# XiangLi2022/CM-TTS

Measured on AMD Instinct MI355X. Metric: mel-frames/s (text->mel hot path, consistency sampling T=4), higher is better.
Workload: dtype f32

## Files before the change

cm-tts_amd/_lib.py:

```python
import ctypes as C
import os
import sys

_HERE = os.path.dirname(os.path.abspath(__file__))
LIB_PATH = os.environ.get("CMTTS_LIB") or os.path.join(_HERE, "libcmtts_hip.so")


class CMTTSConfigStruct(C.Structure):
    _fields_ = [(n, C.c_int32) for n in (
        "n_symbols", "hidden", "enc_layers", "enc_heads", "ffn_kernel",
        "pred_filter", "pred_layers", "pred_kernel", "dur_layers", "dur_kernel", "cwt_hidden",
        "pitch_bins", "energy_bins", "use_uv", "multi_speaker", "external_speaker_dim", "n_speaker",
        "n_mels", "res_layers", "res_channels")] + [(n, C.c_float) for n in (
            "cwt_std_scale", "pitch_norm_eps", "sigma_min", "sigma_max", "sigma_data", "rho")]


class VarianceControlsStruct(C.Structure):
    _fields_ = [("p_control", C.c_float), ("e_control", C.c_float), ("d_target", C.c_void_p), ("e_target", C.c_void_p),
                ("cwt_spec", C.c_void_p), ("f0_mean", C.c_void_p), ("f0_std", C.c_void_p), ("uv", C.c_void_p)]


class ControlTablesStruct(C.Structure):
    _fields_ = [("d", C.c_void_p), ("e", C.c_void_p), ("p", C.c_void_p), ("ld", C.c_int)]

# ... 77 lines not shown
    "cmtts_comm_destroy": (_i, [_vp]),
    "cmtts_allgather_workspace_bytes": (_sz, [_i, _i, _i, _i]),
    "cmtts_allgather_mels": (_i, [_vp, _i, _vp, _vp, _i, _i, _i, _vp, _vp, _vp, _sz, _vp]),
    "cmtts_allgather_pcm_workspace_bytes": (_sz, [_i, _i, _i64]),
    "cmtts_allgather_pcm": (_i, [_vp, _i, _vp, _vp, _i, _i64, _vp, _vp, _vp, _sz, _vp]),
    "cmtts_exchange_records": (_i, [_vp, _i, _vp, C.POINTER(_i64), _vp, C.POINTER(_i64), _sz, _vp]),
    "cmtts_transpose": (_i, [_vp, _vp, _i, _i, _i, _vp]),
    "cmtts_pack_conv_weight": (_i, [_vp, _i, _i, _i, C.POINTER(_vp), C.POINTER(_i)]),
    "cmtts_free_device": (None, [_vp]),
    "cmtts_conv1d": (_i, [_vp, _vp, _i, _vp, _i, _i, _i, _i, _i, _i, _i, _i, _vp, _vp]),
}

ABI_VERSION = 8
_lib = None
HEADER_PATH = os.path.join(os.path.dirname(_HERE), "include", "cmtts_hip.h")


def cdef_from_header(path=HEADER_PATH):
    import re
    text = open(path).read()
    text = re.sub(r"/\*.*?\*/", "", text, flags=re.S)
    lines = [ln for ln in text.splitlines() if not ln.lstrip().startswith("#")]
    text = "\n".join(lines)
    text = text.replace('extern "C" {', "")
    text = re.sub(r"^\}\s*$", "", text, flags=re.M)
    return text


def address_of(arg):
    if arg is None:
        return 0
    if isinstance(arg, int):
        return arg
    if isinstance(arg, C.c_void_p):
        return arg.value or 0
    if hasattr(arg, "_obj"):
        return C.addressof(arg._obj)
    if isinstance(arg, (C.Array, C.Structure)):
        return C.addressof(arg)
    if isinstance(arg, C._Pointer):
        return C.cast(arg, C.c_void_p).value or 0
    if hasattr(arg, "data_ptr"):
        return int(arg.data_ptr())
    raise TypeError(f"cannot take the address of {type(arg).__name__}")


class _CffiLib:

    def __init__(self, path):
        import cffi
        self.ffi = cffi.FFI()
        self.ffi.cdef(cdef_from_header())
        self._c = self.ffi.dlopen(path)
        for name, (res, args) in SIGNATURES.items():
            setattr(self, name, self._wrap(name, res, args))

    def _wrap(self, name, res, args):
        ffi, fn = self.ffi, getattr(self._c, name)
        ctypes_ = ffi.typeof(fn).args
        assert len(ctypes_) == len(args), name

        def call(*a):
            conv = []
            for v, ct, at in zip(a, ctypes_, args):
                if at is C.c_char_p:
                    conv.append(ffi.NULL if v is None else v)
                elif ct.kind == "pointer":
                    conv.append(ffi.cast(ct, address_of(v)))
                else:
                    conv.append(v.value if hasattr(v, "value") else v)
            r = fn(*conv)
            if res is C.c_char_p:
                return None if r == ffi.NULL else ffi.string(r)
            return None if res is None else int(r)
        call.__name__ = name
        return call


def _load_ctypes():
    lib = C.CDLL(LIB_PATH)
    for name, (res, args) in SIGNATURES.items():
        fn = getattr(lib, name)
        fn.restype = res
        fn.argtypes = args
    return lib


def load():
    global _lib
    if _lib is not None:
        return _lib
    if not os.path.exists(LIB_PATH):
        raise RuntimeError(
            f"{LIB_PATH} not found: build the HIP extension first "
            "(python -c 'import __graft_entry__ as g; g.build()' or make -C cm-tts_amd/csrc). "
            "cmtts_amd has no CPU or PyTorch fallback.")
    import torch
    want = os.environ.get("CMTTS_FFI", "ctypes")
    if want == "cffi":
        import cffi
        lib = _CffiLib(LIB_PATH)
    elif want == "ctypes":
        lib = _load_ctypes()
    else:
        raise RuntimeError(f"CMTTS_FFI={want!r}: expected 'ctypes' or 'cffi'")
    got = lib.cmtts_abi_version()
    if got != ABI_VERSION:
        raise RuntimeError(f"{LIB_PATH} implements ABI revision {got}, this binding was written for {ABI_VERSION} "
                           "(include/cmtts_hip.h: CMTTS_ABI_VERSION): rebuild the library")
    _lib = lib
    spec = os.environ.get("CMTTS_INTERNAL", "")
    if spec:
        if os.environ.get("CMTTS_INTERNAL_ENABLE") != "1":
            print(f"cmtts_amd: ignoring CMTTS_INTERNAL={spec!r} (measurement hook: set CMTTS_INTERNAL_ENABLE=1 to apply it)", file=sys.stderr)
        else:
            for kv in filter(None, (e.strip() for e in spec.split(","))):
                k, sep, v = kv.partition("=")
                try:
                    val = int(v)
                except ValueError:
                    val = None
                if not sep or not k.strip() or val is None:
                    raise RuntimeError(f"CMTTS_INTERNAL: malformed entry {kv!r} (expected name=integer[,name=integer...])")
                if internal_set(k.strip(), val) < 0:
                    raise RuntimeError(f"CMTTS_INTERNAL: unknown switch {k.strip()!r} (csrc/internal_hooks.h)")
                print(f"cmtts_amd: CMTTS_INTERNAL applied {k.strip()}={val}", file=sys.stderr)
    return lib


_internal = None


def internal_set(name, value):
    global _internal
    load()
    if _internal is None:
        _internal = C.CDLL(LIB_PATH).cmtts_internal_set
        _internal.restype, _internal.argtypes = _i, [C.c_char_p, _i]
    return _internal(name if isinstance(name, bytes) else name.encode(), int(value))


_noise_bits = None


def internal_noise_bits(seeds, B, T, M, first_draw, n_draws, t0, bits, stream):
    global _noise_bits
    load()
    if _noise_bits is None:
        _noise_bits = C.CDLL(LIB_PATH).cmtts_internal_noise_bits
        _noise_bits.restype, _noise_bits.argtypes = _i, [_vp, _i, _i, _i, _i, _i, _i64, _vp, _vp]
    return _noise_bits(seeds, int(B), int(T), int(M), int(first_draw), int(n_draws), int(t0), bits, stream)


def backend():
    return "cffi" if isinstance(load(), _CffiLib) else "ctypes"


def check(rc):
    if rc != 0:
        msg = load().cmtts_last_error()
        raise RuntimeError(f"libcmtts_hip error {rc}: {msg.decode() if msg else '?'}")
```

cm-tts_amd/csrc/cmtts_api.hip:

```cpp
#include <hip/hip_runtime.h>
#include <limits.h>
#include <math.h>
#include <stdio.h>
#include <stdlib.h>
#include <string.h>

#include <algorithm>
#include <map>
#include <string>
#include <vector>

#include "../../include/cmtts_hip.h"
#include "internal_hooks.h"
#include "conv_args.h"
#include "kernels.h"
#include "resblock_args.h"
#include "persist_args.h"
#include "cond_gemm.h"
#include "resblock_pair.h"
#include "inproj.h"
#include "attention.h"
#include "text_state.h"
#include "stream_windows.h"
#include "resample.h"
// ... 966 lines not shown
            }
        if (H % 16 == 0 && (NL * C) % 32 == 0 && m->cond_all.ld == NL * C) {
            const std::vector<unsigned short> fs = to_fragment16_split(hp, 1, H, NL * C);
            CHK(al.upload_bytes(fs.data(), fs.size() * 2, &m->cond_all_f16[2]));
        }
    }
    CHK(al.upload(dproj, &m->dproj_wt));
    if (c.multi_speaker) CHK(al.upload(sproj, &m->sproj_wt));
    {
        GET(w, "net.skip_projection.conv.weight", C, C, 1); GET(b, "net.skip_projection.conv.bias", C);
        std::vector<float> hp;
        CHK(pack_conv(al, *w, b, nullptr, &m->skip_proj, &hp));
        if (C % 32 == 0 && m->skip_proj.ld == C) CHK(al.upload(to_fragment_order(hp, 1, C, C), &m->skip_f));
        GET(w2, "net.output_projection.conv.weight", c.n_mels, C, 1); GET(b2, "net.output_projection.conv.bias", c.n_mels);
        CHK(pack_conv(al, *w2, b2, nullptr, &m->out_proj, &hp));
        {
            const int ld = m->out_proj.ld, Mp = round_up(c.n_mels, 32);
            std::vector<float> padded((size_t)C * Mp, 0.f);
            for (int k = 0; k < C; ++k)
                for (int n = 0; n < c.n_mels; ++n) padded[(size_t)k * Mp + n] = hp[(size_t)k * ld + n];
            CHK(al.upload(to_fragment_order(padded, 1, C, Mp), &m->outp_f));
        }
    }
    if (m->cond_all_f && (NL * C) % 512 == 0) {
        GET(pe, va + "pitch_embed.weight", c.pitch_bins, H);
        float* peT = nullptr;
        void* p2 = nullptr;
        CHK(al.upload(transpose2d(pe->data.data(), c.pitch_bins, H), &peT));
        CHK(al.upload(std::vector<float>((size_t)NL * C, 0.f), &m->cond_zero_bias));
        HIPCHK(hipMalloc(&p2, (size_t)NL * C * c.pitch_bins * sizeof(float) + 256));
        al.ptrs.push_back(p2);
        CondGemmArgs ga;
        memset(&ga, 0, sizeof(ga));
        ga.X = peT; ga.Wf = m->cond_all_f; ga.bias = m->cond_all.bias; ga.Y = (float*)p2;
        ga.B = 1; ga.T = c.pitch_bins; ga.M = NL * C; ga.K = H; ga.force = 1; ga.row_split = NL * C / 512;
        if (cmtts_launch_cond_gemm(&ga, nullptr) == 0) {
            void* p2t = nullptr;
            HIPCHK(hipMalloc(&p2t, (size_t)NL * C * c.pitch_bins * sizeof(float) + 256));
            al.ptrs.push_back(p2t);
            k_transpose((const float*)p2, (float*)p2t, NL, C, c.pitch_bins, nullptr);
            HIPCHK(hipStreamSynchronize(nullptr));
            m->cond_p2 = (float*)p2;
            m->cond_p2t = (float*)p2t;
        }
    }
#undef GET
#undef UP
    m->host.clear();
    m->finalized = true;
    return 0;
}

constexpr int FFN2_SEG = 8;
struct TextWs {
    float *x, *h, *qk, *vt, *st, *o, *f, *part, *c1, *c2, *spk, *out1, *h128, *logd, *dround, *epred, *escaled, *pctl;
    int* cum;
    int64_t *eidx, *mlen;
    size_t bytes;
};
TextWs carve_text(const cmtts_config& c, int B, int L, void* base) {
    const int Lp = round_up(L, 4), H = c.hidden;
    Carver cv(base);
    TextWs w;
    const size_t n = (size_t)B * H * Lp;
    w.out1 = cv.take<float>(n);
    w.cum = cv.take<int>((size_t)B * L);
    w.spk = cv.take<float>((size_t)B * H);
    w.h128 = cv.take<float>((size_t)B * c.cwt_hidden * Lp);
    w.x = cv.take<float>(n);
    w.h = cv.take<float>(n);
    w.qk = cv.take<float>(3 * n);
    w.vt = w.qk + 2 * n;
    w.st = cv.take<float>((size_t)B * c.enc_heads * Lp * Lp);
    w.o = cv.take<float>(n);
    w.f = cv.take<float>(4 * n);
    w.part = cv.take<float>(FFN2_SEG * n);
    w.c1 = cv.take<float>(n);
    w.c2 = cv.take<float>(n);
    w.logd = cv.take<float>((size_t)B * L);
    w.dround = cv.take<float>((size_t)B * L);
    w.epred = cv.take<float>((size_t)B * L);
    w.eidx = cv.take<int64_t>((size_t)B * L);
    w.mlen = cv.take<int64_t>((size_t)B);
    w.escaled = cv.take<float>((size_t)B * L);
    w.pctl = cv.take<float>((size_t)B * L);
    w.bytes = cv.off + 256;
    return w;
}

struct FrameWs {
    float *xlr, *h128, *hp, *c1, *c2, *cwt, *r, *s1, *s2, *stats, *f0;
    int64_t* pidx;
    size_t bytes;
};
FrameWs carve_frame(const cmtts_config& c, int B, int T, void* base) {
    Carver cv(base);
    FrameWs w;
    const size_t n = (size_t)B * c.hidden * T;
    w.xlr = cv.take<float>(n);
    w.h128 = cv.take<float>((size_t)B * c.cwt_hidden * T);
    w.hp = cv.take<float>((size_t)B * c.cwt_hidden * T);
    w.c1 = cv.take<float>(n);
    w.c2 = cv.take<float>(n);
    w.cwt = cv.take<float>((size_t)B * T * 16);
    w.r = cv.take<float>((size_t)B * T);
    w.s1 = cv.take<float>((size_t)B * c.cwt_hidden);
    w.s2 = cv.take<float>((size_t)B * c.cwt_hidden);
    w.stats = cv.take<float>((size_t)B * 2);
    w.f0 = cv.take<float>((size_t)B * T);
    w.pidx = cv.take<int64_t>((size_t)B * T);
    w.bytes = cv.off + 256;
    return w;
}

struct DenWs {
    float *hin, *h, *u, *zb, *skip, *emb, *e1, *e2, *dproj, *sproj, *dp, *tbuf, *xcur, *cp;
    float* pst;
    unsigned long long* halo;
    size_t bytes;
};
DenWs carve_den(const cmtts_config& c, int B, int T, void* base) {
    Carver cv(base);
    DenWs w;
    const int C = c.res_channels, NL = c.res_layers;
    const size_t n = (size_t)B * C * T;
    w.hin = cv.take<float>((size_t)B * c.n_mels * T);
    w.h = cv.take<float>(n);
    w.u = cv.take<float>(n);
    w.zb = cv.take<float>(n);
    w.skip = cv.take<float>(n);
    w.emb = cv.take<float>((size_t)B * C);
    w.e1 = cv.take<float>((size_t)B * 4 * C);
    w.e2 = cv.take<float>((size_t)B * C);
    w.dproj = cv.take<float>((size_t)B * NL * C);
    w.sproj = cv.take<float>((size_t)B * NL * C);
    w.dp = cv.take<float>((size_t)B * NL * C);
    w.tbuf = cv.take<float>((size_t)B);
    w.xcur = cv.take<float>((size_t)B * T * c.n_mels);
    w.cp = cv.take<float>((size_t)NL * n);
    w.halo = cv.take<unsigned long long>(cmtts_persist_halo_bytes(B, T) / sizeof(unsigned long long));
    w.pst = cv.take<float>(cmtts_persist_state_floats(B, T));
    w.bytes = cv.off + 256;
    return w;
}

struct EnergyHead {
    const float* xin; const float* e_target; float e_control; const float* bins; int nbins; const float* E; float* out1; int64_t* e_idx; float* e_scaled;
    bool done;
    const float* e_table = nullptr;
};
int g_energy_head = 1;
int g_pred_wino = 1;
int g_pred_xres = 1;
int predictor(const Predictor& P, const float* in, int ld_in, int B, int T, int ld, const int64_t* ln_lens,
              const int64_t* out_lens, float* bufA, float* bufB, float* out, int O, hipStream_t s, int mode16 = 0, bool frame_level = false,
              EnergyHead* eh = nullptr) {
    const float* cur = in;
    int ldc = ld_in;
    auto other = [&](const float* p) { return p == bufA ? bufB : bufA; };
    int pend_ln = -1;
    for (size_t li = 0; li < P.convs.size(); ++li) {
        const PackedConv& w = P.convs[li];
        int rx = -2;
        float* dst = other(cur);
        if (frame_level && !mode16 && g_pred_wino && !ln_lens && li < P.convs_q.size() && P.convs_q[li] && w.taps == 5 && w.cout == 256 &&
            (pend_ln < 0 || w.cin == 256)) {
            ConvXlArgs xa;
            memset(&xa, 0, sizeof(xa));
            xa.x = cur; xa.y = dst; xa.wf = P.convs_q[li]; xa.bias = w.bias; xa.bstride = (long)w.cout * ld;
            xa.B = B; xa.C = 256; xa.T = T; xa.ld = ld; xa.k = w.taps; xa.dil = 1; xa.slope = 1.0f; xa.relu = 1;
            if (w.cin != 256) { xa.cin = w.cin; xa.xbstride = (long)w.cin * ldc; }
            if (pend_ln >= 0) { xa.ln_g = P.ln_g[pend_ln]; xa.ln_b = P.ln_b[pend_ln]; xa.ln_eps = 1e-12f; }
            if (ldc == ld || w.cin != 256) {
                rx = cmtts_launch_conv_k5q(&xa, (void*)s);
                if (rx == -3) return fail(CMTTS_E_HIP, "conv_k5q launch failed");
                if (rx == 0) pend_ln = -2;
            }
        }
        const bool small = (long)((T + 63) / 64) * B < 192;
        if (rx != 0 && !mode16 && g_pred_xres && small && P.convs_f[li] && w.cin == 256 && w.cout == 256 && ldc == ld) {
            ConvArgs a = conv_args(w, cur, T, ldc, (long)w.cin * ldc, dst, ld, (long)w.cout * ld, T);
            a.out[0].act = ACT_RELU;
            a.xres_nt = 1;
            if (pend_ln >= 0) { a.ln_g = P.ln_g[pend_ln]; a.ln_b = P.ln_b[pend_ln]; a.ln_eps = 1e-12f; a.ln_lens = ln_lens; a.ln_skip_tiles = 1; }
            rx = cmtts_launch_conv_xres(&a, P.convs_f[li], B, (void*)s);
            if (rx == -3) return fail(CMTTS_E_HIP, "conv_xres launch failed");
            if (rx == 0) pend_ln = -2;
        }
        if (pend_ln >= 0) {
            float* nd = other(cur);
            k_layernorm_ct(cur, nd, P.ln_g[pend_ln], P.ln_b[pend_ln], 1e-12f, ln_lens, B, T, ld, s);
            cur = nd;
            dst = other(cur);
        }
        pend_ln = -1;
        if (mode16 && li < P.convs_f16[mode16 - 1].size() && P.convs_f16[mode16 - 1][li]) {
            ConvArgs a = conv_args(w, cur, T, ldc, (long)w.cin * ldc, dst, ld, (long)w.cout * ld, T);
            a.out[0].act = ACT_RELU;
            a.text_epi = 1;
            rx = cmtts_launch_conv16(&a, P.convs_f16[mode16 - 1][li], mode16, B, (void*)s);
            if (rx == -3) return fail(CMTTS_E_HIP, "text16: predictor conv launch failed");
        }
        if (rx != 0 && g_pred_xl && P.convs_f[li] && ldc == ld && (long)((T + 63) / 64) * B >= 192) {
            ConvXlArgs xa;
            memset(&xa, 0, sizeof(xa));
            xa.x = cur; xa.y = dst; xa.wf = P.convs_f[li]; xa.bias = w.bias; xa.bstride = (long)w.cout * ld;
            xa.B = B; xa.C = 256; xa.T = T; xa.ld = ld; xa.k = w.taps; xa.dil = 1; xa.slope = 1.0f; xa.relu = 1;
            if (w.cin != 256) { xa.cin = w.cin; xa.xbstride = (long)w.cin * ldc; }
            rx = cmtts_launch_conv_xl(&xa, (void*)s);
            if (rx == -3) return fail(CMTTS_E_HIP, "conv_xl launch failed");
        }
        if (rx != 0) {
            ConvArgs a = conv_args(w, cur, T, ldc, (long)w.cin * ldc, dst, ld, (long)w.cout * ld, T);
            a.out[0].act = ACT_RELU;
            CHK(launch(a, EPI_PLAIN, B, s));
        }
        cur = dst;
        ldc = ld;
        if (g_pred_head && eh && g_energy_head && O == 1 && li + 1 == P.convs.size() && w.cout == 256) {
            k_ln_linear_energy(cur, P.ln_g[li], P.ln_b[li], 1e-12f, P.lin_w, P.lin_b, out, ln_lens, out_lens, B, T, ld, eh->xin, eh->e_target, eh->e_control,
                               eh->bins, eh->nbins, eh->E, eh->out1, eh->e_idx, eh->e_scaled, s, eh->e_table);
            eh->done = true;
            return 0;
        }
        if (g_pred_head && li + 1 == P.convs.size() && w.cout == 256 &&
            k_ln_linear(cur, P.ln_g[li], P.ln_b[li], 1e-12f, P.lin_w, P.lin_b, out, ln_lens, out_lens, B, T, ld, O, s))
            return 0;
        pend_ln = (int)li;
    }
    if (pend_ln >= 0) {
        float* nd = other(cur);
        k_layernorm_ct(cur, nd, P.ln_g[pend_ln], P.ln_b[pend_ln], 1e-12f, ln_lens, B, T, ld, s);
        cur = nd;
    }
    k_chan_linear(cur, P.lin_w, P.lin_b, out, out_lens, B, P.convs.back().cout, T, ld, O, s);
    return 0;
}

int cond_projections(cmtts_model* m, const DenWs& w, const float* cond_ct, int B, int T, hipStream_t s) {
    const cmtts_config& c = m->cfg;
    if (g_cond_gemm16 && m->precision >= 1 && m->precision <= 3 && m->cond_all_f16[m->precision - 1]) {
        CondGemmArgs g;
        g.X = cond_ct; g.Wf = nullptr; g.bias = m->cond_all.bias; g.Y = w.cp;
        g.row_split = 0;
        g.B = B; g.T = T; g.M = c.res_layers * c.res_channels; g.K = c.hidden; g.force = 1;
        const int r = cmtts_launch_cond_gemm16(&g, m->cond_all_f16[m->precision - 1], m->precision, (void*)s);
        if (r == 0) return 0;
        if (r != -2) return fail(CMTTS_E_HIP, "cond_gemm16 launch failed");
    }
    if (m->cond_all_f) {
        CondGemmArgs g;
        g.X = cond_ct; g.Wf = m->cond_all_f; g.bias = m->cond_all.bias; g.Y = w.cp;
        g.row_split = 0;
        g.B = B; g.T = T; g.M = c.res_layers * c.res_channels; g.K = c.hidden; g.force = g_cond_gemm == 2;
        const int r = g_cond_gemm ? cmtts_launch_cond_gemm(&g, (void*)s) : -2;
        if (r == 0) return 0;
        if (r != -2) return fail(CMTTS_E_HIP, "cond_gemm launch failed");
    }
    ConvArgs a = conv_args(m->cond_all, cond_ct, T, T, (long)c.hidden * T, w.cp, T, (long)c.res_layers * c.res_channels * T, T);
    return launch(a, EPI_PLAIN, B, s);
}

struct CondFactors {
    const float* p1 = nullptr;
    const float* p1t = nullptr;
    int ldp = 0, L = 0;
    const int64_t* mel2ph = nullptr;
    const int64_t* p_idx = nullptr;
    bool usable(const cmtts_model* m) const;
};
int g_cond_factored = 1;
int g_cond_inkernel = 1;
inline bool C_IS_256(const cmtts_config& c) { return c.res_channels == 256; }
bool CondFactors::usable(const cmtts_model* m) const {
    return g_cond_factored && p1 && mel2ph && p_idx && m->precision == 0 && m->cond_p2 && g_fused_resblock;
}
int cond_factored(cmtts_model* m, const DenWs& w, const CondFactors& f, int B, int T, hipStream_t s) {
    const cmtts_config& c = m->cfg;
    const int r = cmtts_launch_cond_expand(f.p1, f.ldp, f.L, m->cond_p2, c.pitch_bins, f.mel2ph, f.p_idx, w.cp, B, c.res_layers * c.res_channels, T, (void*)s);
    return r == 0 ? 0 : fail(CMTTS_E_HIP, "cond_expand launch failed");
}
int cond_phoneme_factor(cmtts_model* m, const float* out1, int B, int Lp, float* p1, hipStream_t s) {
    const cmtts_config& c = m->cfg;
    if (!m->cond_p2) return fail(CMTTS_E_UNSUPPORTED, "factored conditioner projections are not available for this model");
    CondGemmArgs g;
    memset(&g, 0, sizeof(g));
    g.X = out1; g.Wf = m->cond_all_f; g.bias = m->cond_zero_bias; g.Y = p1;
    g.B = B; g.T = Lp; g.M = c.res_layers * c.res_channels; g.K = c.hidden; g.force = 1;
    g.flat = 1;
    const long tiles = ((long)B * Lp + 63) / 64;
    const int npass = g.M / 512;
    int best = 1;
    double best_t = 1e30;
    for (int sp = 1; sp <= npass; ++sp) {
        const int ppg = (npass + sp - 1) / sp, groups = (npass + ppg - 1) / ppg;
        const long wg = tiles * groups, cap = persist_blocks();
        const double t = (double)((wg + cap - 1) / cap) * ppg;
        if (t < best_t - 1e-9) { best_t = t; best = sp; }
    }
    g.row_split = best;
    const int r = cmtts_launch_cond_gemm(&g, (void*)s);
    return r == 0 ? 0 : fail(r == -2 ? CMTTS_E_UNSUPPORTED : CMTTS_E_HIP, "cond_gemm (phoneme factor) launch failed");
}

int step_embedding(cmtts_model* m, const DenWs& w, const float* timesteps, const float* spk, int B, hipStream_t s,
                   float t_host = NAN) {
    const cmtts_config& c = m->cfg;
    const int C = c.res_channels, NL = c.res_layers;
    if (c.multi_speaker && !spk) return fail(CMTTS_E_INVALID, "speaker_emb is required for a multi-speaker model");
    const bool cacheable = g_step_cache && t_host == t_host;
    if (cacheable) {
        for (const cmtts_model::StepRow& e : m->step_rows)
            if (e.t == t_host && hipEventQuery(e.ready) == hipSuccess) {
                k_broadcast_row(e.row, w.dproj, B, NL * C, s);
                if (c.multi_speaker) {
                    k_dense_small(spk, c.hidden, 1, m->sproj_wt, nullptr, nullptr, w.sproj, B, c.hidden, NL * C, DENSE_NONE, s);
                    k_add_rows(w.dproj, w.sproj, w.dp, (long)B * NL * C, s);
                }
                return 0;
            }
    }
    k_diff_embed(timesteps, m->omega_res, w.emb, B, C, s);
    k_dense_small(w.emb, C, 1, m->mlp0_wt, nullptr, nullptr, w.e1, B, C, 4 * C, DENSE_MISH, s);
    k_dense_small(w.e1, 4 * C, 1, m->mlp2_wt, nullptr, nullptr, w.e2, B, 4 * C, C, DENSE_NONE, s);
    k_dense_small(w.e2, C, 1, m->dproj_wt, nullptr, nullptr, w.dproj, B, C, NL * C, DENSE_NONE, s);
    if (c.multi_speaker) {
        k_dense_small(spk, c.hidden, 1, m->sproj_wt, nullptr, nullptr, w.sproj, B, c.hidden, NL * C, DENSE_NONE, s);
        k_dense_small(w.e2, C, 1, m->dproj_wt, nullptr, w.sproj, w.dp, B, C, NL * C, DENSE_NONE, s);
    }
    if (cacheable && m->step_rows.size() < 16) {
        bool known = false;
        for (const cmtts_model::StepRow& e : m->step_rows) known = known || e.t == t_host;
        if (!known) {
            cmtts_model::StepRow e{t_host, nullptr, nullptr};
            void* p = nullptr;
            if (hipMalloc(&p, (size_t)NL * C * sizeof(float)) == hipSuccess && hipEventCreateWithFlags(&e.ready, hipEventDisableTiming) == hipSuccess) {
                e.row = (float*)p;
                m->al.ptrs.push_back(p);
                HIPCHK(hipMemcpyAsync(e.row, w.dproj, (size_t)NL * C * sizeof(float), hipMemcpyDeviceToDevice, s));
                HIPCHK(hipEventRecord(e.ready, s));
                m->step_rows.push_back(e);
            } else if (p) {
                (void)hipFree(p);
            }
        }
    }
    return 0;
}

struct MelPost {
    const float* xold;
    const float* noise;
    float c_out, c_skip, nstd;
    float* out;
};

int denoiser_prologue(cmtts_model* m, const DenWs& w, const float* x_src, float in_scale, const float* timesteps, const float* spk, int B,
                      int T, hipStream_t s, bool embed, float t_host, bool* halo_zeroed) {
    const cmtts_config& c = m->cfg;
    const int C = c.res_channels, NL = c.res_layers, M = c.n_mels;
    const long cs = (long)C * T;
    *halo_zeroed = false;
    int rin = -2;
    if (g_inproj_fused && m->in_proj_f) {
        InProjArgs ia;
        memset(&ia, 0, sizeof(ia));
        ia.x = x_src; ia.scale = in_scale; ia.wf = m->in_proj_f; ia.bias = m->in_proj.bias; ia.h = w.h;
        ia.B = B; ia.T = T; ia.M = M; ia.C = C;
        const bool persist_path = g_fused_resblock && g_persist && NL <= PERSIST_MAX_LAYERS;
        if (persist_path) { ia.zero = w.halo; ia.zero_f4 = (long)(cmtts_persist_halo_bytes(B, T) / 16); }
        rin = cmtts_launch_inproj(&ia, (void*)s);
        if (rin == -3) return fail(CMTTS_E_HIP, "inproj launch failed");
        *halo_zeroed = rin == 0 && persist_path && cmtts_persist_halo_bytes(B, T) % 16 == 0;
    }
    if (rin != 0) {
        k_mel_prep(x_src, nullptr, in_scale, w.hin, B, T, M, s);
        ConvArgs a = conv_args(m->in_proj, w.hin, T, T, (long)M * T, w.h, T, cs, T);
        a.out[0].act = ACT_RELU;
        CHK(launch(a, EPI_PLAIN, B, s));
    }
    if (embed) CHK(step_embedding(m, w, timesteps, spk, B, s, t_host));
    return 0;
}

int batch_invariant_form(const cmtts_model* m) {
    if (!m->batch_invariant || m->precision != 0 || !m->winograd || !g_persist_wino || !m->res[0].w3w) return 0;
    return m->winograd == 1 && g_persist_wino == 3 && m->res[0].w3w43 ? 1 : -1;
}
int check_batch_invariant(const cmtts_model* m) {
    if (batch_invariant_form(m) >= 0) return 0;
    return fail(CMTTS_E_UNSUPPORTED, "batch_invariant: the persistent denoiser stack runs the F(2,3) form (model option \"winograd\" = 2), "
                                     "which has no per-layer counterpart; set \"winograd\" to 1 or 0");
}

int denoiser_core(cmtts_model* m, const DenWs& w, const float* x_src, float in_scale, const float* timesteps,
                  const float* cond_ct, const float* spk, int B, int T, const MelPost& post, hipStream_t s, bool embed = true,
                  SideStream* pending = nullptr, float t_host = NAN,
                  const CondFactors* cfk = nullptr, bool* cp_ready = nullptr) {
    CHK(check_device_flag(true));
    const cmtts_config& c = m->cfg;
    const int C = c.res_channels, NL = c.res_layers, M = c.n_mels;
    const long cs = (long)C * T;
    bool halo_zeroed = false;
    CHK(denoiser_prologue(m, w, x_src, in_scale, timesteps, spk, B, T, s, embed, t_host, &halo_zeroed));
    if (pending) CHK(branch_join(pending));
    const float* dp = m->cfg.multi_speaker ? w.dp : w.dproj;
    const bool unfused = !g_fused_resblock;
    float* hcur = w.h;
    float* halt = w.u;
    bool layers_done = false;
    if (!unfused && g_persist && NL <= PERSIST_MAX_LAYERS) {
        PersistArgs pa;
        memset(&pa, 0, sizeof(pa));
        pa.x0 = w.h; pa.cp = w.cp; pa.cp_bstride = (long)NL * C * T;
        pa.dp = dp; pa.d = w.dproj; pa.vec_stride = (long)NL * C;
        pa.skip = w.skip; pa.halo = w.halo; pa.tmo = g_tmo_host;
        pa.B = B; pa.T = T; pa.NL = NL;
        pa.halo_zeroed = halo_zeroed;
        const int prec = m->precision;
        if (cfk && !(cp_ready && *cp_ready)) {
            pa.fact = 1; pa.p1 = cfk->p1; pa.p2 = m->cond_p2; pa.mel2ph = (const long long*)cfk->mel2ph; pa.pidx = (const long long*)cfk->p_idx;
            pa.ldp = cfk->ldp; pa.Lph = cfk->L; pa.ld2 = c.pitch_bins;
            pa.p1t = cfk->p1t; pa.p2t = m->cond_p2t;
        }
        if (g_persist_tail && m->skip_f && m->outp_f) {
            pa.tail = 1;
            pa.Wsf = m->skip_f; pa.bs = m->skip_proj.bias; pa.Wpf = m->outp_f; pa.bp = m->out_proj.bias;
            pa.skip_div = (float)sqrt((double)NL); pa.n_mels = M;
            pa.xold = post.xold; pa.noise = post.noise; pa.c_out = post.c_out; pa.c_skip = post.c_skip; pa.nstd = post.nstd;
            pa.out = post.out;
        }
        pa.wino = g_persist_wino && m->winograd && !prec && m->res[0].w3w && w.pst;
        if (pa.wino && g_persist_wino == 3 && m->winograd == 1 && m->res[0].w3w43) pa.wino = 3;
        pa.xst = w.pst;
        for (int l = 0; l < NL; ++l) {
            pa.W3f[l] = prec ? (const float*)m->res[l].w3f16[prec - 1] : (pa.wino == 3 ? m->res[l].w3w43 : pa.wino ? m->res[l].w3w : m->res[l].w3f);
            pa.Wof[l] = prec ? (const float*)m->res[l].wof16[prec - 1] : m->res[l].wof;
            pa.b3[l] = m->res[l].b3f; pa.bo[l] = m->res[l].outp.bias;
        }
        const bool prof = g_prof.on && g_prof.used + 2 <= g_prof.ev.size();
        const int need = cmtts_persist_plan(B, T, NL, persist_blocks(), g_persist == 2);
        if (need) CHK(persist_admit(s, need, persist_blocks()));
        if (prof) (void)hipEventRecord(g_prof.ev[g_prof.used], s);
        const int rc = prec ? cmtts_launch_denoiser_persist_lp(&pa, prec, persist_blocks(), g_persist == 2, (void*)s)
                            : cmtts_launch_denoiser_persist(&pa, persist_blocks(), g_persist == 2, (void*)s);
        if (rc == -3) return fail(CMTTS_E_HIP, "persistent denoiser launch failed");
        if (rc == 0) {
            CHK(persist_launched(s, need));
            if (prof) { (void)hipEventRecord(g_prof.ev[g_prof.used + 1], s); g_prof.used += 2; }
            layers_done = true;
            if (pa.tail) return 0;
        }
    }
    if (!layers_done && cfk && !(cp_ready && *cp_ready)) {
        CHK(cond_factored(m, w, *cfk, B, T, s));
        if (cp_ready) *cp_ready = true;
    }
    const bool w43 = batch_invariant_form(m) > 0;
    for (int l = 0; l < NL && !layers_done; ++l) {
        const ResLayer& R = m->res[l];
        const bool prof = g_prof.on && g_prof.used + 2 <= g_prof.ev.size() && (g_prof.seen++ % g_prof.stride) == 0;
        if (!unfused) {
            ResArgs ra;
            memset(&ra, 0, sizeof(ra));
            ra.x_in = hcur; ra.cp = w.cp + (long)l * C * T; ra.cp_bstride = (long)NL * C * T;
            ra.dp = dp + (long)l * C; ra.d = w.dproj + (long)l * C;
            ra.x_out = halt; ra.skip = w.skip;
            ra.W3f = R.w3f; ra.b3 = R.b3f; ra.Wof = R.wof; ra.bo = R.outp.bias;
            ra.vec_stride = (long)NL * C; ra.B = B; ra.T = T; ra.accum_skip = l > 0; ra.flag = g_tmo_host;
            if (prof) (void)hipEventRecord(g_prof.ev[g_prof.used], s);
            int lrc;
            if (m->precision == 0 || m->precision == 3) {
                const long tiles32 = (long)((T + 31) / 32) * B;
                ra.z = w.zb;
                if (w43) {
                    ra.W3f = R.w3w43;
                    lrc = cmtts_launch_resblock_w43(&ra, (void*)s);
                } else if (g_split_resblock == 2 || (g_split_resblock == 1 && tiles32 <= SPLIT_MAX_TILES)) lrc = cmtts_launch_resblock_split(&ra, (void*)s);
                else lrc = cmtts_launch_resblock(&ra, (void*)s);
            } else {
                ra.W3f = (const float*)R.w3f16[m->precision - 1];
                ra.Wof = (const float*)R.wof16[m->precision - 1];
                lrc = cmtts_launch_resblock_lp(&ra, m->precision, (void*)s);
            }
            if (lrc != 0) return fail(CMTTS_E_HIP, "fused residual block launch failed");
            if (prof) { (void)hipEventRecord(g_prof.ev[g_prof.used + 1], s); g_prof.used += 2; }
            float* t = hcur; hcur = halt; halt = t;
            continue;
        }
        {
            ConvArgs a = conv_args(R.cond, cond_ct, T, T, (long)c.hidden * T, halt, T, cs, T);
            a.out[0].bvec = dp + (long)l * C; a.out[0].bvec_zs = (long)NL * C;
            a.out[0].res = hcur; a.out[0].r_zs0 = cs; a.out[0].ldr = T;
            CHK(launch(a, EPI_PLAIN, B, s));
        }
        if (w43) {
            ResArgs ra;
            memset(&ra, 0, sizeof(ra));
            ra.u = halt; ra.x_in = hcur; ra.x_out = halt; ra.skip = w.skip; ra.z = w.zb;
            ra.d = w.dproj + (long)l * C; ra.dp = dp + (long)l * C; ra.cp = w.cp;
            ra.W3f = R.w3w43; ra.b3 = R.b3f; ra.Wof = R.wof; ra.bo = R.outp.bias;
// ... 235 lines not shown
            }
        }
        if (ffn_fused) {
            k_reduce_partials(w.part, FFN2_SEG, E.ffn2.bias, w.x, src_lens, w.x, B, H, L, Lp, s);
        } else if (ffn2_seg) {
            const int kseg = E.ffn2.cin / FFN2_SEG;
            ConvArgs a = conv_args(E.ffn2, w.f, L, Lp, 4 * hs, w.part, Lp, (long)FFN2_SEG * hs, L);
            a.K = kseg;
            a.zdiv = FFN2_SEG; a.a_zs0 = 0; a.a_zs1 = (long)kseg * a.a_ld; a.x_zs1 = (long)kseg * Lp;
            a.out[0].y_zs1 = hs; a.out[0].bias = nullptr;
            CHK(launch(a, EPI_PLAIN, B * FFN2_SEG, s));
            k_reduce_partials(w.part, FFN2_SEG, E.ffn2.bias, w.x, src_lens, w.x, B, H, L, Lp, s);
        } else {
            ConvArgs a = conv_args(E.ffn2, w.f, L, Lp, 4 * hs, w.x, Lp, hs, L);
            a.out[0].res = w.x; a.out[0].r_zs0 = hs; a.out[0].ldr = Lp; a.out[0].lens = src_lens;
            CHK(launch(a, EPI_PLAIN, B, s));
        }
    }
    return 0;
}

int cmtts_text_forward(cmtts_model* m, const int64_t* texts, const int64_t* src_lens, const float* spker_embeds,
                       const int64_t* speakers, int B, int L, float d_control, float* log_d, float* d_rounded, int64_t* mel_len,
                       float* e_pred, int64_t* e_idx, float* enc_out_ct, float* speaker_emb,
                       void* text_ws, size_t text_ws_bytes, void* stream) {
    return cmtts_text_forward_ragged(m, texts, src_lens, nullptr, spker_embeds, speakers, B, L, d_control, log_d, d_rounded, mel_len, e_pred,
                                     e_idx, enc_out_ct, speaker_emb, text_ws, text_ws_bytes, stream);
}

int cmtts_text_forward_ragged(cmtts_model* m, const int64_t* texts, const int64_t* src_lens, const int64_t* pad_lens, const float* spker_embeds,
                              const int64_t* speakers, int B, int L, float d_control, float* log_d, float* d_rounded, int64_t* mel_len,
                              float* e_pred, int64_t* e_idx, float* enc_out_ct, float* speaker_emb,
                              void* text_ws, size_t text_ws_bytes, void* stream) {
    if (!m || !m->finalized) return fail(CMTTS_E_INVALID, "model not finalized");
    if (!texts || !src_lens || !text_ws || B <= 0 || L <= 0) return fail(CMTTS_E_INVALID, "cmtts_text_forward: bad argument");
    const cmtts_config& c = m->cfg;
    if (c.multi_speaker && c.n_speaker > 0 && !speakers) return fail(CMTTS_E_INVALID, "speakers (ids into the speaker_emb table) are required (model/cmtts.py:78)");
    if (c.multi_speaker && c.n_speaker <= 0 && !spker_embeds) return fail(CMTTS_E_INVALID, "Speaker embedding should not be None (model/cmtts.py:80)");
    const cmtts_control_tables& ct = m->ct;
    if ((ct.d || ct.e || ct.p) && ct.ld != L)
        return fail(CMTTS_E_INVALID, "cmtts_text_forward: the control tables' row pitch ld must equal L (cmtts_set_control_tables)");
    if (ct.d && d_control != 1.0f)
        return fail(CMTTS_E_INVALID, "cmtts_text_forward: a duration table replaces d_control, which must then be 1");
    if (ct.e && m->vc.e_control != 1.0f)
        return fail(CMTTS_E_INVALID, "cmtts_text_forward: an energy table replaces e_control, which must then be 1");
    TextWs w = carve_text(c, B, L, text_ws);
    if (text_ws_bytes < w.bytes) return fail(CMTTS_E_WORKSPACE, "text workspace too small");
    hipStream_t s = (hipStream_t)stream;
    const int H = c.hidden, Lp = round_up(L, 4);
    if (!log_d) log_d = w.logd;
    if (!d_rounded) d_rounded = w.dround;
    if (!mel_len) mel_len = w.mlen;
    if (!e_pred) e_pred = w.epred;
    if (!e_idx) e_idx = w.eidx;

    k_embed_tokens(texts, src_lens, m->embed, m->omega_h, m->pe_h, PE_ROWS, w.x, B, L, Lp, H, (float)sqrt((double)H), s);
    CHK(fft_stack(m, m->enc, w, src_lens, B, L, s, pad_lens));
    k_layernorm_ct(w.x, w.x, m->encln_g, m->encln_b, 1e-5f, src_lens, B, L, Lp, s);
    if (enc_out_ct && c.multi_speaker)
        k_copy_rows(enc_out_ct, L, w.x, Lp, L, (long)B * H, s);
    if (c.multi_speaker) {
        if (c.n_speaker > 0) k_gather_rows(m->spk_table, speakers, w.spk, B, H, c.n_speaker, s);
        else k_dense_small(spker_embeds, c.external_speaker_dim, 1, m->spk_wt, m->spk_b, nullptr, w.spk, B,
                      c.external_speaker_dim, H, DENSE_NONE, s);
        k_add_rowvec(w.x, w.spk, B, H, L, Lp, s, pad_lens);
        if (speaker_emb) HIPCHK(hipMemcpyAsync(speaker_emb, w.spk, (size_t)B * H * 4, hipMemcpyDeviceToDevice, s));
    }
    SideStream* ss = side_for(s);
    hipStream_t se = ss ? ss->side : s;
    float* ec1 = ss ? w.qk : w.c1;
    float* ec2 = ss ? w.qk + (size_t)B * H * Lp : w.c2;
    if (ss) CHK(branch_fork(ss));
    const int t16mode = (m->text16 && (m->precision == 1 || m->precision == 2)) ? m->precision : 0;
    CHK(predictor(m->dur, w.x, Lp, B, L, Lp, src_lens, src_lens, w.c1, w.c2, log_d, 1, s, t16mode));
    if (m->vc.d_target) {
        HIPCHK(hipMemcpyAsync(d_rounded, m->vc.d_target, (size_t)B * L * 4, hipMemcpyDeviceToDevice, s));
        k_cumsum_durations(m->vc.d_target, w.cum, mel_len, B, L, s);
    } else if (ct.d) {
        k_durations_table(log_d, ct.d, d_rounded, w.cum, mel_len, B, L, s);
    } else {
        k_durations(log_d, d_control, d_rounded, w.cum, mel_len, B, L, s);
    }
    if (ct.p) HIPCHK(hipMemcpyAsync(w.pctl, ct.p, (size_t)B * L * 4, hipMemcpyDeviceToDevice, s));
    if (enc_out_ct && !c.multi_speaker)
        k_copy_rows(enc_out_ct, L, w.x, Lp, L, (long)B * H, s);
    k_pos_embed_add(w.x, w.h, m->energy.alpha, m->omega_h, m->pe_h, PE_ROWS, B, H, L, Lp, se);
    EnergyHead eh{w.x, m->vc.e_target, m->vc.e_control, m->energy_bins, c.energy_bins - 1, m->energy_emb, w.out1, e_idx, w.escaled, false, ct.e};
    CHK(predictor(m->energy, w.h, Lp, B, L, Lp, pad_lens, pad_lens, ec1, ec2, e_pred, 1, se, t16mode, false, H == 256 ? &eh : nullptr));
    if (ss) CHK(branch_join(ss));
    if (!eh.done)
        k_energy_embed(w.x, e_pred, w.escaled, m->vc.e_target, m->vc.e_control, m->energy_bins, c.energy_bins - 1, m->energy_emb,
                       w.out1, e_idx, B, H, L, Lp, s, ct.e);
    {
        ConvArgs a = conv_args(m->cwt_in, w.out1, L, Lp, (long)H * Lp, w.h128, Lp, (long)c.cwt_hidden * Lp, L);
        int rc = -2;
        if (g_ffn_xres && g_pred_xres && m->cwt_in_f) {
            a.xres_nt = 1;
            rc = cmtts_launch_conv_xres(&a, m->cwt_in_f, B, (void*)s);
            if (rc == -3) return fail(CMTTS_E_HIP, "conv_xres launch failed");
            a.xres_nt = 0;
        }
        if (rc != 0) CHK(launch(a, EPI_PLAIN, B, s));
    }
    if (!m->vc.e_target && (ct.e || m->vc.e_control != 1.0f))
        HIPCHK(hipMemcpyAsync(e_pred, w.escaled, (size_t)B * L * 4, hipMemcpyDeviceToDevice, s));
    HIPCHK(hipGetLastError());
    return 0;
}

int cmtts_frame_forward(cmtts_model* m, const void* text_ws, int B, int L, int T, float* cond_ct, int64_t* mel2ph,
                        float* cwt_out, float* f0_denorm, int64_t* p_idx, float* f0_stats, void* frame_ws,
                        size_t frame_ws_bytes, void* stream) {
    return cmtts_frame_forward_sub(m, text_ws, B, L, 0, B, T, cond_ct, mel2ph, cwt_out, f0_denorm, p_idx, f0_stats, nullptr, frame_ws, frame_ws_bytes, stream);
}

int cmtts_frame_forward_sub(cmtts_model* m, const void* text_ws, int B_all, int L_all, int b0, int B, int T, float* cond_ct, int64_t* mel2ph,
                            float* cwt_out, float* f0_denorm, int64_t* p_idx, float* f0_stats, float* cond_p1, void* frame_ws,
                            size_t frame_ws_bytes, void* stream) {
    return cmtts_frame_forward_sub_t(m, text_ws, B_all, L_all, b0, B, T, cond_ct, mel2ph, cwt_out, f0_denorm, p_idx, f0_stats, cond_p1, nullptr, frame_ws,
                                     frame_ws_bytes, stream);
}

int cmtts_frame_forward_sub_t(cmtts_model* m, const void* text_ws, int B_all, int L_all, int b0, int B, int T, float* cond_ct, int64_t* mel2ph,
                              float* cwt_out, float* f0_denorm, int64_t* p_idx, float* f0_stats, float* cond_p1, float* cond_p1t, void* frame_ws,
                              size_t frame_ws_bytes, void* stream) {
    if (!m || !m->finalized) return fail(CMTTS_E_INVALID, "model not finalized");
    if (!text_ws || !frame_ws || !cond_ct || !mel2ph || B <= 0 || L_all <= 0 || T <= 0 || b0 < 0 || b0 + B > B_all)
        return fail(CMTTS_E_INVALID, "cmtts_frame_forward: bad argument");
    const cmtts_config& c = m->cfg;
    const int L = L_all;
    TextWs tw = carve_text(c, B_all, L_all, const_cast<void*>(text_ws));
    tw.out1 += (size_t)b0 * c.hidden * round_up(L_all, 4);
    tw.h128 += (size_t)b0 * c.cwt_hidden * round_up(L_all, 4);
    tw.cum += (size_t)b0 * L_all;
    tw.pctl += (size_t)b0 * L_all;
    if (m->ct.p && m->ct.ld != L_all)
        return fail(CMTTS_E_INVALID, "cmtts_frame_forward: the control tables' row pitch ld must equal L_all (cmtts_set_control_tables)");
    if (m->ct.p && m->vc.p_control != 1.0f)
        return fail(CMTTS_E_INVALID, "cmtts_frame_forward: a pitch table replaces p_control, which must then be 1");
    FrameWs w = carve_frame(c, B, T, frame_ws);
    if (frame_ws_bytes < w.bytes) return fail(CMTTS_E_WORKSPACE, "frame workspace too small");
    hipStream_t s = (hipStream_t)stream;
    const int H = c.hidden, Lp = round_up(L, 4), O = c.use_uv ? 11 : 10, CH = c.cwt_hidden;
    if (!cwt_out) cwt_out = w.cwt;
    if (!f0_denorm) f0_denorm = w.f0;
    if (!p_idx) p_idx = w.pidx;
    if (!f0_stats) f0_stats = w.stats;

    SideStream* ss = side_for(s);
    hipStream_t sst = ss ? ss->side : s;
    if (ss) CHK(branch_fork(ss));
    if (cond_p1t && !cond_p1) return fail(CMTTS_E_INVALID, "cmtts_frame_forward_sub_t: cond_p1t needs cond_p1");
    if (cond_p1 && m->cond_p2) {
        CHK(cond_phoneme_factor(m, tw.out1, B, Lp, cond_p1, sst));
        if (cond_p1t) k_transpose(cond_p1, cond_p1t, B * c.res_layers, c.res_channels, Lp, sst);
    }
    if (!(g_stats_mlp && k_stats_mlp(tw.out1, (long)H * Lp, Lp, m->st0_wt, m->st0_b, m->st2_wt, m->st2_b, m->st4_wt, m->st4_b, f0_stats, B, H, CH, CH, 2, sst))) {
        k_dense_small(tw.out1, (long)H * Lp, Lp, m->st0_wt, m->st0_b, nullptr, w.s1, B, H, CH, DENSE_RELU, sst);
        k_dense_small(w.s1, CH, 1, m->st2_wt, m->st2_b, nullptr, w.s2, B, CH, CH, DENSE_RELU, sst);
        k_dense_small(w.s2, CH, 1, m->st4_wt, m->st4_b, nullptr, f0_stats, B, CH, 2, DENSE_NONE, sst);
    }
    k_mel2ph(tw.cum, mel2ph, B, L, T, s);
    if (!g_cwt_in_phoneme) k_length_regulate(tw.out1, mel2ph, w.xlr, B, H, Lp, T, s);
    bool hp_done = false;
    if (g_cwt_in_phoneme) {
        k_pos_embed_add_lr(tw.h128, Lp, mel2ph, m->cwt_in.bias, w.hp, m->cwt.alpha, m->omega_cwt, m->pe_cwt, PE_ROWS, B, CH, T, s);
        hp_done = true;
    } else {
        ConvArgs a = conv_args(m->cwt_in, w.xlr, T, T, (long)H * T, w.h128, T, (long)CH * T, T);
        CHK(launch(a, EPI_PLAIN, B, s));
    }
    if (!hp_done) k_pos_embed_add(w.h128, w.hp, m->cwt.alpha, m->omega_cwt, m->pe_cwt, PE_ROWS, B, CH, T, T, s);
    CHK(predictor(m->cwt, w.hp, T, B, T, T, nullptr, nullptr, w.c1, w.c2, cwt_out, O, s, (m->text16 && (m->precision == 1 || m->precision == 2)) ? m->precision : 0, true));
    if (ss) CHK(branch_join(ss));
    if (m->ct.p) k_pitch_table_scale(cwt_out, mel2ph, tw.cum, tw.pctl, B, O, L, T, s);
    else if (m->vc.p_control != 1.0f) k_scale(cwt_out, cwt_out, (long)B * T * O, m->vc.p_control, s);
    if (m->vc.cwt_spec) {
        k_pitch_index(m->vc.cwt_spec, 10, m->vc.f0_mean, m->vc.f0_std, 1, 1.0f, nullptr, 0, c.use_uv ? m->vc.uv : nullptr,
                      c.pitch_norm_eps, w.r, p_idx, f0_denorm, B, T, s);
    } else {
        k_pitch_index(cwt_out, O, f0_stats, f0_stats + 1, 2, c.cwt_std_scale, c.use_uv ? cwt_out + (O - 1) : nullptr, O, nullptr,
                      c.pitch_norm_eps, w.r, p_idx, f0_denorm, B, T, s);
    }
    if (g_cwt_in_phoneme) k_lr_gather_add(tw.out1, mel2ph, Lp, p_idx, m->pitch_emb, cond_ct, B, H, T, s);
    else k_gather_add(w.xlr, p_idx, m->pitch_emb, cond_ct, B, H, T, s);
    HIPCHK(hipGetLastError());
    return 0;
}

namespace {
struct TextStateLayout {
    long off[TEXT_STATE_MAX_REGIONS], bytes[TEXT_STATE_MAX_REGIONS], stride[TEXT_STATE_MAX_REGIONS];
    long rec_bytes;
    int n_regions;
};
TextStateLayout text_state_layout(const cmtts_config& c, int L, bool with_p) {
    const int Lp = round_up(L, 4);
    TextStateLayout t;
    t.bytes[0] = (long)c.hidden * Lp * 4;
    t.bytes[1] = (long)c.cwt_hidden * Lp * 4;
    t.bytes[2] = (long)c.hidden * 4;
    t.bytes[3] = (long)L * 4;
    t.bytes[4] = (long)L * 4;
    t.n_regions = with_p ? 5 : 4;
    long off = TEXT_STATE_HEADER_BYTES;
    for (int g = 0; g < t.n_regions; ++g) {
        t.stride[g] = t.bytes[g];
        t.off[g] = off;
        off += (t.bytes[g] + 15) / 16 * 16;
    }
    t.rec_bytes = off;
    return t;
}
TextStateCopy text_state_args(const cmtts_config& c, void* ws, int B_all, int L, void* records, int n, int unpack, bool with_p) {
    const TextStateLayout t = text_state_layout(c, L, with_p);
    TextWs tw = carve_text(c, B_all, L, ws);
    char* base[TEXT_STATE_MAX_REGIONS] = {(char*)tw.out1, (char*)tw.h128, (char*)tw.spk, (char*)tw.cum, (char*)tw.pctl};
    TextStateCopy a;
    memset(&a, 0, sizeof(a));
    int chunks = 0;
    for (int g = 0; g < t.n_regions; ++g) {
        TextStateRegion& R = a.reg[g];
        R.ws = base[g]; R.ws_stride = t.stride[g]; R.rec_off = t.off[g]; R.bytes = t.bytes[g];
        R.vec16 = ((uintptr_t)R.ws % 16 == 0 && R.ws_stride % 16 == 0 && R.bytes % 16 == 0 && (uintptr_t)records % 16 == 0) ? 1 : 0;
        R.chunk0 = chunks;
        chunks += (int)((R.bytes + TEXT_STATE_CHUNK - 1) / TEXT_STATE_CHUNK);
    }
    a.n_regions = t.n_regions; a.n_chunks = chunks; a.unpack = unpack;
    a.layout = with_p ? TEXT_STATE_LAYOUT_P : TEXT_STATE_LAYOUT;
    a.n = n; a.B_all = B_all; a.L_all = L; a.hidden = c.hidden; a.cwt_hidden = c.cwt_hidden;
    a.rec = (char*)records; a.rec_bytes = t.rec_bytes;
    a.cum = tw.cum;
    return a;
}
}

size_t cmtts_text_state_record_bytes(const cmtts_model* m, int L_all) {
    if (!m || L_all <= 0) return 0;
    return (size_t)text_state_layout(m->cfg, L_all, m->ct.p != nullptr).rec_bytes;
}

int cmtts_text_state_pack(cmtts_model* m, const void* text_ws, int B_all, int L_all, const int32_t* rows, int n, const int64_t* global_idx,
                          const int64_t* src_lens, void* records, void* stream) {
    if (!m || !m->finalized) return fail(CMTTS_E_INVALID, "model not finalized");
    if (!text_ws || !records || (n > 0 && !rows) || B_all <= 0 || L_all <= 0 || n < 0)
        return fail(CMTTS_E_INVALID, "cmtts_text_state_pack: bad argument");
    if ((uintptr_t)records % 16) return fail(CMTTS_E_INVALID, "cmtts_text_state_pack: records must be 16-byte aligned");
    if (m->ct.p && m->ct.ld != L_all)
        return fail(CMTTS_E_INVALID, "cmtts_text_state_pack: the control tables' row pitch ld must equal L_all (cmtts_set_control_tables)");
    TextStateCopy a = text_state_args(m->cfg, const_cast<void*>(text_ws), B_all, L_all, records, n, 0, m->ct.p != nullptr);
    a.rows = rows; a.index = global_idx; a.src_lens = src_lens;
    if (cmtts_launch_text_state_copy(&a, stream) != 0) return fail(CMTTS_E_HIP, "text-state pack launch failed");
    return 0;
}

int cmtts_text_state_unpack(cmtts_model* m, const void* records, int n, int L_all, void* text_ws, size_t text_ws_bytes, void* stream) {
    if (!m || !m->finalized) return fail(CMTTS_E_INVALID, "model not finalized");
    if (!text_ws || !records || n <= 0 || L_all <= 0) return fail(CMTTS_E_INVALID, "cmtts_text_state_unpack: bad argument");
    if ((uintptr_t)records % 16) return fail(CMTTS_E_INVALID, "cmtts_text_state_unpack: records must be 16-byte aligned");
    if (text_ws_bytes < carve_text(m->cfg, n, L_all, nullptr).bytes) return fail(CMTTS_E_WORKSPACE, "text workspace too small");
    if (m->ct.p && m->ct.ld != L_all)
        return fail(CMTTS_E_INVALID, "cmtts_text_state_unpack: the control tables' row pitch ld must equal L_all (cmtts_set_control_tables)");
    TextStateCopy a = text_state_args(m->cfg, text_ws, n, L_all, const_cast<void*>(records), n, 1, m->ct.p != nullptr);
    if (cmtts_launch_text_state_copy(&a, stream) != 0) return fail(CMTTS_E_HIP, "text-state unpack launch failed");
    return 0;
}

int cmtts_length_regulate(const float* x_ct, const float* durations, int B, int C, int L, int T, float* out_ct,
                          int64_t* mel2ph, int64_t* mel_len, int32_t* scratch_cum, void* stream) {
    if (!x_ct || !durations || !out_ct || !mel2ph || !mel_len || !scratch_cum || B <= 0 || L <= 0 || T <= 0)
        return fail(CMTTS_E_INVALID, "cmtts_length_regulate: bad argument");
    hipStream_t s = (hipStream_t)stream;
    k_cumsum_durations(durations, scratch_cum, mel_len, B, L, s);
    k_mel2ph(scratch_cum, mel2ph, B, L, T, s);
    k_length_regulate(x_ct, mel2ph, out_ct, B, C, L, T, s);
    HIPCHK(hipGetLastError());
    return 0;
}

int cmtts_denoiser_forward(cmtts_model* m, const float* x, const float* timesteps, const float* cond_ct,
                           const float* speaker_emb, int B, int T, float* out, void* ws, size_t ws_bytes, void* stream) {
    if (!m || !m->finalized) return fail(CMTTS_E_INVALID, "model not finalized");
    if (!x || !timesteps || !cond_ct || !out || !ws || B <= 0 || T <= 0)
        return fail(CMTTS_E_INVALID, "cmtts_denoiser_forward: bad argument");
    CHK(check_batch_invariant(m));
    DenWs w = carve_den(m->cfg, B, T, ws);
    if (ws_bytes < w.bytes) return fail(CMTTS_E_WORKSPACE, "denoiser workspace too small");
    hipStream_t s = (hipStream_t)stream;
    SideStream* ss = g_fused_resblock ? side_for(s) : nullptr;
    if (ss) CHK(branch_fork(ss));
    if (g_fused_resblock) CHK(cond_projections(m, w, cond_ct, B, T, ss ? ss->side : s));
    const MelPost post = {nullptr, nullptr, 1.0f, 0.0f, 0.0f, out};
    CHK(denoiser_core(m, w, x, 1.0f, timesteps, cond_ct, speaker_emb, B, T, post, s, true, ss));
    HIPCHK(hipGetLastError());
    return 0;
}

int cmtts_schedule(const cmtts_model* m, int n_steps, float* sigmas, float* renoise_std) {
    if (!m || !sigmas || !renoise_std || n_steps < 1) return fail(CMTTS_E_INVALID, "cmtts_schedule: bad argument");
    const cmtts_config& c = m->cfg;
    if (n_steps == 1) {
        sigmas[0] = c.sigma_max;
        renoise_std[0] = -1.0f;
        return 0;
    }
    const double rho = c.rho, tmax = pow((double)c.sigma_max, 1.0 / rho), tmin = pow((double)c.sigma_min, 1.0 / rho);
    for (int i = 0; i < n_steps; ++i) {
        const double tsi = 0.0, tsn = (i + 1 == n_steps) ? 1.0 : 0.0;
        const double t = pow(tmax + tsi / 1.0 * (tmin - tmax), rho);
        double nt = pow(tmax + tsn / 1.0 * (tmin - tmax), rho);
        nt = nt < c.sigma_min ? (double)c.sigma_min : (nt > c.sigma_max ? (double)c.sigma_max : nt);
        sigmas[i] = (float)t;
        renoise_std[i] = (float)sqrt(nt * nt - (double)c.sigma_min * (double)c.sigma_min);
    }
    return 0;
}

}
namespace {
int sample_core(cmtts_model* m, const DenWs& w, const float* noise, long noise_stride, const float* cond_ct, const float* speaker_emb, int B,
                int T, int n_steps, const float* sigmas, const float* renoise_std, float* mel, hipStream_t s, const CondFactors* cf = nullptr,
                const int64_t* seeds = nullptr) {
    const cmtts_config& c = m->cfg;
    const long nel = (long)B * T * c.n_mels;
    SideStream* ss = g_fused_resblock ? side_for(s) : nullptr;
    if (ss) CHK(branch_fork(ss));
    const CondFactors* cfk = nullptr;
    CondFactors cf_local;
    bool cp_ready = false;
    if (g_fused_resblock) {
        if (cf && cf->usable(m)) {
            const bool inkernel = g_cond_inkernel && g_persist && g_persist_tail && m->skip_f && m->outp_f && c.res_layers <= PERSIST_MAX_LAYERS &&
                                  cmtts_persist_plan(B, T, c.res_layers, persist_blocks(), g_persist == 2) > 0;
            if (inkernel && cf->ldp <= T && m->cond_p2t && C_IS_256(c)) {
                cf_local = *cf;
                if (!cf_local.p1t) {
                    k_transpose(cf->p1, w.cp, B * c.res_layers, c.res_channels, cf->ldp, ss ? ss->side : s);
                    cf_local.p1t = w.cp;
                }
                cfk = &cf_local;
            } else CHK(cond_factored(m, w, *cf, B, T, ss ? ss->side : s));
        } else CHK(cond_projections(m, w, cond_ct, B, T, ss ? ss->side : s));
    }
    const float* renoise0 = noise + noise_stride;
    if (seeds) {
        renoise0 = noise;
        int n_re = 0;
        for (int i = 0; i < n_steps; ++i)
            if (renoise_std[i] >= 0.0f) n_re = i + 1;
        if (cmtts_launch_noise_fill(seeds, B, T, c.n_mels, 0, 1, 0, c.sigma_max, w.xcur, nullptr, (void*)s) != 0 ||
            (n_re && cmtts_launch_noise_fill(seeds, B, T, c.n_mels, 1, n_re, 0, 1.0f, const_cast<float*>(noise), nullptr, (void*)(ss ? ss->side : s)) != 0))
            return fail(CMTTS_E_HIP, "seeded noise launch failed");
    } else
        k_scale(noise, w.xcur, nel, c.sigma_max, s);
    const float smin = c.sigma_min, sd2 = c.sigma_data * c.sigma_data;
    for (int i = 0; i < n_steps; ++i) {
        const float sg = sigmas[i];
        const float dm = sg - smin;
        const float c_skip = sd2 / (dm * dm + sd2);
        const float rt = sqrtf(sg * sg + sd2);
        const float c_out = dm * c.sigma_data / rt;
        const float c_in = 1.0f / rt;
        const float t_resc = 250.0f * logf(sg + 1e-44f);
        const bool new_sigma = i == 0 || sigmas[i] != sigmas[i - 1];
        const bool embed_side = i == 0 && ss != nullptr;
        if (new_sigma) k_fill_float(w.tbuf, t_resc, B, embed_side ? ss->side : s);
        if (embed_side) CHK(step_embedding(m, w, w.tbuf, speaker_emb, B, ss->side, t_resc));
        const bool last = i + 1 == n_steps;
        const bool renoise = renoise_std[i] >= 0.0f;
        const MelPost post = {w.xcur, renoise ? renoise0 + (long)i * noise_stride : nullptr, c_out, c_skip,
                              renoise ? renoise_std[i] : 0.0f, last ? mel : w.xcur};
        CHK(denoiser_core(m, w, w.xcur, c_in, w.tbuf, cond_ct, speaker_emb, B, T, post, s, new_sigma && !embed_side, i == 0 ? ss : nullptr, t_resc, cfk, &cp_ready));
    }
    HIPCHK(hipGetLastError());
    return 0;
}

DenWs den_slice(const cmtts_config& c, const DenWs& w, int b0, int T) {
    const long C = c.res_channels, NL = c.res_layers, M = c.n_mels;
    DenWs v = w;
    v.hin += (long)b0 * M * T; v.h += b0 * C * T; v.u += b0 * C * T; v.zb += b0 * C * T; v.skip += b0 * C * T;
    v.emb += b0 * C; v.e1 += b0 * 4 * C; v.e2 += b0 * C; v.dproj += b0 * NL * C; v.sproj += b0 * NL * C; v.dp += b0 * NL * C;
    v.tbuf += b0; v.xcur += (long)b0 * T * M; v.cp += (long)b0 * NL * C * T;
    return v;
}
}
extern "C" {

int cmtts_sample(cmtts_model* m, const float* noise, const float* cond_ct, const float* speaker_emb, int B, int T,
                 int n_steps, const float* sigmas, const float* renoise_std, float* mel, void* ws, size_t ws_bytes,
                 void* stream) {
    if (!m || !m->finalized) return fail(CMTTS_E_INVALID, "model not finalized");
    if (!noise || !cond_ct || !mel || !ws || !sigmas || !renoise_std || B <= 0 || T <= 0 || n_steps < 1)
        return fail(CMTTS_E_INVALID, "cmtts_sample: bad argument");
    CHK(check_batch_invariant(m));
    const cmtts_config& c = m->cfg;
    DenWs w = carve_den(c, B, T, ws);
    if (ws_bytes < w.bytes) return fail(CMTTS_E_WORKSPACE, "denoiser workspace too small");
    return sample_core(m, w, noise, (long)B * T * c.n_mels, cond_ct, speaker_emb, B, T, n_steps, sigmas, renoise_std, mel, (hipStream_t)stream);
}

int cmtts_sample_factored(cmtts_model* m, const float* noise, const float* cond_ct, const float* speaker_emb, int B, int T,
                          int n_steps, const float* sigmas, const float* renoise_std, float* mel, void* ws, size_t ws_bytes,
                          void* stream, const float* cond_p1, int p1_ld, int L, const int64_t* mel2ph, const int64_t* p_idx) {
    return cmtts_sample_factored_t(m, noise, cond_ct, speaker_emb, B, T, n_steps, sigmas, renoise_std, mel, ws, ws_bytes, stream, cond_p1, nullptr, p1_ld, L,
                                   mel2ph, p_idx);
}

int cmtts_sample_factored_t(cmtts_model* m, const float* noise, const float* cond_ct, const float* speaker_emb, int B, int T,
                            int n_steps, const float* sigmas, const float* renoise_std, float* mel, void* ws, size_t ws_bytes,
                            void* stream, const float* cond_p1, const float* cond_p1t, int p1_ld, int L, const int64_t* mel2ph, const int64_t* p_idx) {
    if (!m || !m->finalized) return fail(CMTTS_E_INVALID, "model not finalized");
    if (!noise || !cond_ct || !mel || !ws || !sigmas || !renoise_std || B <= 0 || T <= 0 || n_steps < 1)
        return fail(CMTTS_E_INVALID, "cmtts_sample_factored: bad argument");
    if (cond_p1 && (!mel2ph || !p_idx || L <= 0 || p1_ld < L)) return fail(CMTTS_E_INVALID, "cmtts_sample_factored: incomplete factors");
    CHK(check_batch_invariant(m));
    const cmtts_config& c = m->cfg;
    DenWs w = carve_den(c, B, T, ws);
    if (ws_bytes < w.bytes) return fail(CMTTS_E_WORKSPACE, "denoiser workspace too small");
    CondFactors cf;
    cf.p1 = cond_p1; cf.ldp = p1_ld; cf.L = L; cf.mel2ph = mel2ph; cf.p_idx = p_idx;
    cf.p1t = cond_p1 ? cond_p1t : nullptr;
    return sample_core(m, w, noise, (long)B * T * c.n_mels, cond_ct, speaker_emb, B, T, n_steps, sigmas, renoise_std, mel, (hipStream_t)stream,
                       cond_p1 ? &cf : nullptr);
}

int cmtts_noise_fill(const int64_t* seeds, int B, int T, int M, int first_draw, int n_draws, int64_t t0, float* out, void* stream) {
    if (!seeds || !out || B < 1 || T < 1 || M < 1 || n_draws < 1 || first_draw < 0 || t0 < 0)
        return fail(CMTTS_E_INVALID, "cmtts_noise_fill: bad argument");
    const int rc = cmtts_launch_noise_fill(seeds, B, T, M, first_draw, n_draws, t0, 1.0f, out, nullptr, stream);
    if (rc == -2) return fail(CMTTS_E_UNSUPPORTED, "cmtts_noise_fill: B or n_draws > 65535, or T * ceil(M / 4) >= 2^31");
    if (rc != 0) return fail(CMTTS_E_HIP, "cmtts_noise_fill: launch failed");
    return 0;
}

int cmtts_noise_fill_groups(const cmtts_noise_group* groups, int n_groups, int M, int first_draw, int n_draws, void* stream) {
    if (!groups || n_groups < 1 || M < 1 || n_draws < 1 || first_draw < 0) return fail(CMTTS_E_INVALID, "cmtts_noise_fill_groups: bad argument");
    std::vector<NoiseGroup> gs((size_t)n_groups);
    for (int g = 0; g < n_groups; ++g) {
        const cmtts_noise_group& G = groups[g];
        if (!G.seeds || !G.out || G.B < 1 || G.T < 1) return fail(CMTTS_E_INVALID, "cmtts_noise_fill_groups: bad group");
        gs[g] = NoiseGroup{G.seeds, G.out, G.B, G.T, 0, 1};
    }
    const int rc = cmtts_launch_noise_fill_groups(gs.data(), n_groups, M, first_draw, n_draws, stream);
    if (rc == -2) return fail(CMTTS_E_UNSUPPORTED, "cmtts_noise_fill_groups: n_draws > 65535 or a launch of more than 2^31 - 1 workgroups");
    if (rc != 0) return fail(CMTTS_E_HIP, "cmtts_noise_fill_groups: launch failed");
    return 0;
}

int cmtts_internal_noise_bits(const int64_t* seeds, int B, int T, int M, int first_draw, int n_draws, int64_t t0, uint32_t* bits, void* stream) {
    if (!seeds || !bits || B < 1 || T < 1 || M < 1 || n_draws < 1 || first_draw < 0 || t0 < 0)
        return fail(CMTTS_E_INVALID, "cmtts_internal_noise_bits: bad argument");
    if (cmtts_launch_noise_fill(seeds, B, T, M, first_draw, n_draws, t0, 1.0f, nullptr, bits, stream) != 0)
        return fail(CMTTS_E_HIP, "cmtts_internal_noise_bits: launch failed");
    return 0;
}

static size_t seeded_tail_offset(const cmtts_config& c, int B, int T) { return (carve_den(c, B, T, nullptr).bytes + 255) & ~(size_t)255; }
size_t cmtts_sample_seeded_workspace_bytes(const cmtts_model* m, int B, int T, int n_steps) {
    if (!m || B < 1 || T < 1 || n_steps < 1) return 0;
    return seeded_tail_offset(m->cfg, B, T) + (size_t)n_steps * B * T * m->cfg.n_mels * sizeof(float);
}

int cmtts_sample_seeded(cmtts_model* m, const int64_t* seeds, const float* cond_ct, const float* speaker_emb, int B, int T,
                        int n_steps, const float* sigmas, const float* renoise_std, float* mel, void* ws, size_t ws_bytes,
                        void* stream, const float* cond_p1, const float* cond_p1t, int p1_ld, int L, const int64_t* mel2ph, const int64_t* p_idx) {
    if (!m || !m->finalized) return fail(CMTTS_E_INVALID, "model not finalized");
    if (!seeds || !cond_ct || !mel || !ws || !sigmas || !renoise_std || B <= 0 || T <= 0 || n_steps < 1)
        return fail(CMTTS_E_INVALID, "cmtts_sample_seeded: bad argument");
    if (cond_p1 && (!mel2ph || !p_idx || L <= 0 || p1_ld < L)) return fail(CMTTS_E_INVALID, "cmtts_sample_seeded: incomplete factors");
    CHK(check_batch_invariant(m));
    const cmtts_config& c = m->cfg;
    if (B > 65535) return fail(CMTTS_E_UNSUPPORTED, "cmtts_sample_seeded: B > 65535");
    DenWs w = carve_den(c, B, T, ws);
    if (ws_bytes < cmtts_sample_seeded_workspace_bytes(m, B, T, n_steps)) return fail(CMTTS_E_WORKSPACE, "seeded sampler workspace too small");
    const float* tail = reinterpret_cast<const float*>(static_cast<char*>(ws) + seeded_tail_offset(c, B, T));
    CondFactors cf;
    cf.p1 = cond_p1; cf.ldp = p1_ld; cf.L = L; cf.mel2ph = mel2ph; cf.p_idx = p_idx;
    cf.p1t = cond_p1 ? cond_p1t : nullptr;
    return sample_core(m, w, tail, (long)B * T * c.n_mels, cond_ct, speaker_emb, B, T, n_steps, sigmas, renoise_std, mel, (hipStream_t)stream,
                       cond_p1 ? &cf : nullptr, seeds);
}

int cmtts_sample_ragged(cmtts_model* m, const cmtts_sample_group* groups, int n_groups, int n_steps, const float* sigmas,
                        const float* renoise_std, int tail_frames, void* stream) {
    if (!m || !m->finalized) return fail(CMTTS_E_INVALID, "model not finalized");
    if (!groups || n_groups < 1 || n_steps < 1 || !sigmas || !renoise_std || tail_frames < 0)
        return fail(CMTTS_E_INVALID, "cmtts_sample_ragged: bad argument");
    CHK(check_batch_invariant(m));
    const cmtts_config& c = m->cfg;
    const int C = c.res_channels, NL = c.res_layers, M = c.n_mels;
    hipStream_t s = (hipStream_t)stream;
    long padded_tiles = 0;
    for (int g = 0; g < n_groups; ++g) {
        const cmtts_sample_group& G = groups[g];
        if (!G.noise || !G.cond_ct || !G.mel || !G.ws || G.B <= 0 || G.T <= 0) return fail(CMTTS_E_INVALID, "cmtts_sample_ragged: bad group");
        if (c.multi_speaker && !G.speaker_emb) return fail(CMTTS_E_INVALID, "speaker_emb is required for a multi-speaker model");
        if (G.ws_bytes < carve_den(c, G.B, G.T, nullptr).bytes) return fail(CMTTS_E_WORKSPACE, "denoiser workspace too small");
        padded_tiles += (long)G.B * ((G.T + 63) / 64);
    }
    bool one_launch = m->precision == 0 && g_fused_resblock && g_persist && g_persist_tail && g_inproj_fused && m->skip_f && m->outp_f &&
                      m->in_proj_f && NL <= PERSIST_MAX_LAYERS && n_groups <= PERSIST_MAX_GROUPS && padded_tiles * 2 > persist_blocks();
    for (int g = 0; g < n_groups && one_launch; ++g)
        if ((groups[g].T + 63) / 64 > 127 || (groups[g].T + 63) / 64 > std::min(persist_blocks(), PERSIST_MAX_WG) || groups[g].B > 1023 || (long)C * groups[g].T >= (1L << 30) ||
            cmtts_persist_halo_bytes(groups[g].B, groups[g].T) % 16 != 0)
            one_launch = false;
    if (!one_launch) {
        for (int g = 0; g < n_groups; ++g) {
            const cmtts_sample_group& G = groups[g];
            const int rc = cmtts_sample_factored(m, G.noise, G.cond_ct, G.speaker_emb, G.B, G.T, n_steps, sigmas, renoise_std, G.mel, G.ws, G.ws_bytes,
                                                 stream, G.cond_p1, G.p1_ld, G.L, G.mel2ph, G.p_idx);
            if (rc != 0) return rc;
        }
        return 0;
    }
    CHK(check_device_flag(true));
    const int cap_all = std::min(persist_blocks(), PERSIST_MAX_WG);
    auto utt_tiles = [&](const cmtts_sample_group& G, int b, int eval) {
        const int tiles = (G.T + 63) / 64;
        if (!G.active_frames) return (long)tiles;
// ... 682 lines not shown
    if (!r) return fail(CMTTS_E_INVALID, "cmtts_resampler_half_width: null argument");
    return r->R;
}
int cmtts_resample_encode(cmtts_resampler* r, const float* wav, int rows, int64_t ld, const int32_t* segments, int N, int encoding,
                          float max_wav_value, void* out, int64_t out_ld, void* stream) {
    const char* who = "cmtts_resample_encode";
    if (!r || !wav || !segments || !out) return fail(CMTTS_E_INVALID, std::string(who) + ": null argument");
    if (rows <= 0 || ld <= 0 || N <= 0 || N > 65535 || out_ld <= 0)
        return fail(CMTTS_E_INVALID, std::string(who) + ": rows, ld, N and out_ld must be positive (N <= 65535)");
    if (encoding < CMTTS_ENC_F32 || encoding > CMTTS_ENC_ALAW) return fail(CMTTS_E_INVALID, std::string(who) + ": unknown encoding");
    if (!(max_wav_value > 0.f && max_wav_value <= 32768.f)) return fail(CMTTS_E_INVALID, std::string(who) + ": max_wav_value outside (0, 32768]");
    hipStream_t s = (hipStream_t)stream;
    std::vector<ResampleSegment> tab(N);
    bool on_host = false;
    CHK(fetch_table(who, segments, tab.data(), (size_t)N * sizeof(ResampleSegment), s, &on_host));
    const long L = r->L, M = r->M, half = r->half;
    auto fdiv = [](long a, long b) { return a >= 0 ? a / b : -((-a + b - 1) / b); };
    for (int n = 0; n < N; ++n) {
        const ResampleSegment& g = tab[n];
        const char* bad = nullptr;
        if (g.row < 0 || g.row >= rows) bad = "source row outside [0, rows)";
        else if (g.n_valid < 0) bad = "negative sample count";
        else if (g.m0 < 0 || g.m1 < g.m0) bad = "m0 < 0 or m1 < m0";
        else if ((long)g.m1 > ((long)g.n_valid * L + M - 1) / M) bad = "m1 beyond ceil(n L / M)";
        else if ((long)g.m1 - g.m0 > out_ld) bad = "more outputs than out_ld";
        else if (g.m1 > g.m0) {
            const long lo = std::max(-fdiv(-((long)g.m0 * M - half), L), 0L);
            const long hi = std::min(fdiv(((long)g.m1 - 1) * M + half, L), (long)g.n_valid - 1);
            if (lo <= hi && (lo < g.origin || hi >= (long)g.origin + ld)) bad = "the row does not hold the source samples these outputs need";
        }
        if (bad) {
            char msg[240];
            snprintf(msg, sizeof msg, "%s: segment %d (%d, %d, %d, %d, %d): %s", who, n, g.row, g.origin, g.m0, g.m1, g.n_valid, bad);
            return fail(CMTTS_E_INVALID, msg);
        }
    }
    if (N > r->seg_cap) {
        if (r->seg) (void)hipFree(r->seg);
        r->seg = nullptr; r->seg_cap = 0;
        const int cap = std::max(64, N);
        HIPCHK(hipMalloc(&r->seg, (size_t)cap * sizeof(ResampleSegment)));
        r->seg_cap = cap;
    }
    HIPCHK(hipMemcpyAsync(r->seg, segments, (size_t)N * sizeof(ResampleSegment), on_host ? hipMemcpyHostToDevice : hipMemcpyDeviceToDevice, s));
    const int rc = cmtts_launch_resample_encode(wav, (long)ld, r->seg, N, r->table, r->L, r->M, r->R, encoding, max_wav_value, out, (long)out_ld, (void*)s);
    if (rc != 0) return fail(CMTTS_E_HIP, "resample_encode launch failed");
    return 0;
}
int cmtts_internal_mel_window_gather(const float* mel_ct, int B, int T, const int32_t* windows, int N, int Tw, float* out, void* stream) {
    (void)B;
    if (!mel_ct || !windows || !out || N <= 0 || Tw <= 0 || Tw > T) return fail(CMTTS_E_INVALID, "cmtts_internal_mel_window_gather: bad argument");
    return cmtts_launch_mel_window_gather(mel_ct, 80, T, (const StreamWindow*)windows, N, Tw, out, stream) == 0 ? 0
                                                                                                              : fail(CMTTS_E_HIP, "gather launch failed");
}

struct Knob { const char* name; int* var; int lo, hi; };
static int knob_set(const Knob* tab, size_t n, const char* name, int value, bool* found) {
    for (size_t i = 0; i < n; ++i)
        if (!strcmp(name, tab[i].name)) {
            *found = true;
            const int prev = *tab[i].var;
            if (value >= tab[i].lo && value <= tab[i].hi) *tab[i].var = value;
            return prev;
        }
    *found = false;
    return 0;
}

int cmtts_set_option(const char* name, int value) {
    if (!name) return fail(CMTTS_E_INVALID, "cmtts_set_option: null name");
    if (!strcmp(name, "cooperative_launch")) {
        const int prev = cmtts_persist_set_cooperative(value == 2 ? -1 : (value == 0 || value == 1) ? value : -2);
        return prev < 0 ? 2 : prev;
    }
    if (!strcmp(name, "process_group")) {
        return cmtts_persist_note_process_group(value);
    }
    static const Knob tab[] = {
        {"branch_streams", &g_branch_streams, 0, 1},
        {"resblock_split", &g_split_resblock, 0, 2},
        {"step_cache", &g_step_cache, 0, 1},
    };
    bool found;
    const int prev = knob_set(tab, sizeof(tab) / sizeof(tab[0]), name, value, &found);
    if (found) return prev;
    return fail(CMTTS_E_INVALID, "cmtts_set_option: unknown option");
}

int cmtts_model_set_option(cmtts_model* m, const char* name, int value) {
    if (!m || !name) return fail(CMTTS_E_INVALID, "cmtts_model_set_option: null argument");
    const Knob tab[] = {
        {"ffn2_split", &m->ffn2_split, 0, 1},
        {"text16", &m->text16, 0, 1},
        {"winograd", &m->winograd, 0, 2},
        {"batch_invariant", &m->batch_invariant, 0, 1},
    };
    bool found;
    const int prev = knob_set(tab, sizeof(tab) / sizeof(tab[0]), name, value, &found);
    if (found) return prev;
    return fail(CMTTS_E_INVALID, "cmtts_model_set_option: unknown option");
}

int cmtts_vocoder_set_option(cmtts_vocoder* v, const char* name, int value) {
    if (!v || !name) return fail(CMTTS_E_INVALID, "cmtts_vocoder_set_option: null argument");
    const Knob tab[] = {
        {"ups16", &v->ups16, 0, 1},
        {"winograd", &v->winograd, 0, 1},
        {"batch_invariant", &v->batch_invariant, 0, 1},
    };
    bool found;
    const int prev = knob_set(tab, sizeof(tab) / sizeof(tab[0]), name, value, &found);
    if (found) return prev;
    return fail(CMTTS_E_INVALID, "cmtts_vocoder_set_option: unknown option");
}

int cmtts_internal_set(const char* name, int value) {
    if (!name) return fail(CMTTS_E_INVALID, "cmtts_internal_set: null name");
    static const Knob tab[] = {
        {"qkv_nt", &g_qkv_nt, 0, 3},
        {"cwt_in_phoneme", &g_cwt_in_phoneme, 0, 1},
        {"pred_xres", &g_pred_xres, 0, 1},
        {"xres_small", &g_xres_small, 0, 1},
        {"cond_inkernel", &g_cond_inkernel, 0, 1},
        {"cond_factored", &g_cond_factored, 0, 1},
        {"cond_gemm16", &g_cond_gemm16, 0, 1},
        {"cond_gemm", &g_cond_gemm, 0, 2},
        {"persist_tail", &g_persist_tail, 0, 1},
        {"persist_wino", &g_persist_wino, 0, 3},
        {"inproj_fused", &g_inproj_fused, 0, 1},
        {"ffn_xres", &g_ffn_xres, 0, 1},
        {"ffn_wino", &g_ffn_wino, 0, 2},
        {"ffn_fused", &g_ffn_fused, 0, 1},
        {"text_xres", &g_text_xres, 0, 15},
        {"attn_fused", &g_attn_fused, 0, 1},
        {"pred_xl", &g_pred_xl, 0, 1},
        {"pred_head", &g_pred_head, 0, 1},
        {"voc_pair", &g_voc_pair, 0, 2},
        {"voc_pair3", &g_voc_pair3, 0, 1},
        {"voc_pairw", &g_voc_pairw, 0, 1},
        {"voc_pair128", &g_voc_pair128, 0, 1},
        {"voc_rb16", &g_voc_rb16, 0, 2},
        {"voc_xl", &g_voc_xl, 0, 1},
        {"voc_wino64_k", &g_voc_wino64_k, 3, 99},
        {"voc_wino43", &g_voc_wino43, 0, 3},
        {"voc_qpair", &g_voc_qpair, 0, 2},
        {"voc_wino64", &g_voc_wino64, 0, 1},
        {"voc_wino", &g_voc_wino, 0, 2},
        {"voc_xl16", &g_voc_xl16, 0, 1},
        {"voc_upsT", &g_voc_upsT, 0, 1},
        {"post_v4", &g_post_v4, 0, 1},
        {"pred_wino", &g_pred_wino, 0, 1},
        {"energy_head", &g_energy_head, 0, 1},
        {"stats_mlp", &g_stats_mlp, 0, 1},
        {"text_xt16", &g_conv_xt16, 0, 1},
    };
    if (!strcmp(name, "voc_xl_split")) return cmtts_xl_set_split(value);
    if (!strcmp(name, "attn_qb")) return cmtts_attention_set_qb(value);
    if (!strcmp(name, "xres_nt")) return cmtts_xres_set_nt(value);
    bool found;
    const int prev = knob_set(tab, sizeof(tab) / sizeof(tab[0]), name, value, &found);
    if (found) return prev;
    return fail(CMTTS_E_INVALID, "cmtts_internal_set: unknown switch");
}

int cmtts_internal_cond_projections(cmtts_model* m, const float* cond_ct, int B, int T, float* cp, void* stream) {
    if (!m || !cond_ct || !cp || B <= 0 || T <= 0) return fail(CMTTS_E_INVALID, "cmtts_internal_cond_projections: bad argument");
    DenWs w;
    memset(&w, 0, sizeof(w));
    w.cp = cp;
    return cond_projections(m, w, cond_ct, B, T, (hipStream_t)stream);
}

int cmtts_internal_cond_factored(cmtts_model* m, const float* p1, int p1_ld, int L, const int64_t* mel2ph, const int64_t* p_idx, int B, int T,
                                 float* cp, void* stream) {
    if (!m || !m->finalized || !p1 || !mel2ph || !p_idx || !cp) return fail(CMTTS_E_INVALID, "cmtts_internal_cond_factored: bad argument");
    if (!m->cond_p2) return fail(CMTTS_E_UNSUPPORTED, "no pitch-table factor for this model");
    DenWs w;
    memset(&w, 0, sizeof(w));
    w.cp = cp;
    CondFactors cf;
    cf.p1 = p1; cf.ldp = p1_ld; cf.L = L; cf.mel2ph = mel2ph; cf.p_idx = p_idx;
    return cond_factored(m, w, cf, B, T, (hipStream_t)stream);
}

int cmtts_poll_error(void) { return check_device_flag(); }

int cmtts_set_persistent_denoiser(int mode) {
    const int prev = g_persist;
    if (mode >= 0 && mode <= 2) g_persist = mode;
    return prev;
}

int cmtts_set_fused_resblock(int on) {
    const int prev = g_fused_resblock ? 1 : 0;
    g_fused_resblock = on != 0;
    return prev;
}

int cmtts_set_precision(cmtts_model* m, int mode) {
    if (!m || mode < 0 || mode > 3) return fail(CMTTS_E_INVALID, "cmtts_set_precision: mode 0 (fp32), 1 (bf16), 2 (fp16) or 3 (fp16x3)");
    m->precision = mode;
    return 0;
}

int cmtts_set_variance_controls(cmtts_model* m, const cmtts_variance_controls* vc) {
    if (!m) return fail(CMTTS_E_INVALID, "cmtts_set_variance_controls: null model");
    const cmtts_variance_controls off = {1.f, 1.f, nullptr, nullptr, nullptr, nullptr, nullptr, nullptr};
    if (!vc) { m->vc = off; return 0; }
    if (!(vc->p_control > 0.f) || !(vc->e_control == vc->e_control))
        return fail(CMTTS_E_INVALID, "cmtts_set_variance_controls: p_control must be > 0 (it also scales the uv logit)");
    if (vc->cwt_spec && (!vc->f0_mean || !vc->f0_std || (m->cfg.use_uv && !vc->uv)))
        return fail(CMTTS_E_INVALID, "cmtts_set_variance_controls: a pitch target needs cwt_spec, f0_mean, f0_std (and uv)");
    m->vc = *vc;
    return 0;
}

int cmtts_set_control_tables(cmtts_model* m, const cmtts_control_tables* t) {
    if (!m) return fail(CMTTS_E_INVALID, "cmtts_set_control_tables: null model");
    const cmtts_control_tables off = {nullptr, nullptr, nullptr, 0};
    if (!t) t = &off;
    if ((t->d || t->e || t->p) && t->ld <= 0)
        return fail(CMTTS_E_INVALID, "cmtts_set_control_tables: ld (the row pitch = L of the next text-side call) must be > 0");
    m->ct = *t;
    return 0;
}

int cmtts_vocoder_set_precision(cmtts_vocoder* v, int mode) {
    if (!v || mode < 0 || mode > 3) return fail(CMTTS_E_INVALID, "cmtts_vocoder_set_precision: mode 0 (fp32), 1 (bf16), 2 (fp16) or 3 (fp16x3)");
    v->precision = mode;
    return 0;
}

int cmtts_set_resblock_tile(int frames) {
    if (frames != 0 && frames != 32 && frames != 64) return fail(CMTTS_E_INVALID, "cmtts_set_resblock_tile: 0, 32 or 64");
    cmtts_resblock_set_tile(frames);
    return 0;
}

int cmtts_set_debug_stamps(void* dev_buf) {
    cmtts_resblock_set_debug((long long*)dev_buf);
    cmtts_persist_set_debug((long long*)dev_buf);
    cmtts_pair_set_debug((long long*)dev_buf);
    cmtts_xres_set_debug((long long*)dev_buf);
    {
        int M = 0, K = 0;
        const char* mk = getenv("CMTTS_CONV_DBG_MK");
        if (mk && sscanf(mk, "%d,%d", &M, &K) == 2) cmtts_conv_set_debug(dev_buf ? (long long*)dev_buf : nullptr, M, K);
        else cmtts_conv_set_debug(nullptr, 0, 0);
    }
    return 0;
}

int cmtts_profile_begin(int max_launches, int stride) {
    if (max_launches <= 0 || stride <= 0) return fail(CMTTS_E_INVALID, "cmtts_profile_begin: bad argument");
    g_prof.stride = stride;
    g_prof.seen = 0;
    for (hipEvent_t e : g_prof.ev) (void)hipEventDestroy(e);
    g_prof.ev.assign((size_t)max_launches * 2, nullptr);
    for (auto& e : g_prof.ev) HIPCHK(hipEventCreate(&e));
    g_prof.used = 0;
    g_prof.on = true;
    return 0;
}
int cmtts_profile_end(double* total_ms, int* n_launches) {
    if (!total_ms || !n_launches) return fail(CMTTS_E_INVALID, "cmtts_profile_end: bad argument");
    g_prof.on = false;
    double tot = 0.0;
    for (size_t i = 0; i + 1 < g_prof.used; i += 2) {
        HIPCHK(hipEventSynchronize(g_prof.ev[i + 1]));
        float ms = 0.f;
        HIPCHK(hipEventElapsedTime(&ms, g_prof.ev[i], g_prof.ev[i + 1]));
        tot += ms;
    }
    *total_ms = tot;
    *n_launches = (int)(g_prof.used / 2);
    for (hipEvent_t e : g_prof.ev) (void)hipEventDestroy(e);
    g_prof.ev.clear();
    g_prof.used = 0;
    return 0;
}

int cmtts_wav_to_int16(const float* wav, int16_t* pcm, int64_t n, float max_wav_value, void* stream) {
    if (!wav || !pcm || n < 0) return fail(CMTTS_E_INVALID, "cmtts_wav_to_int16: bad argument");
    if (n) k_wav_to_int16(wav, pcm, (long)n, max_wav_value, (hipStream_t)stream);
    HIPCHK(hipGetLastError());
    return 0;
}

size_t cmtts_decoder_workspace_bytes(const cmtts_model* m, int B, int T) { return carve_text(m->cfg, B, T, nullptr).bytes; }

int cmtts_decoder_forward(cmtts_model* m, const float* x_ct, const int64_t* lens, int B, int T, float* out_ct, void* ws,
                          size_t ws_bytes, void* stream) {
    if (!m || !m->finalized) return fail(CMTTS_E_INVALID, "model not finalized");
    if (m->dec.empty()) return fail(CMTTS_E_INVALID, "cmtts_decoder_forward: the state dict held no decoder.* tensors");
    if (!x_ct || !lens || !out_ct || !ws || B <= 0 || T <= 0) return fail(CMTTS_E_INVALID, "cmtts_decoder_forward: bad argument");
    if (T + 1 >= PE_ROWS) return fail(CMTTS_E_UNSUPPORTED, "cmtts_decoder_forward: T exceeds the position table");
    const cmtts_config& c = m->cfg;
    TextWs w = carve_text(c, B, T, ws);
    if (ws_bytes < w.bytes) return fail(CMTTS_E_WORKSPACE, "decoder workspace too small");
    hipStream_t s = (hipStream_t)stream;
    const int H = c.hidden, Tp = round_up(T, 4);
    k_copy_rows(w.f, Tp, x_ct, T, T, (long)B * H, s);
    k_pos_embed_add(w.f, w.x, m->dec_alpha, m->omega_h, m->pe_h, PE_ROWS, B, H, T, Tp, s, lens);
    CHK(fft_stack(m, m->dec, w, lens, B, T, s));
    k_layernorm_ct(w.x, w.x, m->decln_g, m->decln_b, 1e-5f, lens, B, T, Tp, s);
    k_copy_rows(out_ct, T, w.x, Tp, T, (long)B * H, s);
    HIPCHK(hipGetLastError());
    return 0;
}

int cmtts_length_mask(const int64_t* lens, uint8_t* mask, int B, int W, void* stream) {
    if (!lens || !mask || B <= 0 || W < 0) return fail(CMTTS_E_INVALID, "cmtts_length_mask: bad argument");
    if (W == 0) return 0;
    k_length_mask(lens, mask, B, W, (hipStream_t)stream);
    HIPCHK(hipGetLastError());
// ... 43 lines not shown
```

cm-tts_amd/csrc/cond_gemm.h:

```cpp
#pragma once

struct CondGemmArgs {
    const float* X;
    const float* Wf;
    const float* bias;
    float* Y;
    int B, T, M, K;
    int force;
    int flat;
    int row_split;
};

#ifdef __cplusplus
extern "C" {
#endif
int cmtts_launch_cond_gemm(const CondGemmArgs* a, void* stream);
int cmtts_launch_cond_expand(const float* p1, int ldp, int L, const float* p2, int ld2, const int64_t* mel2ph, const int64_t* pidx,
                             float* cp, int B, int M, int T, void* stream);
int cmtts_launch_cond_gemm16(const CondGemmArgs* a, const void* wf16, int mode, void* stream);
#ifdef __cplusplus
}
#endif
```

cm-tts_amd/csrc/cond_gemm.hip:

```cpp
#include <hip/hip_runtime.h>
#include "cond_gemm.h"

typedef float f32x16 __attribute__((ext_vector_type(16)));
typedef float f32x4 __attribute__((ext_vector_type(4)));

namespace {

constexpr int K = 256;
constexpr int NW = 8;
constexpr int MT = 2;
constexpr int FN = 64;
constexpr int NT = FN / 32;
constexpr int X_LD = FN + 4;
constexpr int RING = 4;
constexpr int NG = K / 8;

__device__ __forceinline__ float ldg(const float* base, unsigned idx) {
    return *reinterpret_cast<const float*>(reinterpret_cast<const char*>(base) + (size_t)(idx * 4u));
}
__device__ __forceinline__ int acc_row(int r, int lane) { return (r & 3) + 8 * (r >> 2) + 4 * (lane >> 5); }

__global__ __launch_bounds__(64 * NW, 2) void cond_gemm_kernel(const CondGemmArgs a) {
    extern __shared__ __attribute__((aligned(16))) float xs[];
    const int tid = threadIdx.x, lane = tid & 63, w = tid >> 6;
    const int t0 = blockIdx.x * FN;
    const int l31 = lane & 31, khalf = lane >> 5;
    const int T = a.T;
    const long ncol = a.flat ? (long)a.B * T : T;
    auto col_x = [&](long c) -> long { return a.flat ? (c / T) * (long)K * T + (c % T) : (long)blockIdx.y * K * T + c; };
    auto col_y = [&](long c) -> long { return a.flat ? (c / T) * (long)a.M * T + (c % T) : (long)blockIdx.y * a.M * T + c; };
    const float* xin = a.X;
    float* yb = a.Y;

    {
        const long t = t0 + lane;
        const long xo = col_x(t < ncol ? t : ncol - 1);
#pragma unroll 1
        for (int i = 0; i < K / NW; i += 8) {
            float xv[8];
#pragma unroll
            for (int q = 0; q < 8; ++q) xv[q] = xin[xo + (long)(w * (K / NW) + i + q) * T];
#pragma unroll
            for (int q = 0; q < 8; ++q) xs[(w * (K / NW) + i + q) * X_LD + lane] = t < ncol ? xv[q] : 0.f;
        }
    }
    const int MTn = a.M / 32;
    auto load_a = [&](f32x4 (&dst)[MT], int mt0, int g) {
#pragma unroll
        for (int i = 0; i < MT; ++i)
            dst[i] = *reinterpret_cast<const f32x4*>(a.Wf + (((long)g * MTn + mt0 + i) * 64 + lane) * 4);
    };
    auto load_b = [&](float (&dst)[4][NT], int g) {
        const float* bs = xs + (g * 8 + khalf) * X_LD + l31;
#pragma unroll
        for (int kk = 0; kk < 4; ++kk)
#pragma unroll
            for (int j = 0; j < NT; ++j) dst[kk][j] = bs[2 * kk * X_LD + j * 32];
    };
    const int npass_all = a.M / (32 * MT * NW);
    const int ppg = (npass_all + (int)gridDim.z - 1) / (int)gridDim.z;
    const int p_first = (int)blockIdx.z * ppg;
    const int npass = min(npass_all, p_first + ppg);
    if (p_first >= npass) return;
    f32x4 A[RING][MT];
#pragma unroll
    for (int s = 0; s < RING - 1; ++s) load_a(A[s], (p_first * NW + w) * MT, s);
    __syncthreads();

    for (int p = p_first; p < npass; ++p) {
        const int mt0 = (p * NW + w) * MT;
        f32x16 acc[MT][NT];
#pragma unroll
        for (int i = 0; i < MT; ++i)
#pragma unroll
            for (int j = 0; j < NT; ++j)
#pragma unroll
                for (int r = 0; r < 16; ++r) acc[i][j][r] = 0.f;
        float Bv[2][4][NT];
        load_b(Bv[0], 0);
        const int mt_next = (min(p + 1, npass - 1) * NW + w) * MT;
#pragma unroll 1
        for (int it = 0; it < NG; it += RING) {
#pragma unroll
            for (int s = 0; s < RING; ++s) {
                const int nx = it + s + RING - 1;
                if (nx < NG) load_a(A[(s + RING - 1) % RING], mt0, nx);
                else load_a(A[(s + RING - 1) % RING], mt_next, nx - NG);
                load_b(Bv[(s + 1) & 1], min(it + s + 1, NG - 1));
                __builtin_amdgcn_sched_barrier(0);
#pragma unroll
                for (int kk = 0; kk < 4; ++kk)
#pragma unroll
                    for (int i = 0; i < MT; ++i)
#pragma unroll
                        for (int j = 0; j < NT; ++j)
                            acc[i][j] = __builtin_amdgcn_mfma_f32_32x32x2f32(A[s][i][kk], Bv[s & 1][kk][j], acc[i][j], 0, 0, 0);
                __builtin_amdgcn_sched_barrier(0);
            }
        }
#pragma unroll
        for (int i = 0; i < MT; ++i) {
            const int m0 = (mt0 + i) * 32;
            float bi[16];
#pragma unroll
            for (int r = 0; r < 16; ++r) bi[r] = ldg(a.bias, (unsigned)(m0 + acc_row(r, lane)));
#pragma unroll
            for (int j = 0; j < NT; ++j) {
                const long t = t0 + j * 32 + l31;
                const long yo = col_y(t < ncol ? t : ncol - 1);
#pragma unroll
                for (int r = 0; r < 16; ++r)
                    if (t < ncol) yb[yo + (long)(m0 + acc_row(r, lane)) * T] = acc[i][j][r] + bi[r];
            }
        }
    }
}

}

extern "C" int cmtts_launch_cond_gemm(const CondGemmArgs* ap, void* stream_) {
    const CondGemmArgs& a = *ap;
    if (a.K != K || a.M % (32 * MT * NW) != 0 || (long)a.M * a.T >= (1L << 30) || a.B <= 0 || a.T <= 0) return -2;
    if (a.flat && (long)a.B * a.T >= (1L << 30)) return -2;
    if (!a.force && (long)((a.T + FN - 1) / FN) * a.B < 128) return -2;
    static bool attr_set = false;
    const size_t lds = (size_t)K * X_LD * sizeof(float);
    if (!attr_set) {
        if (hipFuncSetAttribute(reinterpret_cast<const void*>(cond_gemm_kernel), hipFuncAttributeMaxDynamicSharedMemorySize,
                                (int)lds) != hipSuccess)
            return -3;
        attr_set = true;
    }
    const int zsplit = a.row_split > 1 ? a.row_split : 1;
    const dim3 grid = a.flat ? dim3((unsigned)(((long)a.B * a.T + FN - 1) / FN), 1, zsplit) : dim3((a.T + FN - 1) / FN, a.B, zsplit);
    hipLaunchKernelGGL(cond_gemm_kernel, grid, dim3(64 * NW), lds, (hipStream_t)stream_, a);
    return hipGetLastError() == hipSuccess ? 0 : -3;
}

namespace {
constexpr int CEX_ROWS = 64;
template <int V>
__global__ __launch_bounds__(256) void cond_expand_kernel(const float* __restrict__ p1, int ldp, int L, const float* __restrict__ p2, int ld2,
                                                          const int64_t* __restrict__ mel2ph, const int64_t* __restrict__ pidx,
                                                          float* __restrict__ cp, int M, int T) {
    const int t = (blockIdx.x * 64 + (threadIdx.x & 63)) * V;
    const int r0 = blockIdx.y * CEX_ROWS + (threadIdx.x >> 6) * (CEX_ROWS / 4), b = blockIdx.z;
    if (t >= T) return;
    int ph[V], ix[V];
#pragma unroll
    for (int e = 0; e < V; ++e) {
        const int64_t p64 = mel2ph[(long)b * T + t + e];
        ph[e] = (int)(p64 > L ? L : p64);
        const int i = (int)pidx[(long)b * T + t + e];
        ix[e] = i < 0 ? 0 : (i >= ld2 ? ld2 - 1 : i);
    }
    const float* a = p1 + ((long)b * M + r0) * ldp;
    const float* q = p2 + (long)r0 * ld2;
    float* o = cp + ((long)b * M + r0) * T + t;
#pragma unroll 1
    for (int r = 0; r < CEX_ROWS / 4; r += 4) {
        float av[4][V], qv[4][V];
#pragma unroll
        for (int j = 0; j < 4; ++j)
#pragma unroll
            for (int e = 0; e < V; ++e) {
                av[j][e] = a[(long)(r + j) * ldp + (ph[e] > 0 ? ph[e] - 1 : 0)];
                qv[j][e] = q[(long)(r + j) * ld2 + ix[e]];
            }
#pragma unroll
        for (int j = 0; j < 4; ++j) {
            if (V == 4) {
                f32x4 v;
#pragma unroll
                for (int e = 0; e < 4; ++e) v[e] = (ph[e] > 0 ? av[j][e] : 0.f) + qv[j][e];
                *reinterpret_cast<f32x4*>(o + (long)(r + j) * T) = v;
            } else {
                o[(long)(r + j) * T] = (ph[0] > 0 ? av[j][0] : 0.f) + qv[j][0];
            }
        }
    }
}
}

extern "C" int cmtts_launch_cond_expand(const float* p1, int ldp, int L, const float* p2, int ld2, const int64_t* mel2ph, const int64_t* pidx,
                                        float* cp, int B, int M, int T, void* stream_) {
    if (M % CEX_ROWS != 0 || B <= 0 || T <= 0 || L <= 0) return -2;
    if ((T & 3) == 0 && ((uintptr_t)cp & 15) == 0)
        hipLaunchKernelGGL(cond_expand_kernel<4>, dim3((T / 4 + 63) / 64, M / CEX_ROWS, B), dim3(256), 0, (hipStream_t)stream_, p1, ldp, L, p2, ld2,
                           mel2ph, pidx, cp, M, T);
    else
        hipLaunchKernelGGL(cond_expand_kernel<1>, dim3((T + 63) / 64, M / CEX_ROWS, B), dim3(256), 0, (hipStream_t)stream_, p1, ldp, L, p2, ld2,
                           mel2ph, pidx, cp, M, T);
    return hipGetLastError() == hipSuccess ? 0 : -3;
}
```

cm-tts_amd/csrc/conv_k5q.hip:

```cpp
#include <hip/hip_runtime.h>
#include <stdint.h>
#include "resblock_pair.h"
#include "xcd_map.h"
#ifndef XCD_MAP
#define XCD_MAP 1
#endif

namespace {

typedef float f32x4 __attribute__((ext_vector_type(4)));
typedef float f32x2 __attribute__((ext_vector_type(2)));

constexpr int CO = 256;
constexpr int KT = 5, PAD = 2;
constexpr int BN = 64;
constexpr int XIN = BN + KT;
constexpr int XW = 72;
constexpr int NPT = 12;
constexpr int NV = XW / 4;
constexpr int R = 4;
constexpr int U = 2;

template <int CIN, bool LN>
__global__ __launch_bounds__(256, 2) void conv_k5q_kernel(const ConvXlArgs a) {
    constexpr int NKS = CIN / 4;
    static_assert(NKS % U == 0, "k-steps per round");
    extern __shared__ __attribute__((aligned(16))) float Xs[];
    const int tid = threadIdx.x, lane = tid & 63, nthr = blockDim.x;
    const int wl = __builtin_amdgcn_readfirstlane(tid >> 6), nwv = nthr >> 6;
    const int w = blockIdx.z * nwv + wl;
    int bx_ = blockIdx.x, by_ = blockIdx.y;
    if (XCD_MAP) xcd_tile(bx_, by_);
    const int b = by_;
    const int t0 = bx_ * BN;
    const int T = a.T;
    const float* xb = a.x + (long)b * (a.cin ? a.xbstride : a.bstride);
    float* gs = Xs + CIN * XW;
    if (LN) {
        for (int i = tid; i < 256; i += nthr) { gs[i] = a.ln_g[i]; gs[256 + i] = a.ln_b[i]; }
    }
    {
        const int tbase = t0 - PAD;
        constexpr int total = CIN * NV;
#pragma unroll 1
        for (int base = tid; base < total; base += nthr * NV) {
            f32x4 v[NV];
#pragma unroll
            for (int u = 0; u < NV; ++u) {
                const int idx = min(base + u * nthr, total - 1), r = idx / NV, q = idx - r * NV;
                const int t = tbase + 4 * q;
                const float* src = xb + (long)r * a.ld;
                if (t >= 0 && t + 3 < T) v[u] = *reinterpret_cast<const f32x4*>(src + t);
                else {
#pragma unroll
                    for (int c = 0; c < 4; ++c) v[u][c] = src[min(max(t + c, 0), T - 1)];
                }
            }
#pragma unroll
            for (int u = 0; u < NV; ++u) {
                const int idx = base + u * nthr;
                if (idx < total) {
                    const int r = idx / NV, q = idx - r * NV;
                    const int t = tbase + 4 * q;
                    f32x4 o;
#pragma unroll
                    for (int c = 0; c < 4; ++c) o[c] = (4 * q + c < XIN && t + c >= 0 && t + c < T) ? v[u][c] : 0.f;
                    *reinterpret_cast<f32x4*>(Xs + r * XW + 4 * q) = o;
                }
            }
        }
    }
    __syncthreads();
    if constexpr (LN) {
        static_assert(!LN || CIN == 256, "LayerNorm prologue: 256 channels");
        const int l31 = lane & 31, khalf = lane >> 5;
        for (int cb = 32 * wl; cb < XW; cb += 32 * nwv) {
            const int c = cb + l31;
            const int t = t0 - PAD + c;
            const bool live = c < XIN && t >= 0 && t < T;
            const float* cr = Xs + min(c, XW - 1) + 4 * khalf * XW;
            float p[4] = {0.f, 0.f, 0.f, 0.f}, q[4];
#pragma unroll 8
            for (int i2 = 0; i2 < 32; ++i2)
#pragma unroll
                for (int y = 0; y < 4; ++y) p[y] += cr[(y + 8 * i2) * XW];
#pragma unroll
            for (int y = 0; y < 4; ++y) q[y] = __shfl_xor(p[y], 32);
            float tot = 0.f;
#pragma unroll
            for (int y = 0; y < 4; ++y) tot += khalf ? q[y] : p[y];
#pragma unroll
            for (int y = 0; y < 4; ++y) tot += khalf ? p[y] : q[y];
            const float mean = tot / 256.0f;
#pragma unroll
            for (int y = 0; y < 4; ++y) p[y] = 0.f;
#pragma unroll 8
            for (int i2 = 0; i2 < 32; ++i2)
#pragma unroll
                for (int y = 0; y < 4; ++y) { const float d = cr[(y + 8 * i2) * XW] - mean; p[y] = __fmaf_rn(d, d, p[y]); }
#pragma unroll
            for (int y = 0; y < 4; ++y) q[y] = __shfl_xor(p[y], 32);
            float var = 0.f;
#pragma unroll
            for (int y = 0; y < 4; ++y) var += khalf ? q[y] : p[y];
#pragma unroll
            for (int y = 0; y < 4; ++y) var += khalf ? p[y] : q[y];
            var = var / 256.0f;
            const float rstd = 1.0f / sqrtf(var + a.ln_eps);
            if (live) {
                float* wc = Xs + c + 4 * khalf * XW;
                const float* g = gs + 4 * khalf;
                const float* be = gs + 256 + 4 * khalf;
#pragma unroll 1
                for (int i0 = 0; i0 < 32; i0 += 4) {
                    float xv[16], gv[16], bv[16];
#pragma unroll
                    for (int e = 0; e < 16; ++e) {
                        const int k = (e & 3) + 8 * (i0 + (e >> 2));
                        xv[e] = wc[k * XW]; gv[e] = g[k]; bv[e] = be[k];
                    }
#pragma unroll
                    for (int e = 0; e < 16; ++e) {
                        const int k = (e & 3) + 8 * (i0 + (e >> 2));
                        wc[k * XW] = __fmaf_rn((xv[e] - mean) * rstd, gv[e], bv[e]);
                    }
                }
            }
        }
        __syncthreads();
    }

    f32x4 M[4][6];
#pragma unroll
    for (int i = 0; i < 4; ++i)
#pragma unroll
        for (int p = 0; p < 6; ++p) M[i][p] = f32x4{0.f, 0.f, 0.f, 0.f};
    {
        constexpr int NWVT = CO / 64;
        const __amdgpu_buffer_rsrc_t rs = __builtin_amdgcn_make_buffer_rsrc(const_cast<float*>(a.wf), 0, NKS * NWVT * NPT * 1024, 0x00020000);
        const int voff = lane * 16;
        f32x4 A[R][6];
        auto load_a = [&](f32x4 (&dst)[6], int ks0, int n) {
            const int soff = ((min(ks0 + n / 2, NKS - 1) * NWVT + w) * NPT + 6 * (n % 2)) * 1024;
#pragma unroll
            for (int p = 0; p < 6; ++p) dst[p] = __builtin_bit_cast(f32x4, __builtin_amdgcn_raw_buffer_load_b128(rs, voff + p * 1024, soff, 0));
        };
        const float* xl = Xs + (lane >> 4) * XW + 4 * (lane & 15);
        float D[2][6];
        auto load_d = [&](float (&d)[6], int ks0, int n) {
            const float* r = xl + min(ks0 + n / 2, NKS - 1) * (4 * XW);
            if (n % 2 == 0) {
                const f32x4 p = *reinterpret_cast<const f32x4*>(r);
                const f32x2 q = *reinterpret_cast<const f32x2*>(r + 4);
                d[0] = p[0]; d[1] = p[1]; d[2] = p[2]; d[3] = p[3]; d[4] = q.x; d[5] = q.y;
            } else {
                const f32x4 p = *reinterpret_cast<const f32x4*>(r + 4);
                d[0] = r[3]; d[1] = p[0]; d[2] = p[1]; d[3] = p[2]; d[4] = p[3]; d[5] = r[8];
            }
        };
#pragma unroll
        for (int s = 0; s < R - 1; ++s) load_a(A[s], 0, s);
        load_d(D[0], 0, 0);
#pragma unroll 1
        for (int ks0 = 0; ks0 < NKS; ks0 += U) {
#pragma unroll
            for (int n = 0; n < U * 2; ++n) {
                const int slot = n % R;
                float V[6];
                {
                    const float (&d)[6] = D[n & 1];
                    const f32x2 P01 = {d[0], d[1]}, P23 = {d[2], d[3]}, P45 = {d[4], d[5]};
                    const f32x2 c4 = {4.f, 4.f}, cm5 = {-5.f, -5.f}, c2 = {2.f, -2.f};
                    const f32x2 V05 = __builtin_elementwise_fma(c4, P01, __builtin_elementwise_fma(cm5, P23, P45));
                    const float u0 = __builtin_fmaf(-4.f, d[2], d[4]), u1 = __builtin_fmaf(-4.f, d[1], d[3]);
                    const float u2 = d[4] - d[2], u3 = d[3] - d[1];
                    const f32x2 a0 = {u0, u0}, a1 = {u1, -u1}, b0 = {u2, u2}, b1 = {u3, u3};
                    const f32x2 V12 = a0 + a1;
                    const f32x2 V34 = __builtin_elementwise_fma(c2, b1, b0);
                    V[0] = V05.x; V[1] = V12.x; V[2] = V12.y; V[3] = V34.x; V[4] = V34.y; V[5] = V05.y;
                }
                __builtin_amdgcn_sched_barrier(0);
                load_a(A[(slot + R - 1) % R], ks0, n + R - 1);
                load_d(D[(n + 1) & 1], ks0, n + 1);
#pragma unroll
                for (int p = 0; p < 6; ++p)
#pragma unroll
                    for (int i = 0; i < 4; ++i) M[i][p] = __builtin_amdgcn_mfma_f32_16x16x4f32(A[slot][p][i], V[p], M[i][p], 0, 0, 0);
                __builtin_amdgcn_sched_barrier(0);
            }
        }
    }

    float* yb = a.y + (long)b * a.bstride;
    const int q4 = lane & 15, rq = lane >> 4;
    const int tq = t0 + 4 * q4;
    const bool vec = ((a.ld & 3) == 0) && ((reinterpret_cast<size_t>(yb) & 15) == 0) && tq + 3 < T;
#pragma unroll
    for (int i = 0; i < 4; ++i) {
        float bi[4];
#pragma unroll
        for (int r = 0; r < 4; ++r) bi[r] = a.bias[w * 64 + 16 * i + 4 * rq + r];
#pragma unroll
        for (int r = 0; r < 4; ++r) {
            const int row = w * 64 + 16 * i + 4 * rq + r;
            const float m0 = M[i][0][r], m1 = M[i][1][r], m2 = M[i][2][r], m3 = M[i][3][r], m4 = M[i][4][r], m5 = M[i][5][r];
            const float s12 = m1 + m2, d12 = m1 - m2, s34 = m3 + m4, d34 = m3 - m4;
            f32x4 y;
            y[0] = ((m0 + s12) + s34) + bi[r];
            y[1] = __builtin_fmaf(2.f, d34, d12) + bi[r];
            y[2] = __builtin_fmaf(4.f, s34, s12) + bi[r];
            y[3] = (__builtin_fmaf(8.f, d34, d12) + m5) + bi[r];
            if (a.relu) {
#pragma unroll
                for (int c = 0; c < 4; ++c) y[c] = y[c] > 0.f ? y[c] : 0.f;
            }
            const long o = (long)row * a.ld + tq;
            if (vec) *reinterpret_cast<f32x4*>(yb + o) = y;
            else {
#pragma unroll
                for (int c = 0; c < 4; ++c)
                    if (tq + c < T) yb[o + c] = y[c];
            }
        }
    }
}

template <int CIN, bool LN>
int launch_k5q(const ConvXlArgs& a, hipStream_t stream) {
    const size_t lds = ((size_t)CIN * XW + (LN ? 512 : 0)) * sizeof(float);
    static bool attr_set = false;
    if (!attr_set) {
        if (hipFuncSetAttribute(reinterpret_cast<const void*>(conv_k5q_kernel<CIN, LN>), hipFuncAttributeMaxDynamicSharedMemorySize, (int)lds) != hipSuccess) return -3;
        attr_set = true;
    }
    const long tiles = (long)((a.T + BN - 1) / BN) * a.B;
    const int split = a.row_split == 1 || a.row_split == 2 || a.row_split == 4 ? a.row_split : (tiles >= 128 ? 1 : tiles >= 64 ? 2 : 4);
    dim3 grid((a.T + BN - 1) / BN, a.B, split);
    hipLaunchKernelGGL((conv_k5q_kernel<CIN, LN>), grid, dim3(256 / split), lds, stream, a);
    return hipGetLastError() == hipSuccess ? 0 : -3;
}

}

extern "C" int cmtts_launch_conv_k5q(const ConvXlArgs* a, void* stream_) {
    hipStream_t s = (hipStream_t)stream_;
    if (a->C != CO || a->k != KT || a->dil != 1 || a->T < 1 || a->B < 1 || a->res || a->accum || a->slope != 1.0f || !a->wf || !a->bias) return -2;
    const int cin = a->cin ? a->cin : a->C;
    if (a->ln_g && (!a->ln_b || cin != 256)) return -2;
    if (cin == 256) return a->ln_g ? launch_k5q<256, true>(*a, s) : launch_k5q<256, false>(*a, s);
    if (cin == 128 && !a->ln_g) return launch_k5q<128, false>(*a, s);
    return -2;
}
```

cm-tts_amd/csrc/internal_hooks.h:

```cpp
#pragma once
#ifdef __cplusplus
extern "C" {
#endif
int cmtts_internal_set(const char* name, int value);
struct cmtts_model;
int cmtts_internal_cond_projections(struct cmtts_model* m, const float* cond_ct, int B, int T, float* cp, void* stream);
int cmtts_internal_cond_factored(struct cmtts_model* m, const float* p1, int p1_ld, int L, const int64_t* mel2ph, const int64_t* p_idx, int B, int T,
                                 float* cp, void* stream);
int cmtts_internal_mel_window_gather(const float* mel_ct, int B, int T, const int32_t* windows, int N, int Tw, float* out, void* stream);
int cmtts_internal_noise_bits(const int64_t* seeds, int B, int T, int M, int first_draw, int n_draws, int64_t t0, uint32_t* bits, void* stream);
#ifdef __cplusplus
}
#endif
```

cm-tts_amd/csrc/kernels.h:

```cpp
#pragma once
#include <hip/hip_runtime.h>
#include <stdint.h>

enum DenseAct { DENSE_NONE = 0, DENSE_RELU = 1, DENSE_MISH = 2 };

void k_embed_tokens(const int64_t* texts, const int64_t* lens, const float* E, const float* omega, const float* tab,
                    int tab_rows, float* x, int B, int L, int ld, int C, float scale, hipStream_t s);
void k_layernorm_ct(const float* in, float* out, const float* gamma, const float* beta, float eps,
                    const int64_t* lens, int B, int T, int ld, hipStream_t s);
void k_softmax_cols(float* st, const int64_t* lens, int nz, int H, int L, int ld, long zs, hipStream_t s);
void k_add_rowvec(float* x, const float* vec, int B, int C, int L, int ld, hipStream_t s,
                  const int64_t* lens = nullptr);
void k_pos_embed_add(const float* x, float* out, const float* alpha, const float* omega, const float* tab,
                     int tab_rows, int B, int C, int T, int ld, hipStream_t s,
                     const int64_t* lens = nullptr);
void k_pos_embed_add_lr(const float* src, int ldl, const int64_t* mel2ph, const float* padv, float* out, const float* alpha, const float* omega,
                        const float* tab, int tab_rows, int B, int C, int T, hipStream_t s);
void k_chan_linear(const float* x, const float* W, const float* bias, float* out, const int64_t* lens,
                   int B, int C, int T, int ld, int O, hipStream_t s);
bool k_stats_mlp(const float* in, long in_bs, long in_ks, const float* W0, const float* b0, const float* W1, const float* b1, const float* W2,
                 const float* b2, float* out, int B, int K0, int N0, int N1, int N2, hipStream_t s);
void k_dense_small(const float* in, long in_bs, long in_ks, const float* Wt, const float* bias,
                   const float* add, float* out, int B, int K, int N, int act, hipStream_t s);
void k_energy_embed(const float* x, const float* e_pred, float* e_scaled, const float* e_target, float e_control,
                    const float* bins, int nbins, const float* E, float* out1, int64_t* e_idx, int B, int C, int L, int ld,
                    hipStream_t s, const float* e_table = nullptr);
void k_durations(const float* logd, float d_control, float* d_rounded, int* cum, int64_t* mel_len,
                 int B, int L, hipStream_t s);
void k_durations_table(const float* logd, const float* dtab, float* d_rounded, int* cum, int64_t* mel_len,
                       int B, int L, hipStream_t s);
void k_durations_table_serial(const float* logd, const float* dtab, float* d_rounded, int* cum, int64_t* mel_len,
                              int B, int L, hipStream_t s);
void k_pitch_table_scale(float* cwt, const int64_t* mel2ph, const int* cum, const float* ptab, int B, int O, int L, int T, hipStream_t s);
void k_durations_serial(const float* logd, float d_control, float* d_rounded, int* cum, int64_t* mel_len,
                 int B, int L, hipStream_t s);
void k_broadcast_row(const float* row, float* out, int B, int n, hipStream_t s);
void k_add_rows(const float* a, const float* b, float* out, long n, hipStream_t s);
void k_reduce_partials(const float* part, int nseg, const float* bias, const float* res, const int64_t* lens, float* out, int B, int C,
                       int L, int ld, hipStream_t s);
void k_ln_linear_energy(const float* x, const float* gamma, const float* beta, float eps, const float* W, const float* bias, float* out,
                        const int64_t* ln_lens, const int64_t* out_lens, int B, int T, int ld, const float* xin, const float* e_target, float e_control,
                        const float* bins, int nbins, const float* E, float* out1, int64_t* e_idx, float* e_scaled, hipStream_t s,
                        const float* e_table = nullptr);
bool k_ln_linear(const float* x, const float* gamma, const float* beta, float eps, const float* W, const float* bias, float* out,
                 const int64_t* ln_lens, const int64_t* out_lens, int B, int T, int ld, int O, hipStream_t s);
void k_cumsum_durations(const float* dur, int* cum, int64_t* mel_len, int B, int L, hipStream_t s);
void k_mel2ph(const int* cum, int64_t* mel2ph, int B, int L, int T, hipStream_t s);
void k_length_regulate(const float* out1, const int64_t* mel2ph, float* xlr, int B, int C, int ldl,
                       int T, hipStream_t s, const float* padv = nullptr);
void k_pitch_index(const float* cwt, int O, const float* mean_p, const float* std_p, int stat_ld, float std_scale,
                   const float* uv_logit, int uv_ld, const uint8_t* uv_mask, float eps, float* r_ws, int64_t* p_idx,
                   float* f0_denorm, int B, int T, hipStream_t s);
void k_gather_add(const float* x, const int64_t* idx, const float* E, float* out, int B, int C, int T,
                  hipStream_t s);
void k_lr_gather_add(const float* out1, const int64_t* mel2ph, int ldl, const int64_t* idx, const float* E, float* out, int B, int C, int T,
                     hipStream_t s);
void k_mel_prep(const float* x, const float* scale_b, float scale, float* hin, int B, int T, int M, hipStream_t s);
void k_mel_post(const float* F, const float* xold, const float* noise, float c_out, float c_skip,
                float nstd, float* out, int B, int T, int M, unsigned* flag, hipStream_t s);
void k_diff_embed(const float* t, const float* omega, float* emb, int B, int C, hipStream_t s);
extern int g_post_v4;
void k_conv_post(const float* x, const float* w, const float* bias, float pre_div, float slope, float* wav, int B,
                 int C, int T, int ld, int KW, hipStream_t s);
void k_wav_to_int16(const float* wav, int16_t* pcm, long n, float max_wav, hipStream_t s);
void k_length_mask(const int64_t* lens, uint8_t* mask, int B, int W, hipStream_t s);
void k_transpose(const float* in, float* out, int B, int R, int Cn, hipStream_t s);
void k_fill_lens(int64_t* lens, int64_t v, int B, hipStream_t s);
void k_gather_rows(const float* table, const int64_t* idx, float* out, int B, int C, int n_rows, hipStream_t s);
void k_copy_rows(float* dst, int dst_ld, const float* src, int src_ld, int width, long rows, hipStream_t s);
void k_scale(const float* in, float* out, long n, float sc, hipStream_t s);
void k_fill_float(float* p, float v, int n, hipStream_t s);
```

cm-tts_amd/csrc/kernels.hip:

```cpp
#include <hip/hip_runtime.h>
#include <math.h>
#include <stdint.h>
#include "kernels.h"

namespace {

__device__ __forceinline__ float sin_exact(float a) { return (float)sin((double)a); }
__device__ __forceinline__ float cos_exact(float a) { return (float)cos((double)a); }

__device__ __forceinline__ float pos_embed(int p, int c, int C, const float* omega, const float* tab, int tab_rows) {
    if (p == 0) return 0.f;
    if (p < tab_rows) return tab[(long)p * C + c];
    const int half = C >> 1;
    const int j = c < half ? c : c - half;
    const float arg = (float)p * omega[j];
    return c < half ? sin_exact(arg) : cos_exact(arg);
}

template <typename FlagFn>
__device__ void block_positions(FlagFn flag, int T, int* pos, int* counts) {
    const int tid = threadIdx.x;
    const int seg = (T + 255) / 256;
    const int start = tid * seg;
    const int end = min(T, start + seg);
// ... 622 lines not shown
    if (t >= T) return;
    const long off = ((long)b * C + c) * T + t;
    out[off] = x[off] + E[idx[(long)b * T + t] * C + c];
}

__global__ void mel_prep_kernel(const float* x, const float* scale_b, float scale, float* hin, int T, int M) {
    const int t = blockIdx.x * blockDim.x + threadIdx.x;
    const int m = blockIdx.y, b = blockIdx.z;
    if (t >= T) return;
    const float s = scale_b ? scale_b[b] : scale;
    hin[((long)b * M + m) * T + t] = s * x[((long)b * T + t) * M + m];
}

__global__ void mel_post_kernel(const float* F, const float* xold, const float* noise, float c_out, float c_skip,
                                float nstd, float* out, int T, int M, unsigned* flag) {
    const int m = threadIdx.x;
    const int t = blockIdx.x * blockDim.y + threadIdx.y;
    const int b = blockIdx.y;
    if (t >= T || m >= M) return;
    const long o = ((long)b * T + t) * M + m;
    float v = c_out * F[((long)b * M + m) * T + t];
    if (xold) v += c_skip * xold[o];
    if (noise) v += noise[o] * nstd * 0.85f;
    out[o] = v;
    if (flag && !(fabsf(v) <= 3.402823466e38f) && *(volatile unsigned*)flag == 0u) *(volatile unsigned*)flag = 2u;
}

__global__ void diff_embed_kernel(const float* t, const float* omega, float* emb, int C) {
    const int c = threadIdx.x, b = blockIdx.x;
    if (c >= C) return;
    const int half = C >> 1;
    const int j = c < half ? c : c - half;
    const float arg = t[b] * omega[j];
    emb[(long)b * C + c] = c < half ? sin_exact(arg) : cos_exact(arg);
}

constexpr int POST_V = 4;
constexpr int POST_KW_MAX = 7;
__global__ __launch_bounds__(256) void conv_post_kernel(const float* __restrict__ x, const float* __restrict__ w, const float* __restrict__ bias,
                                                        float pre_div, float slope, float* __restrict__ wav, int C, int T, int ld, int KW) {
    extern __shared__ float wsh[];
    for (int i = threadIdx.x; i < C * KW; i += 256) wsh[i] = w[i];
    __syncthreads();
    const int t0 = (blockIdx.x * 256 + threadIdx.x) * POST_V;
    const int b = blockIdx.y;
    if (t0 >= T) return;
    const int pad = KW / 2;
    float acc[POST_V];
#pragma unroll
    for (int v = 0; v < POST_V; ++v) acc[v] = 0.f;
    for (int c = 0; c < C; ++c) {
        const float* xr = x + ((long)b * C + c) * ld;
        float xv[POST_V + POST_KW_MAX - 1];
#pragma unroll
        for (int q = 0; q < POST_V + POST_KW_MAX - 1; ++q) {
            const int tt = t0 + q - pad;
            float v = (q < POST_V + KW - 1 && tt >= 0 && tt < T) ? xr[tt] : 0.f;
            if (pre_div != 1.0f) v = v / pre_div;
            xv[q] = v > 0.f ? v : v * slope;
        }
#pragma unroll
        for (int k = 0; k < POST_KW_MAX; ++k) {
            if (k < KW) {
                const float wk = wsh[c * KW + k];
#pragma unroll
                for (int v = 0; v < POST_V; ++v) acc[v] = fmaf(wk, xv[v + k], acc[v]);
            }
        }
    }
    const float bs = bias[0];
#pragma unroll
    for (int v = 0; v < POST_V; ++v)
        if (t0 + v < T) wav[(long)b * T + t0 + v] = tanhf(acc[v] + bs);
}

__global__ __launch_bounds__(256) void conv_post_v4_kernel(const float* __restrict__ x, const float* __restrict__ w, const float* __restrict__ bias,
                                                           float pre_div, float slope, float* __restrict__ wav, int C, int T, int ld, int KW) {
    extern __shared__ float wsh[];
    for (int i = threadIdx.x; i < C * KW; i += 256) wsh[i] = w[i];
    __syncthreads();
    const int t0 = (blockIdx.x * 256 + threadIdx.x) * POST_V;
    const int b = blockIdx.y;
    if (t0 >= T) return;
    const int pad = KW / 2;
    float acc[POST_V];
#pragma unroll
    for (int v = 0; v < POST_V; ++v) acc[v] = 0.f;
    const int tl = max(t0 - 4, 0), tr = min(t0 + 4, ((T + 3) & ~3) - 4);
    constexpr int CU = 4;
    for (int c0 = 0; c0 < C; c0 += CU) {
        float4 Lq[CU], Mq[CU], Rq[CU];
#pragma unroll
        for (int u = 0; u < CU; ++u) {
            const float* xr = x + ((long)b * C + min(c0 + u, C - 1)) * ld;
            Lq[u] = *reinterpret_cast<const float4*>(xr + tl);
            Mq[u] = *reinterpret_cast<const float4*>(xr + t0);
            Rq[u] = *reinterpret_cast<const float4*>(xr + tr);
        }
#pragma unroll
        for (int u = 0; u < CU; ++u) {
            if (c0 + u >= C) break;
            const float raw[12] = {Lq[u].x, Lq[u].y, Lq[u].z, Lq[u].w, Mq[u].x, Mq[u].y, Mq[u].z, Mq[u].w, Rq[u].x, Rq[u].y, Rq[u].z, Rq[u].w};
            float xv[POST_V + POST_KW_MAX - 1];
#pragma unroll
            for (int q = 0; q < POST_V + POST_KW_MAX - 1; ++q) {
                const int tt = t0 + q - pad;
                const int ri = q - pad + 4;
                float v = (q < POST_V + KW - 1 && tt >= 0 && tt < T && ri >= 0 && ri < 12) ? raw[ri < 0 ? 0 : (ri > 11 ? 11 : ri)] : 0.f;
                if (pre_div != 1.0f) v = v / pre_div;
                xv[q] = v > 0.f ? v : v * slope;
            }
#pragma unroll
            for (int k = 0; k < POST_KW_MAX; ++k) {
                if (k < KW) {
                    const float wk = wsh[(c0 + u) * KW + k];
#pragma unroll
                    for (int v = 0; v < POST_V; ++v) acc[v] = fmaf(wk, xv[v + k], acc[v]);
                }
            }
        }
    }
    const float bs = bias[0];
#pragma unroll
    for (int v = 0; v < POST_V; ++v)
        if (t0 + v < T) wav[(long)b * T + t0 + v] = tanhf(acc[v] + bs);
}

__global__ void wav_to_int16_kernel(const float* wav, int16_t* pcm, long n, float max_wav) {
    const long i = (long)blockIdx.x * blockDim.x + threadIdx.x;
    if (i < n) pcm[i] = (int16_t)(int)(wav[i] * max_wav);
}

__global__ __launch_bounds__(256) void transpose_kernel(const float* in, float* out, int R, int Cn) {
    __shared__ float tile[32][33];
    const int b = blockIdx.z;
    const int r0 = blockIdx.y * 32, c0 = blockIdx.x * 32;
    const int tx = threadIdx.x & 31, ty = threadIdx.x >> 5;
    for (int i = ty; i < 32; i += 8) {
        const int r = r0 + i, c = c0 + tx;
        tile[i][tx] = (r < R && c < Cn) ? in[((long)b * R + r) * Cn + c] : 0.f;
    }
    __syncthreads();
    for (int i = ty; i < 32; i += 8) {
        const int c = c0 + i, r = r0 + tx;
        if (c < Cn && r < R) out[((long)b * Cn + c) * R + r] = tile[tx][i];
    }
}

__global__ void scale_kernel(const float* in, float* out, long n, float sc) {
    const long i = (long)blockIdx.x * blockDim.x + threadIdx.x;
    if (i < n) out[i] = in[i] * sc;
}

__global__ void pitch_table_scale_kernel(float* cwt, const int64_t* mel2ph, const int* cum, const float* ptab, int O, int L, int T) {
    const int i = blockIdx.x * blockDim.x + threadIdx.x;
    const int b = blockIdx.y;
    if (i >= T * O) return;
    int64_t ph = mel2ph[(long)b * T + i / O];
    if (ph <= 0) {
        const int ml = cum[(long)b * L + L - 1];
        ph = (ml > 0 && ml <= T) ? mel2ph[(long)b * T + ml - 1] : 1;
    }
    ph = ph < 1 ? 1 : (ph > L ? L : ph);
    const long off = (long)b * T * O + i;
    cwt[off] = cwt[off] * ptab[(long)b * L + (ph - 1)];
}

__global__ void fill_float_kernel(float* p, float v, int n) {
    const int i = blockIdx.x * blockDim.x + threadIdx.x;
    if (i < n) p[i] = v;
}

__global__ void fill_lens_kernel(int64_t* lens, int64_t v, int B) {
    const int i = blockIdx.x * blockDim.x + threadIdx.x;
    if (i < B) lens[i] = v;
}

inline int cdiv(long a, long b) { return (int)((a + b - 1) / b); }

}

void k_embed_tokens(const int64_t* texts, const int64_t* lens, const float* E, const float* omega, const float* tab,
                    int tab_rows, float* x, int B, int L, int ld, int C, float scale, hipStream_t s) {
    hipLaunchKernelGGL(embed_tokens_kernel, dim3(B, cdiv(C, EMB_CG)), dim3(256), (256 + L) * sizeof(int), s, texts, lens, E, omega,
                       tab, tab_rows, x, L, ld, C, scale);
}
void k_layernorm_ct(const float* in, float* out, const float* gamma, const float* beta, float eps,
                    const int64_t* lens, int B, int T, int ld, hipStream_t s) {
    hipLaunchKernelGGL(layernorm_ct_kernel, dim3(cdiv(T, 32), B), dim3(256), 0, s, in, out, gamma, beta, eps, lens, T, ld);
}
void k_softmax_cols(float* st, const int64_t* lens, int nz, int H, int L, int ld, long zs, hipStream_t s) {
    hipLaunchKernelGGL(softmax_cols_kernel, dim3(cdiv(L, 64), nz), dim3(256), 0, s, st, lens, H, L, ld, zs);
}
void k_add_rowvec(float* x, const float* vec, int B, int C, int L, int ld, hipStream_t s, const int64_t* lens) {
    hipLaunchKernelGGL(add_rowvec_kernel, dim3(cdiv(L, 64), C, B), dim3(64), 0, s, x, vec, C, L, ld, lens);
}
void k_pos_embed_add(const float* x, float* out, const float* alpha, const float* omega, const float* tab,
                     int tab_rows, int B, int C, int T, int ld, hipStream_t s, const int64_t* lens) {
    hipLaunchKernelGGL(pos_embed_add_kernel, dim3(B, cdiv(C, POS_CG)), dim3(256), (256 + T) * sizeof(int), s, x, out, alpha, omega, tab,
                       tab_rows, C, T, ld, lens);
}
void k_pos_embed_add_lr(const float* src, int ldl, const int64_t* mel2ph, const float* padv, float* out, const float* alpha, const float* omega,
                        const float* tab, int tab_rows, int B, int C, int T, hipStream_t s) {
    hipLaunchKernelGGL(pos_embed_add_lr_kernel, dim3(B, cdiv(C, POS_CG)), dim3(256), (256 + T) * sizeof(int), s, src, ldl, mel2ph, padv, out, alpha,
                       omega, tab, tab_rows, C, T);
}
void k_chan_linear(const float* x, const float* W, const float* bias, float* out, const int64_t* lens, int B,
                   int C, int T, int ld, int O, hipStream_t s) {
    hipLaunchKernelGGL(chan_linear_kernel, dim3(cdiv(T, 64), B), dim3(256), (size_t)(O * C + 3 * 16 * 64) * sizeof(float), s,
                       x, W, bias, out, lens, C, T, ld, O);
}
void k_dense_small(const float* in, long in_bs, long in_ks, const float* Wt, const float* bias, const float* add,
                   float* out, int B, int K, int N, int act, hipStream_t s) {
    if (K >= 512 && cdiv(N, 64) * cdiv(B, DB) < 128)
        hipLaunchKernelGGL(dense_small_kernel<16>, dim3(cdiv(N, 64), cdiv(B, DB)), dim3(1024), 0, s, in, in_bs, in_ks, Wt,
                           bias, add, out, B, K, N, act);
    else
        hipLaunchKernelGGL(dense_small_kernel<4>, dim3(cdiv(N, 64), cdiv(B, DB)), dim3(256), 0, s, in, in_bs, in_ks, Wt,
                           bias, add, out, B, K, N, act);
}
bool k_stats_mlp(const float* in, long in_bs, long in_ks, const float* W0, const float* b0, const float* W1, const float* b1, const float* W2,
                 const float* b2, float* out, int B, int K0, int N0, int N1, int N2, hipStream_t s) {
    const size_t lds = (size_t)(K0 + N0 + N1 + 3 * SM_COLS) * sizeof(float);
    if (lds > 48 * 1024) return false;
    hipLaunchKernelGGL(stats_mlp_kernel, dim3(B), dim3(4 * SM_COLS), lds, s, in, in_bs, in_ks, W0, b0, W1, b1, W2, b2, out, K0, N0, N1, N2);
    return true;
}
void k_energy_embed(const float* x, const float* e_pred, float* e_scaled, const float* e_target, float e_control,
                    const float* bins, int nbins, const float* E, float* out1, int64_t* e_idx, int B, int C, int L, int ld,
                    hipStream_t s, const float* e_table) {
    hipLaunchKernelGGL(energy_embed_kernel, dim3(cdiv(L, 64), B, cdiv(C, ENE_CG)), dim3(64), 0, s, x, e_pred, e_scaled, e_target,
                       e_control, bins, nbins, E, out1, e_idx, C, L, ld, e_table);
}
void k_durations(const float* logd, float d_control, float* d_rounded, int* cum, int64_t* mel_len, int B, int L,
                 hipStream_t s) {
    hipLaunchKernelGGL(durations_wave_kernel, dim3(B), dim3(64), 0, s, logd, d_control, d_rounded, cum, mel_len, L);
}
void k_durations_table(const float* logd, const float* dtab, float* d_rounded, int* cum, int64_t* mel_len, int B, int L,
                       hipStream_t s) {
    hipLaunchKernelGGL(durations_wave_table_kernel, dim3(B), dim3(64), 0, s, logd, dtab, d_rounded, cum, mel_len, L);
}
void k_durations_table_serial(const float* logd, const float* dtab, float* d_rounded, int* cum, int64_t* mel_len, int B, int L,
                              hipStream_t s) {
    hipLaunchKernelGGL(durations_table_kernel, dim3(cdiv(B, 64)), dim3(64), 0, s, logd, dtab, d_rounded, cum, mel_len, B, L);
}
void k_durations_serial(const float* logd, float d_control, float* d_rounded, int* cum, int64_t* mel_len, int B, int L,
                        hipStream_t s) {
    hipLaunchKernelGGL(durations_kernel, dim3(cdiv(B, 64)), dim3(64), 0, s, logd, d_control, d_rounded, cum, mel_len, B, L);
}
void k_broadcast_row(const float* row, float* out, int B, int n, hipStream_t s) {
    hipLaunchKernelGGL(broadcast_row_kernel, dim3(cdiv(n, 256), B), dim3(256), 0, s, row, out, n);
}
void k_add_rows(const float* a, const float* b, float* out, long n, hipStream_t s) {
    hipLaunchKernelGGL(add_rows_kernel, dim3((unsigned)((n + 255) / 256)), dim3(256), 0, s, a, b, out, n);
}
void k_reduce_partials(const float* part, int nseg, const float* bias, const float* res, const int64_t* lens, float* out, int B, int C,
                       int L, int ld, hipStream_t s) {
    hipLaunchKernelGGL(reduce_partials_kernel, dim3(cdiv(L, 64), cdiv(C, 4), B), dim3(256), 0, s, part, nseg, bias, res, lens, out, C, L, ld);
}
void k_ln_linear_energy(const float* x, const float* gamma, const float* beta, float eps, const float* W, const float* bias, float* out,
                        const int64_t* ln_lens, const int64_t* out_lens, int B, int T, int ld, const float* xin, const float* e_target, float e_control,
                        const float* bins, int nbins, const float* E, float* out1, int64_t* e_idx, float* e_scaled, hipStream_t s,
                        const float* e_table) {
    const EnergyEpi ee{xin, e_target, e_control, bins, nbins, E, out1, e_idx, e_scaled, e_table};
    if (e_table)
        hipLaunchKernelGGL((ln_linear_kernel<1, 2>), dim3(cdiv(T, 64), B), dim3(256), 0, s, x, gamma, beta, eps, W, bias, out, ln_lens, out_lens, T, ld, ee);
    else
        hipLaunchKernelGGL((ln_linear_kernel<1, 1>), dim3(cdiv(T, 64), B), dim3(256), 0, s, x, gamma, beta, eps, W, bias, out, ln_lens, out_lens, T, ld, ee);
}
bool k_ln_linear(const float* x, const float* gamma, const float* beta, float eps, const float* W, const float* bias, float* out,
                 const int64_t* ln_lens, const int64_t* out_lens, int B, int T, int ld, int O, hipStream_t s) {
    const dim3 grid(cdiv(T, 64), B), block(256);
    switch (O) {
        case 1: hipLaunchKernelGGL(ln_linear_kernel<1>, grid, block, 0, s, x, gamma, beta, eps, W, bias, out, ln_lens, out_lens, T, ld); return true;
        case 10: hipLaunchKernelGGL(ln_linear_kernel<10>, grid, block, 0, s, x, gamma, beta, eps, W, bias, out, ln_lens, out_lens, T, ld); return true;
        case 11: hipLaunchKernelGGL(ln_linear_kernel<11>, grid, block, 0, s, x, gamma, beta, eps, W, bias, out, ln_lens, out_lens, T, ld); return true;
        default: return false;
    }
}
void k_cumsum_durations(const float* dur, int* cum, int64_t* mel_len, int B, int L, hipStream_t s) {
    hipLaunchKernelGGL(cumsum_durations_kernel, dim3(cdiv(B, 64)), dim3(64), 0, s, dur, cum, mel_len, B, L);
}
void k_mel2ph(const int* cum, int64_t* mel2ph, int B, int L, int T, hipStream_t s) {
    hipLaunchKernelGGL(mel2ph_kernel, dim3(cdiv(T, 256), B), dim3(256), 0, s, cum, mel2ph, L, T);
}
void k_length_regulate(const float* out1, const int64_t* mel2ph, float* xlr, int B, int C, int ldl, int T,
                       hipStream_t s, const float* padv) {
    hipLaunchKernelGGL(length_regulate_kernel, dim3(cdiv(T, 256), C, B), dim3(256), 0, s, out1, mel2ph, xlr, C, ldl, T, padv);
}
void k_pitch_index(const float* cwt, int O, const float* mean_p, const float* std_p, int stat_ld, float std_scale,
                   const float* uv_logit, int uv_ld, const uint8_t* uv_mask, float eps, float* r_ws, int64_t* p_idx,
                   float* f0_denorm, int B, int T, hipStream_t s) {
    hipLaunchKernelGGL(pitch_index_kernel, dim3(B), dim3(256), 0, s, cwt, O, mean_p, std_p, stat_ld, std_scale, uv_logit,
                       uv_ld, uv_mask, eps, r_ws, p_idx, f0_denorm, T);
}
void k_gather_add(const float* x, const int64_t* idx, const float* E, float* out, int B, int C, int T, hipStream_t s) {
    hipLaunchKernelGGL(gather_add_kernel, dim3(cdiv(T, 256), C, B), dim3(256), 0, s, x, idx, E, out, C, T);
}
void k_lr_gather_add(const float* out1, const int64_t* mel2ph, int ldl, const int64_t* idx, const float* E, float* out, int B, int C, int T,
                     hipStream_t s) {
    hipLaunchKernelGGL(lr_gather_add_kernel, dim3(cdiv(T, 256), C, B), dim3(256), 0, s, out1, mel2ph, ldl, idx, E, out, C, T);
}
void k_mel_prep(const float* x, const float* scale_b, float scale, float* hin, int B, int T, int M, hipStream_t s) {
    hipLaunchKernelGGL(mel_prep_kernel, dim3(cdiv(T, 256), M, B), dim3(256), 0, s, x, scale_b, scale, hin, T, M);
}
void k_mel_post(const float* F, const float* xold, const float* noise, float c_out, float c_skip, float nstd,
                float* out, int B, int T, int M, unsigned* flag, hipStream_t s) {
    const int ty = 256 / M > 0 ? 256 / M : 1;
    hipLaunchKernelGGL(mel_post_kernel, dim3(cdiv(T, ty), B), dim3(M, ty), 0, s, F, xold, noise, c_out, c_skip, nstd,
                       out, T, M, flag);
}
void k_diff_embed(const float* t, const float* omega, float* emb, int B, int C, hipStream_t s) {
    hipLaunchKernelGGL(diff_embed_kernel, dim3(B), dim3(C), 0, s, t, omega, emb, C);
}
int g_post_v4 = 1;
void k_conv_post(const float* x, const float* w, const float* bias, float pre_div, float slope, float* wav, int B,
                 int C, int T, int ld, int KW, hipStream_t s) {
    if (g_post_v4 && KW <= POST_KW_MAX && KW / 2 <= 4 && (ld & 3) == 0 && ((uintptr_t)x & 15) == 0 && ld >= ((T + 3) & ~3) && T >= 4) {
        hipLaunchKernelGGL(conv_post_v4_kernel, dim3(cdiv(T, 256 * POST_V), B), dim3(256), (size_t)C * KW * sizeof(float), s, x, w,
                           bias, pre_div, slope, wav, C, T, ld, KW);
        return;
    }
    hipLaunchKernelGGL(conv_post_kernel, dim3(cdiv(T, 256 * POST_V), B), dim3(256), (size_t)C * KW * sizeof(float), s, x, w,
                       bias, pre_div, slope, wav, C, T, ld, KW);
}
void k_wav_to_int16(const float* wav, int16_t* pcm, long n, float max_wav, hipStream_t s) {
    hipLaunchKernelGGL(wav_to_int16_kernel, dim3(cdiv(n, 256)), dim3(256), 0, s, wav, pcm, n, max_wav);
}
__global__ void length_mask_kernel(const int64_t* __restrict__ lens, uint8_t* __restrict__ mask, int B, int W) {
    const long i = (long)blockIdx.x * 256 + threadIdx.x;
    if (i >= (long)B * W) return;
    const int b = (int)(i / W), t = (int)(i - (long)b * W);
    mask[i] = t >= lens[b] ? 1 : 0;
}
void k_length_mask(const int64_t* lens, uint8_t* mask, int B, int W, hipStream_t s) {
    hipLaunchKernelGGL(length_mask_kernel, dim3(cdiv((long)B * W, 256)), dim3(256), 0, s, lens, mask, B, W);
}
void k_transpose(const float* in, float* out, int B, int R, int Cn, hipStream_t s) {
    hipLaunchKernelGGL(transpose_kernel, dim3(cdiv(Cn, 32), cdiv(R, 32), B), dim3(256), 0, s, in, out, R, Cn);
}
__global__ void gather_rows_kernel(const float* __restrict__ table, const int64_t* __restrict__ idx, float* __restrict__ out, int C, int n_rows) {
    const int b = blockIdx.x;
    long r = idx[b];
    r = r < 0 ? 0 : (r >= n_rows ? n_rows - 1 : r);
    for (int c = threadIdx.x; c < C; c += blockDim.x) out[(long)b * C + c] = table[r * C + c];
}
void k_gather_rows(const float* table, const int64_t* idx, float* out, int B, int C, int n_rows, hipStream_t s) {
    hipLaunchKernelGGL(gather_rows_kernel, dim3(B), dim3(256), 0, s, table, idx, out, C, n_rows);
}
__global__ void copy_rows_kernel(float* __restrict__ dst, int dst_ld, const float* __restrict__ src, int src_ld, int width, long rows) {
    const int t = blockIdx.y * blockDim.x + threadIdx.x;
    const long r = (long)blockIdx.x * 4 + threadIdx.y;
    if (t < width && r < rows) dst[r * dst_ld + t] = src[r * src_ld + t];
}
void k_copy_rows(float* dst, int dst_ld, const float* src, int src_ld, int width, long rows, hipStream_t s) {
    hipLaunchKernelGGL(copy_rows_kernel, dim3(cdiv(rows, 4), cdiv(width, 64)), dim3(64, 4), 0, s, dst, dst_ld, src, src_ld, width, rows);
}
void k_scale(const float* in, float* out, long n, float sc, hipStream_t s) {
    hipLaunchKernelGGL(scale_kernel, dim3(cdiv(n, 256)), dim3(256), 0, s, in, out, n, sc);
}
void k_pitch_table_scale(float* cwt, const int64_t* mel2ph, const int* cum, const float* ptab, int B, int O, int L, int T, hipStream_t s) {
    hipLaunchKernelGGL(pitch_table_scale_kernel, dim3(cdiv(T * O, 256), B), dim3(256), 0, s, cwt, mel2ph, cum, ptab, O, L, T);
}
void k_fill_float(float* p, float v, int n, hipStream_t s) {
    hipLaunchKernelGGL(fill_float_kernel, dim3(cdiv(n, 64)), dim3(64), 0, s, p, v, n);
}
void k_fill_lens(int64_t* lens, int64_t v, int B, hipStream_t s) {
    hipLaunchKernelGGL(fill_lens_kernel, dim3(cdiv(B, 64)), dim3(64), 0, s, lens, v, B);
}
```

cm-tts_amd/csrc/resblock_pair.h:

```cpp
#pragma once

struct PairArgs {
    const float* x;
    float* y;
    const void* w1f;
    const float* b1;
    const void* w2f;
    const float* b2;
    long bstride;
    int B, C, T, ld;
    int k, dil;
    int accum;
    float slope;
    long long* dbg;
};

struct ConvXlArgs {
    const float* x;
    float* y;
    const float* wf;
    const float* bias;
    const float* res;
    long bstride;
    int B, C, T, ld;
    int k, dil;
    int accum;
    float slope;
    int relu;
    int cin;
    long xbstride;
    int wino_force;
    const float* ln_g;
    const float* ln_b;
    float ln_eps;
    int row_split;
};

struct WinoEntry { signed char acc, a, b, sgn, wkind, tau; };
#define WINO_F23(t) {0, t, (t) + 2, -1, 0, t}, {1, (t) + 1, (t) + 2, 1, 1, t}, {2, (t) + 2, (t) + 1, -1, 2, t}, {3, (t) + 1, (t) + 3, -1, 3, t}
#define WINO_F22(t) {0, t, (t) + 1, -1, 0, t}, {1, (t) + 1, 0, 0, 5, t}, {3, (t) + 1, (t) + 2, -1, 6, t}
#define WINO_ONE(t) {0, t, 0, 0, 0, t}, {3, (t) + 1, 0, 0, 4, t}
template <int KT> struct WinoTab;
template <> struct WinoTab<3> { static constexpr int N = 4; static constexpr WinoEntry e[N] = {WINO_F23(0)}; };
template <> struct WinoTab<7> { static constexpr int N = 10; static constexpr WinoEntry e[N] = {WINO_F23(0), WINO_F23(3), WINO_ONE(6)}; };
template <> struct WinoTab<11> { static constexpr int N = 15; static constexpr WinoEntry e[N] = {WINO_F23(0), WINO_F23(3), WINO_F23(6), WINO_F22(9)}; };

#ifdef __cplusplus
extern "C" {
#endif
int cmtts_launch_conv_xl(const ConvXlArgs* a, void* stream);
int cmtts_launch_conv_xlw(const ConvXlArgs* a, void* stream);
int cmtts_launch_conv_xlq(const ConvXlArgs* a, void* stream);
int cmtts_launch_conv_xlq_pair(const PairArgs* a, void* stream);
int cmtts_launch_conv_k5q(const ConvXlArgs* a, void* stream);
int cmtts_launch_convT(const float* x, float* y, const float* wf, const float* bias, long xbstride, long ybstride, int B, int cin,
                       int co, int Ti, int To, int ldx, int ldy, int s, float pre_div, float slope, void* stream);
int cmtts_launch_conv_xl16(const ConvXlArgs* a, int mode, int io, void* stream);
int cmtts_launch_resblock_pair(const PairArgs* a, void* stream);
int cmtts_launch_resblock_pair16(const PairArgs* a, int mode, void* stream);
int cmtts_launch_convT16(const float* x, float* y, const void* wf16, const float* bias, long xbstride, long ybstride, int B, int cin,
                         int co, int Ti, int To, int ldx, int ldy, int s, float pre_div, float slope, int mode, void* stream);
int cmtts_launch_resblock16(const float* x, float* y, const void* const* w1f, const void* const* w2f, const float* const* b1,
                            const float* const* b2, long bstride, int B, int C, int T, int ld, int k, int accum, float slope,
                            int mode, void* stream);
int cmtts_launch_resblock_pairw16(const PairArgs* a, int mode, void* stream);
int cmtts_launch_resblock_pair16x3(const PairArgs* a, void* stream);
int cmtts_launch_conv_xl16x3(const ConvXlArgs* a, void* stream);
void cmtts_pair_set_debug(long long* dbg);
int cmtts_xl_set_split(int on);
#ifdef __cplusplus
}
#endif
```

cm-tts_amd/host.py:

```python
import ctypes as C
import math

import numpy as np
import torch

from . import _lib
from . import noise as _noise
from .config import CMTTSConfig, HifiGanConfig


def _ptr(t):
    return C.c_void_p(0) if t is None else C.c_void_p(t.data_ptr())


def _stream():
    return C.c_void_p(torch.cuda.current_stream().cuda_stream)


def _f32(t, device):
    return t.to(device=device, dtype=torch.float32).contiguous()


def _i64(t, device):
    return t.to(device=device, dtype=torch.int64).contiguous()


def _resolve_controls(B, L, p_control=1.0, e_control=1.0, d_control=1.0):
    scal, tabs = [], {}
    for name, v in (("p", p_control), ("e", e_control), ("d", d_control)):
        if isinstance(v, np.ndarray):
            v = torch.from_numpy(v)
        if not isinstance(v, torch.Tensor):
            if isinstance(v, bool) or not isinstance(v, (int, float, np.floating, np.integer)):
                raise ValueError(f"{name}_control: a number, a [B] tensor or a [B, L] tensor, not {type(v).__name__}")
            scal.append(float(v))
            continue
        if v.dtype != torch.float32:
            raise ValueError(f"{name}_control: the table must be float32, not {v.dtype}")
        t = v.detach().to("cpu")
        if t.dim() == 1 and t.shape[0] == B:
            t = t[:, None].expand(B, L)
        elif t.dim() != 2 or tuple(t.shape) != (B, L):
            raise ValueError(f"{name}_control: shape {tuple(v.shape)}, expected [{B}] (per utterance) or [{B}, {L}] (per phoneme)")
        if bool(torch.isnan(t).any()):
            raise ValueError(f"{name}_control: NaN in the table")
        if name == "p" and not bool((t > 0).all()):
            raise ValueError("p_control: every factor must be > 0 (it also scales the uv logit)")
        if name == "d" and not bool((t >= 0).all()):
            raise ValueError("d_control: every factor must be >= 0")
        tabs[name] = t.contiguous()
        scal.append(1.0)
    return tuple(scal), tabs


def _check_no_scalar_with_table(scalars, p_control=None, e_control=None, d_control=None):
    for name, sc, v in zip("ped", scalars, (p_control, e_control, d_control)):
        if isinstance(v, (torch.Tensor, np.ndarray)) and not isinstance(sc, (torch.Tensor, np.ndarray)) and float(sc) != 1.0:
            raise ValueError(f"{name}_control: a table replaces the scalar control, which is {sc} here (it must be 1)")


class _InstalledTables:

    def __init__(self, model, tabs, L, lo=None, hi=None, present_only=()):
        self.model, self.keep = model, []
        ct = _lib.ControlTablesStruct(ld=int(L))
        for name, t in tabs.items():
            if name in present_only:
                t = t[:1]
            elif lo is not None:
                t = t[lo:hi]
            self.keep.append(t.to(device=model.device, dtype=torch.float32).contiguous())
            setattr(ct, name, _ptr(self.keep[-1]))
        self.active = bool(self.keep)
        if self.active:
            _lib.check(model.lib.cmtts_set_control_tables(model._h, C.byref(ct)))

    def clear(self):
        if self.active:
            self.model.lib.cmtts_set_control_tables(self.model._h, None)
            torch.cuda.current_stream(self.model.device).synchronize()
            self.active = False


def _push_state_dict(lib, setter, handle, sd):
    for name, v in sd.items():
        if isinstance(v, torch.Tensor):
            v = v.detach().cpu().numpy()
        a = np.ascontiguousarray(np.asarray(v, dtype=np.float32))
        if a.ndim == 0:
            a = a.reshape(1)
        shape = (C.c_int64 * a.ndim)(*a.shape)
        _lib.check(setter(handle, name.encode(), a.ctypes.data_as(C.c_void_p), shape, a.ndim))


_PG_NOTED = False


def _note_process_group(lib):
    global _PG_NOTED
    if not _PG_NOTED and torch.distributed.is_available() and torch.distributed.is_initialized():
        lib.cmtts_set_option(b"process_group", 1)
        _PG_NOTED = True


def _norm_device(device):
    device = torch.device(device)
    if device.type == "cuda" and device.index is None:
        device = torch.device("cuda", torch.cuda.current_device())
    return device


class _Workspace:

    def __init__(self):
        self._bufs = {}

    def get(self, key, nbytes, device):
        device = _norm_device(device)
        key = (key, torch.cuda.current_stream(device).cuda_stream)
        buf = self._bufs.get(key)
        if buf is None or buf.numel() < nbytes or buf.device != device:
            buf = torch.empty(int(nbytes), dtype=torch.uint8, device=device)
            self._bufs[key] = buf
        return buf


def get_mask_from_lengths(lengths, max_len=None):
    if max_len is None:
        max_len = int(lengths.max().item())
    if lengths.is_cuda and lengths.dtype == torch.int64:
        lengths = lengths.contiguous()
        mask = torch.empty(lengths.shape[0], int(max_len), dtype=torch.bool, device=lengths.device)
        with torch.cuda.device(lengths.device):
            _lib.check(_lib.load().cmtts_length_mask(_ptr(lengths), _ptr(mask), lengths.shape[0], int(max_len), _stream()))
        return mask
    ids = torch.arange(0, max_len, device=lengths.device).unsqueeze(0)
    return ids >= lengths.unsqueeze(1)


class CondFactors:
    __slots__ = ("p1", "p1t", "p1_ld", "L", "mel2ph", "p_idx", "_ptr", "_version", "_shape", "_aux")

    def __init__(self, p1, p1_ld, L, mel2ph, p_idx, cond_ct, p1t=None):
        self.p1, self.p1_ld, self.L, self.mel2ph, self.p_idx = p1, int(p1_ld), int(L), mel2ph, p_idx
        self.p1t = p1t
        self._ptr, self._version, self._shape = cond_ct.data_ptr(), cond_ct._version, tuple(cond_ct.shape)
        self._aux = (p1._version, mel2ph._version, p_idx._version, None if p1t is None else p1t._version)

    def matches(self, cond_ct):
        return (cond_ct.data_ptr() == self._ptr and cond_ct._version == self._version and tuple(cond_ct.shape) == self._shape and
                (self.p1._version, self.mel2ph._version, self.p_idx._version, None if self.p1t is None else self.p1t._version) == self._aux)


class CMTotalTTS(torch.nn.Module):

    def __init__(self, config: CMTTSConfig, device="cuda:0"):
        super().__init__()
        self.config = config
        self.device = _norm_device(device) if torch.cuda.is_available() else torch.device(device)
        self.lib = _lib.load()
        cs = _lib.CMTTSConfigStruct()
        for name, _ in cs._fields_:
            setattr(cs, name, type(getattr(cs, name))(getattr(config, name)))
        self._h = C.c_void_p()
        _lib.check(self.lib.cmtts_create(C.byref(cs), C.byref(self._h)))
        self._ready = False
        self._ws = _Workspace()
        self._cond_factors = True
        self.duration_pitch_energy_net = DurationPitchSpeakerNet(self)
        self.net = CMDenoiserTTS(self)
        self.decoder = FastspeechDecoder(self)

    def __del__(self):
        h = getattr(self, "_h", None)
        if h is not None and h.value and C is not None:
            self.lib.cmtts_destroy(h)
            self._h = None

    def load_state_dict(self, state_dict, strict=True):
        _push_state_dict(self.lib, self.lib.cmtts_set_tensor, self._h, state_dict)
        self._pending = True
        if self.device.type == "cuda" and torch.cuda.is_available():
            self._finalize()
        return self

    def _finalize(self):
        with torch.cuda.device(self.device):
            _lib.check(self.lib.cmtts_finalize(self._h))
        self._pending = False
        self._ready = True

    def eval(self):
        return self

    def set_precision(self, dtype="fp32"):
        mode = {"fp32": 0, "f32": 0, "bf16": 1, "fp16": 2, "f16": 2, "fp16x3": 3}[dtype]
        _lib.check(self.lib.cmtts_set_precision(self._h, mode))
        self._precision_mode = mode
        return self

    def set_option(self, name, value):
        prev = self.lib.cmtts_model_set_option(self._h, name.encode() if isinstance(name, str) else name, int(value))
        if prev < 0:
            _lib.check(prev)
        return prev

    def _require(self):
        _note_process_group(self.lib)
        if not self._ready and getattr(self, "_pending", False):
            if not torch.cuda.is_available():
                raise RuntimeError("CMTotalTTS: no GPU — cmtts_amd has no CPU fallback (the weights are loaded, the kernels cannot run)")
            self.device = _norm_device(self.device if self.device.type == "cuda" else "cuda")
            self._finalize()
        if not self._ready:
            raise RuntimeError("CMTotalTTS: load_state_dict() first")

    def to(self, *args, **kwargs):
        dev = kwargs.get("device", args[0] if args and isinstance(args[0], (str, torch.device, int)) else None)
        if dev is not None and self._ready and torch.cuda.is_available() and _norm_device(dev) != self.device:
            raise RuntimeError(f"CMTotalTTS was built on {self.device}; build another instance for {dev}")
        return self

    def get_segmentation_model(self):
        return self.duration_pitch_energy_net, self.net.forward

    def forward(self, x, timesteps, speakers=None, texts=None, src_lens=None, pitch=None, f0=None, uv=None, cwt_spec=None,
                f0_mean=None, f0_std=None, mel_lens=None, e_targets=None, d_targets=None, mel2phs=None, spker_embeds=None,
                p_control=1.0, e_control=1.0, d_control=1.0, **kwargs):
        p_targets = None if pitch is None else {"pitch": pitch, "f0": f0, "uv": uv, "cwt_spec": cwt_spec,
                                                "f0_mean": f0_mean, "f0_std": f0_std}
        out = self.duration_pitch_energy_net(speakers=speakers, texts=texts, src_lens=src_lens, mels=x, mel_lens=mel_lens,
                                             p_targets=p_targets, e_targets=e_targets, d_targets=d_targets, mel2phs=mel2phs,
                                             spker_embeds=spker_embeds, p_control=p_control, e_control=e_control,
                                             d_control=d_control)
        return self.net(x, timesteps, out["cond"], out["speaker_emb"], out["mel_masks"])


class DurationPitchSpeakerNet(torch.nn.Module):

    def __init__(self, owner: CMTotalTTS):
        super().__init__()
        self.__dict__["_owner"] = owner

    def forward(self, speakers=None, texts=None, src_lens=None, mels=None, mel_lens=None, p_targets=None,
                e_targets=None, d_targets=None, mel2phs=None, spker_embeds=None,
                p_control=1.0, e_control=1.0, d_control=1.0, max_mel_len=None, **kwargs):
        o = self._owner
        if texts is None:
            o._require()
        tshape = tuple(torch.as_tensor(texts).shape)
        if len(tshape) != 2:
            raise ValueError("texts must be [B, L]")
        (p_control, e_control, d_control), tabs = _resolve_controls(tshape[0], tshape[1], p_control, e_control, d_control)
        o._require()
        cfg, lib, dev = o.config, o.lib, o.device
        vc, keep = None, []
        if p_control != 1.0 or e_control != 1.0 or p_targets is not None or e_targets is not None or d_targets is not None:
            vc = _lib.VarianceControlsStruct(p_control=float(p_control), e_control=float(e_control))
            if d_targets is not None:
                keep.append(_f32(d_targets, dev)); vc.d_target = _ptr(keep[-1])
            if e_targets is not None:
                keep.append(_f32(e_targets, dev)); vc.e_target = _ptr(keep[-1])
            if p_targets is not None:
                for k in ("cwt_spec", "f0_mean", "f0_std"):
                    keep.append(_f32(p_targets[k], dev)); setattr(vc, k, _ptr(keep[-1]))
                keep.append(p_targets["uv"].to(device=dev, dtype=torch.uint8).contiguous()); vc.uv = _ptr(keep[-1])
                if mels is None and max_mel_len is None:
                    max_mel_len = int(p_targets["cwt_spec"].shape[1])
        texts = _i64(texts, dev)
        src_lens = _i64(src_lens, dev)
        B, L = texts.shape
        table = cfg.multi_speaker and cfg.n_speaker > 0
        spk_in = _f32(spker_embeds, dev) if (cfg.multi_speaker and not table and spker_embeds is not None) else None
        if cfg.multi_speaker and not table and spk_in is None:
            raise AssertionError("Speaker embedding should not be None")
        spk_ids = None
        if table:
            if speakers is None:
                raise AssertionError("speakers (ids into the speaker_emb table) should not be None")
            if speakers.numel() and (int(speakers.min()) < 0 or int(speakers.max()) >= cfg.n_speaker):
                raise IndexError("index out of range in self")
            spk_ids = _i64(speakers, dev)
        H = cfg.hidden
        with torch.cuda.device(dev):
            f = lambda *s: torch.empty(*s, dtype=torch.float32, device=dev)
            log_d, d_rounded, e_pred = f(B, L), f(B, L), f(B, L)
            mel_len = torch.empty(B, dtype=torch.int64, device=dev)
            e_idx = torch.empty(B, L, dtype=torch.int64, device=dev)
            enc_ct = f(B, H, L)
            spk = f(B, H) if cfg.multi_speaker else None
            nb = lib.cmtts_text_workspace_bytes(o._h, B, L)
            tws = o._ws.get("text", nb, dev)
            if vc is not None:
                _lib.check(lib.cmtts_set_variance_controls(o._h, C.byref(vc)))
            inst = None
            try:
                inst = _InstalledTables(o, tabs, L)
                _lib.check(lib.cmtts_text_forward(o._h, _ptr(texts), _ptr(src_lens), _ptr(spk_in), _ptr(spk_ids), B, L, float(d_control),
                                                  _ptr(log_d), _ptr(d_rounded), _ptr(mel_len), _ptr(e_pred), _ptr(e_idx),
                                                  _ptr(enc_ct), _ptr(spk), _ptr(tws), nb, _stream()))
                if mels is not None:
                    T = int(mels.size(2))
                elif max_mel_len is not None:
                    T = int(max_mel_len)
                else:
                    T = int(mel_len.max().item())
                O = cfg.cwt_out
                cond_ct = f(B, H, T)
                mel2ph = torch.empty(B, T, dtype=torch.int64, device=dev)
                cwt = f(B, T, O)
                f0 = f(B, T)
                p_idx = torch.empty(B, T, dtype=torch.int64, device=dev)
                stats = f(B, 2)
                nf = lib.cmtts_frame_workspace_bytes(o._h, B, T)
                fws = o._ws.get("frame", nf, dev)
                p1_ld = (L + 3) // 4 * 4
                p1 = f(B, cfg.res_layers * cfg.res_channels, p1_ld) if getattr(o, "_precision_mode", 0) == 0 and o._cond_factors else None
                p1t = None if p1 is None else f(B, cfg.res_layers, p1_ld, cfg.res_channels)
                _lib.check(lib.cmtts_frame_forward_sub_t(o._h, _ptr(tws), B, L, 0, B, T, _ptr(cond_ct), _ptr(mel2ph), _ptr(cwt),
                                                         _ptr(f0), _ptr(p_idx), _ptr(stats), _ptr(p1), _ptr(p1t), _ptr(fws), nf, _stream()))
            finally:
                if inst is not None:
                    inst.clear()
                if vc is not None:
                    lib.cmtts_set_variance_controls(o._h, None)
                    torch.cuda.current_stream(dev).synchronize()
        mel_masks = get_mask_from_lengths(mel_len, T)
        factors = None if p1 is None else CondFactors(p1, p1_ld, L, mel2ph, p_idx, cond_ct, p1t)
        cond_ct._cmtts_factors = factors
        return {
            "cond": cond_ct.transpose(1, 2),
            "cond_ct": cond_ct,
            "cond_factors": factors,
            "p_targets": p_targets,
            "p_predictions": {"pitch_pred": None, "f0_denorm": f0, "cwt": cwt,
                              "f0_mean": stats[:, 0], "f0_std": stats[:, 1], "p_idx": p_idx},
            "e_predictions": e_pred,
            "e_idx": e_idx,
            "log_d_predictions": log_d,
            "d_rounded": d_rounded,
            "mel_lens": mel_len,
            "mel_masks": mel_masks,
            "mel2ph": mel2ph,
            "src_masks": get_mask_from_lengths(src_lens, L),
            "speaker_emb": spk,
            "src_lens": src_lens,
            "enc_out": enc_ct.transpose(1, 2),
        }


def _as_cond_ct(conditioner, dev):
    c = conditioner.to(device=dev, dtype=torch.float32).transpose(1, 2)
    return c if c.is_contiguous() else c.contiguous()


class FastspeechDecoder(torch.nn.Module):

    def __init__(self, owner: CMTotalTTS):
        super().__init__()
        self.__dict__["_owner"] = owner

    def forward(self, x, padding_mask=None, attn_mask=None, return_hiddens=False):
        if attn_mask is not None or return_hiddens:
            raise NotImplementedError("FastspeechDecoder: attn_mask / return_hiddens are not used on the inference path")
        o = self._owner
        o._require()
        dev, lib = o.device, o.lib
        x = _f32(x, dev)
        B, T, H = x.shape
        if padding_mask is None:
            padding_mask = x.abs().sum(-1).eq(0)
        padding_mask = padding_mask.to(device=dev, dtype=torch.bool)
        lens = (~padding_mask).sum(1).to(torch.int64)
        if not torch.equal(padding_mask, get_mask_from_lengths(lens, T)):
            raise NotImplementedError("FastspeechDecoder: the padding mask must mark a suffix of every row (a length mask)")
        x_ct = transpose_last2(x)
        with torch.cuda.device(dev):
            out_ct = torch.empty(B, H, T, dtype=torch.float32, device=dev)
            nb = lib.cmtts_decoder_workspace_bytes(o._h, B, T)
            ws = o._ws.get("dec", nb, dev)
            _lib.check(lib.cmtts_decoder_forward(o._h, _ptr(x_ct), _ptr(lens), B, T, _ptr(out_ct), _ptr(ws), nb, _stream()))
        return transpose_last2(out_ct)


class CMDenoiserTTS(torch.nn.Module):

    def __init__(self, owner: CMTotalTTS):
        super().__init__()
        self.__dict__["_owner"] = owner

    def forward(self, x, timesteps, conditioner=None, speaker_emb=None, mask=None):
        o = self._owner
        o._require()
        dev, lib = o.device, o.lib
        x = _f32(x, dev)
        B, one, T, M = x.shape
        assert one == 1 and M == o.config.n_mels
        cond_ct = _as_cond_ct(conditioner, dev)
        t = _f32(timesteps, dev)
        spk = _f32(speaker_emb, dev) if speaker_emb is not None else None
        with torch.cuda.device(dev):
            out = torch.empty_like(x)
            nb = lib.cmtts_denoiser_workspace_bytes(o._h, B, T)
            ws = o._ws.get("den", nb, dev)
            _lib.check(lib.cmtts_denoiser_forward(o._h, _ptr(x), _ptr(t), _ptr(cond_ct), _ptr(spk), B, T, _ptr(out),
                                                  _ptr(ws), nb, _stream()))
        return out


class KarrasDenoiser:

    def __init__(self, sigma_data=0.5, sigma_max=80.0, sigma_min=0.002, rho=7.0, weight_schedule="karras",
                 distillation=False, loss_norm="lpips", **kw):
        self.sigma_data, self.sigma_max, self.sigma_min, self.rho = sigma_data, sigma_max, sigma_min, rho
        self.weight_schedule, self.distillation, self.loss_norm = weight_schedule, distillation, loss_norm

    def get_scalings(self, sigma):
        c_skip = self.sigma_data ** 2 / (sigma ** 2 + self.sigma_data ** 2)
        c_out = sigma * self.sigma_data / (sigma ** 2 + self.sigma_data ** 2) ** 0.5
        c_in = 1 / (sigma ** 2 + self.sigma_data ** 2) ** 0.5
        return c_skip, c_out, c_in

    def get_scalings_for_boundary_condition(self, sigma):
        c_skip = self.sigma_data ** 2 / ((sigma - self.sigma_min) ** 2 + self.sigma_data ** 2)
        c_out = (sigma - self.sigma_min) * self.sigma_data / (sigma ** 2 + self.sigma_data ** 2) ** 0.5
        c_in = 1 / (sigma ** 2 + self.sigma_data ** 2) ** 0.5
        return c_skip, c_out, c_in

    def denoise(self, model, x_t, sigmas, **model_kwargs):
        scal = self.get_scalings_for_boundary_condition if self.distillation else self.get_scalings
        c_skip, c_out, c_in = [v[(...,) + (None,) * (x_t.ndim - v.ndim)] for v in scal(sigmas)]
        rescaled_t = 1000 * 0.25 * torch.log(sigmas + 1e-44)
        model_output = model(c_in * x_t, rescaled_t, **model_kwargs)
        return model_output, c_out * model_output + c_skip * x_t


class DummyGenerator:

    def randn(self, *args, **kwargs):
        return torch.randn(*args, **kwargs)

    def randn_like(self, *args, **kwargs):
        return torch.randn_like(*args, **kwargs)


def _device_seeds(seeds, B, device):
    if isinstance(seeds, (int, np.integer)):
        seeds = _noise.utterance_seeds(int(seeds), np.arange(int(B)))
    if not isinstance(seeds, torch.Tensor):
        seeds = torch.from_numpy(np.ascontiguousarray(_noise._as_u64(seeds).view(np.int64)))
    if seeds.dtype != torch.int64 or tuple(seeds.shape) != (int(B),):
        raise ValueError(f"seeds: expected int64 [{int(B)}], got {seeds.dtype} {tuple(seeds.shape)}")
    return seeds.to(device=device).contiguous()


def seeded_noise(seeds, n_noise, T, n_mels=80, device="cuda:0", first_draw=0, t0=0):
    lib = _lib.load()
    dev = _norm_device(device)
    B = int(seeds.shape[0]) if hasattr(seeds, "shape") else len(seeds)
    sd = _device_seeds(seeds, B, dev)
    with torch.cuda.device(dev):
        out = torch.empty(int(n_noise), B, 1, int(T), int(n_mels), dtype=torch.float32, device=dev)
        _lib.check(lib.cmtts_noise_fill(_ptr(sd), B, int(T), int(n_mels), int(first_draw), int(n_noise), int(t0), _ptr(out), _stream()))
    return out


def seeded_noise_groups(groups, n_noise, n_mels=80, device="cuda:0", first_draw=0):
    lib = _lib.load()
    dev = _norm_device(device)
    arr = (_lib.NoiseGroupStruct * len(groups))()
    outs, keep = [], []
    with torch.cuda.device(dev):
        for g, (seeds, T) in zip(arr, groups):
            B = int(seeds.shape[0]) if hasattr(seeds, "shape") else len(seeds)
            sd = _device_seeds(seeds, B, dev)
            out = torch.empty(int(n_noise), B, 1, int(T), int(n_mels), dtype=torch.float32, device=dev)
            g.seeds, g.B, g.T, g.out = sd.data_ptr(), B, int(T), out.data_ptr()
            keep.append(sd)
            outs.append(out)
        if outs:
            _lib.check(lib.cmtts_noise_fill_groups(arr, len(outs), int(n_mels), int(first_draw), int(n_noise), _stream()))
    return outs


class IndivGenerator:

    def __init__(self, num_samples, seed=0, rank=None, world=None):
        if rank is None or world is None:
            import torch.distributed as dist
            on = dist.is_available() and dist.is_initialized()
            rank = (dist.get_rank() if on else 0) if rank is None else rank
            world = (dist.get_world_size() if on else 1) if world is None else world
        self.num_samples, self.seed, self.rank, self.world_size = int(num_samples), int(seed), int(rank), int(world)
        self.done_samples = 0
        self.draw = 0

    def get_size_and_indices(self, size):
# ... 1208 lines not shown
```

Before: 1.970 million.

## Merge small launches: sampler entry, length masks, p1t transpose, cwt positional staging

Folds several small kernel launches into fewer ones. The sampler's initial noise scale, timestep fill and cached step-row broadcast become a single kernel, and the two length masks come from one kernel. The cond GEMM writes the transposed p1t directly instead of running a separate transpose, and the cwt predictor's first conv gathers phoneme-level input plus positional embedding itself instead of materialising the length-regulated tensor. This targets launch overhead and one intermediate buffer pass in a small-batch hot path, at the cost of more special-case code paths and extra fallbacks.

Result: no change. 1.972 million, median of 3 (+0.1%).

```diff
diff --git a/cm-tts_amd/_lib.py b/cm-tts_amd/_lib.py
--- a/cm-tts_amd/_lib.py
+++ b/cm-tts_amd/_lib.py
@@ -253,6 +253,18 @@
     return _noise_bits(seeds, int(B), int(T), int(M), int(first_draw), int(n_draws), int(t0), bits, stream)
 
 
+_length_masks = None
+
+
+def internal_length_masks(lens_a, mask_a, Ba, Wa, lens_b, mask_b, Bb, Wb, stream):
+    global _length_masks
+    load()
+    if _length_masks is None:
+        _length_masks = C.CDLL(LIB_PATH).cmtts_internal_length_masks
+        _length_masks.restype, _length_masks.argtypes = _i, [_vp, _vp, _i, _i, _vp, _vp, _i, _i, _vp]
+    return _length_masks(lens_a, mask_a, int(Ba), int(Wa), lens_b, mask_b, int(Bb), int(Wb), stream)
+
+
 def backend():
     return "cffi" if isinstance(load(), _CffiLib) else "ctypes"
 
diff --git a/cm-tts_amd/csrc/cmtts_api.hip b/cm-tts_amd/csrc/cmtts_api.hip
--- a/cm-tts_amd/csrc/cmtts_api.hip
+++ b/cm-tts_amd/csrc/cmtts_api.hip
@@ -1142,9 +1142,16 @@
 int g_energy_head = 1;
 int g_pred_wino = 1;
 int g_pred_xres = 1;
+int g_cwt_pos_staged = 1;
+bool predictor_stages_ph(const Predictor& P, int T, int mode16) {
+    if (!g_cwt_pos_staged || mode16 || !g_pred_wino || P.convs.empty() || P.convs_q.empty() || !P.convs_q[0]) return false;
+    const PackedConv& w = P.convs[0];
+    return w.taps == 5 && w.cout == 256 && w.cin == 128 && T < PE_ROWS;
+}
 int predictor(const Predictor& P, const float* in, int ld_in, int B, int T, int ld, const int64_t* ln_lens,
               const int64_t* out_lens, float* bufA, float* bufB, float* out, int O, hipStream_t s, int mode16 = 0, bool frame_level = false,
-              EnergyHead* eh = nullptr) {
+              EnergyHead* eh = nullptr, const ConvK5qPh* ph = nullptr) {
+    if (ph && !(frame_level && !ln_lens && predictor_stages_ph(P, T, mode16))) return fail(CMTTS_E_INVALID, "predictor: phoneme-level staging is not available for this conv");
     const float* cur = in;
     int ldc = ld_in;
     auto other = [&](const float* p) { return p == bufA ? bufB : bufA; };
@@ -1161,7 +1168,12 @@
             xa.B = B; xa.C = 256; xa.T = T; xa.ld = ld; xa.k = w.taps; xa.dil = 1; xa.slope = 1.0f; xa.relu = 1;
             if (w.cin != 256) { xa.cin = w.cin; xa.xbstride = (long)w.cin * ldc; }
             if (pend_ln >= 0) { xa.ln_g = P.ln_g[pend_ln]; xa.ln_b = P.ln_b[pend_ln]; xa.ln_eps = 1e-12f; }
-            if (ldc == ld || w.cin != 256) {
+            if (ph && li == 0) {
+                xa.x = nullptr;
+                rx = cmtts_launch_conv_k5q_ph(&xa, ph, (void*)s);
+                if (rx == -2) return fail(CMTTS_E_UNSUPPORTED, "conv_k5q (phoneme-level staging) declined the launch");
+                if (rx == -3) return fail(CMTTS_E_HIP, "conv_k5q launch failed");
+            } else if (ldc == ld || w.cin != 256) {
                 rx = cmtts_launch_conv_k5q(&xa, (void*)s);
                 if (rx == -3) return fail(CMTTS_E_HIP, "conv_k5q launch failed");
                 if (rx == 0) pend_ln = -2;
@@ -1231,6 +1243,7 @@
     const cmtts_config& c = m->cfg;
     if (g_cond_gemm16 && m->precision >= 1 && m->precision <= 3 && m->cond_all_f16[m->precision - 1]) {
         CondGemmArgs g;
+        memset(&g, 0, sizeof(g));
         g.X = cond_ct; g.Wf = nullptr; g.bias = m->cond_all.bias; g.Y = w.cp;
         g.row_split = 0;
         g.B = B; g.T = T; g.M = c.res_layers * c.res_channels; g.K = c.hidden; g.force = 1;
@@ -1240,6 +1253,7 @@
     }
     if (m->cond_all_f) {
         CondGemmArgs g;
+        memset(&g, 0, sizeof(g));
         g.X = cond_ct; g.Wf = m->cond_all_f; g.bias = m->cond_all.bias; g.Y = w.cp;
         g.row_split = 0;
         g.B = B; g.T = T; g.M = c.res_layers * c.res_channels; g.K = c.hidden; g.force = g_cond_gemm == 2;
@@ -1270,7 +1284,9 @@
     const int r = cmtts_launch_cond_expand(f.p1, f.ldp, f.L, m->cond_p2, c.pitch_bins, f.mel2ph, f.p_idx, w.cp, B, c.res_layers * c.res_channels, T, (void*)s);
     return r == 0 ? 0 : fail(CMTTS_E_HIP, "cond_expand launch failed");
 }
-int cond_phoneme_factor(cmtts_model* m, const float* out1, int B, int Lp, float* p1, hipStream_t s) {
+int g_masks_merged = 1;
+int g_cond_p1t_gemm = 1;
+int cond_phoneme_factor(cmtts_model* m, const float* out1, int B, int Lp, float* p1, hipStream_t s, float* p1t = nullptr, bool* p1t_done = nullptr) {
     const cmtts_config& c = m->cfg;
     if (!m->cond_p2) return fail(CMTTS_E_UNSUPPORTED, "factored conditioner projections are not available for this model");
     CondGemmArgs g;
@@ -1289,12 +1305,18 @@
         if (t < best_t - 1e-9) { best_t = t; best = sp; }
     }
     g.row_split = best;
+    if (p1t_done) *p1t_done = false;
+    if (p1t && p1t_done && g_cond_p1t_gemm) {
+        g.Yt = p1t; g.C = c.res_channels;
+        if (cmtts_cond_gemm_takes_yt(&g)) *p1t_done = true;
+        else g.Yt = nullptr;
+    }
     const int r = cmtts_launch_cond_gemm(&g, (void*)s);
     return r == 0 ? 0 : fail(r == -2 ? CMTTS_E_UNSUPPORTED : CMTTS_E_HIP, "cond_gemm (phoneme factor) launch failed");
 }
 
 int step_embedding(cmtts_model* m, const DenWs& w, const float* timesteps, const float* spk, int B, hipStream_t s,
-                   float t_host = NAN) {
+                   float t_host = NAN, bool row_done = false) {
     const cmtts_config& c = m->cfg;
     const int C = c.res_channels, NL = c.res_layers;
     if (c.multi_speaker && !spk) return fail(CMTTS_E_INVALID, "speaker_emb is required for a multi-speaker model");
@@ -1302,7 +1324,7 @@
     if (cacheable) {
         for (const cmtts_model::StepRow& e : m->step_rows)
             if (e.t == t_host && hipEventQuery(e.ready) == hipSuccess) {
-                k_broadcast_row(e.row, w.dproj, B, NL * C, s);
+                if (!row_done) k_broadcast_row(e.row, w.dproj, B, NL * C, s);
                 if (c.multi_speaker) {
                     k_dense_small(spk, c.hidden, 1, m->sproj_wt, nullptr, nullptr, w.sproj, B, c.hidden, NL * C, DENSE_NONE, s);
                     k_add_rows(w.dproj, w.sproj, w.dp, (long)B * NL * C, s);
@@ -1310,6 +1332,7 @@
                 return 0;
             }
     }
+    if (row_done) return fail(CMTTS_E_INVALID, "step_embedding: the cached row the caller broadcast is gone");
     k_diff_embed(timesteps, m->omega_res, w.emb, B, C, s);
     k_dense_small(w.emb, C, 1, m->mlp0_wt, nullptr, nullptr, w.e1, B, C, 4 * C, DENSE_MISH, s);
     k_dense_small(w.e1, 4 * C, 1, m->mlp2_wt, nullptr, nullptr, w.e2, B, 4 * C, C, DENSE_NONE, s);
@@ -1337,6 +1360,14 @@
     }
     return 0;
 }
+
+const float* step_row_ready(const cmtts_model* m, float t_host) {
+    if (!g_step_cache || t_host != t_host) return nullptr;
+    for (const cmtts_model::StepRow& e : m->step_rows)
+        if (e.t == t_host && hipEventQuery(e.ready) == hipSuccess) return e.row;
+    return nullptr;
+}
+int g_entry_merged = 1;
 
 struct MelPost {
     const float* xold;
@@ -1878,18 +1909,23 @@
     if (ss) CHK(branch_fork(ss));
     if (cond_p1t && !cond_p1) return fail(CMTTS_E_INVALID, "cmtts_frame_forward_sub_t: cond_p1t needs cond_p1");
     if (cond_p1 && m->cond_p2) {
-        CHK(cond_phoneme_factor(m, tw.out1, B, Lp, cond_p1, sst));
-        if (cond_p1t) k_transpose(cond_p1, cond_p1t, B * c.res_layers, c.res_channels, Lp, sst);
+        bool p1t_done = false;
+        CHK(cond_phoneme_factor(m, tw.out1, B, Lp, cond_p1, sst, cond_p1t, &p1t_done));
+        if (cond_p1t && !p1t_done) k_transpose(cond_p1, cond_p1t, B * c.res_layers, c.res_channels, Lp, sst);
     }
     if (!(g_stats_mlp && k_stats_mlp(tw.out1, (long)H * Lp, Lp, m->st0_wt, m->st0_b, m->st2_wt, m->st2_b, m->st4_wt, m->st4_b, f0_stats, B, H, CH, CH, 2, sst))) {
         k_dense_small(tw.out1, (long)H * Lp, Lp, m->st0_wt, m->st0_b, nullptr, w.s1, B, H, CH, DENSE_RELU, sst);
         k_dense_small(w.s1, CH, 1, m->st2_wt, m->st2_b, nullptr, w.s2, B, CH, CH, DENSE_RELU, sst);
         k_dense_small(w.s2, CH, 1, m->st4_wt, m->st4_b, nullptr, f0_stats, B, CH, 2, DENSE_NONE, sst);
     }
-    k_mel2ph(tw.cum, mel2ph, B, L, T, s);
+    const int pmode16 = (m->text16 && (m->precision == 1 || m->precision == 2)) ? m->precision : 0;
+    const bool ph_staged = g_cwt_in_phoneme && predictor_stages_ph(m->cwt, T, pmode16);
+    if (ph_staged) k_mel2ph_pos(tw.cum, mel2ph, tw.h128, (long)CH * Lp, m->cwt_in.bias, reinterpret_cast<int*>(w.hp), B, L, T, s);
+    else k_mel2ph(tw.cum, mel2ph, B, L, T, s);
     if (!g_cwt_in_phoneme) k_length_regulate(tw.out1, mel2ph, w.xlr, B, H, Lp, T, s);
     bool hp_done = false;
-    if (g_cwt_in_phoneme) {
+    if (ph_staged) hp_done = true;
+    else if (g_cwt_in_phoneme) {
         k_pos_embed_add_lr(tw.h128, Lp, mel2ph, m->cwt_in.bias, w.hp, m->cwt.alpha, m->omega_cwt, m->pe_cwt, PE_ROWS, B, CH, T, s);
         hp_done = true;
     } else {
@@ -1897,7 +1933,11 @@
         CHK(launch(a, EPI_PLAIN, B, s));
     }
     if (!hp_done) k_pos_embed_add(w.h128, w.hp, m->cwt.alpha, m->omega_cwt, m->pe_cwt, PE_ROWS, B, CH, T, T, s);
-    CHK(predictor(m->cwt, w.hp, T, B, T, T, nullptr, nullptr, w.c1, w.c2, cwt_out, O, s, (m->text16 && (m->precision == 1 || m->precision == 2)) ? m->precision : 0, true));
+    ConvK5qPh phs;
+    memset(&phs, 0, sizeof(phs));
+    phs.src = tw.h128; phs.pad = m->cwt_in.bias; phs.mel2ph = (const long long*)mel2ph; phs.pos = reinterpret_cast<const int*>(w.hp);
+    phs.alpha = m->cwt.alpha; phs.pe_tab = m->pe_cwt; phs.ld = Lp; phs.pe_rows = PE_ROWS;
+    CHK(predictor(m->cwt, ph_staged ? nullptr : w.hp, T, B, T, T, nullptr, nullptr, w.c1, w.c2, cwt_out, O, s, pmode16, true, nullptr, ph_staged ? &phs : nullptr));
     if (ss) CHK(branch_join(ss));
     if (m->ct.p) k_pitch_table_scale(cwt_out, mel2ph, tw.cum, tw.pctl, B, O, L, T, s);
     else if (m->vc.p_control != 1.0f) k_scale(cwt_out, cwt_out, (long)B * T * O, m->vc.p_control, s);
@@ -2050,6 +2090,14 @@
     const cmtts_config& c = m->cfg;
     const long nel = (long)B * T * c.n_mels;
     SideStream* ss = g_fused_resblock ? side_for(s) : nullptr;
+    bool entry_done = false, row_done = false;
+    if (g_entry_merged && !seeds) {
+        const float t0_resc = 250.0f * logf(sigmas[0] + 1e-44f);
+        const float* row = ss ? step_row_ready(m, t0_resc) : nullptr;
+        k_sampler_entry(noise, w.xcur, nel, c.sigma_max, w.tbuf, t0_resc, B, row, w.dproj, c.res_layers * c.res_channels, s);
+        entry_done = true;
+        row_done = row != nullptr;
+    }
     if (ss) CHK(branch_fork(ss));
     const CondFactors* cfk = nullptr;
     CondFactors cf_local;
@@ -2077,7 +2125,7 @@
         if (cmtts_launch_noise_fill(seeds, B, T, c.n_mels, 0, 1, 0, c.sigma_max, w.xcur, nullptr, (void*)s) != 0 ||
             (n_re && cmtts_launch_noise_fill(seeds, B, T, c.n_mels, 1, n_re, 0, 1.0f, const_cast<float*>(noise), nullptr, (void*)(ss ? ss->side : s)) != 0))
             return fail(CMTTS_E_HIP, "seeded noise launch failed");
-    } else
+    } else if (!entry_done)
         k_scale(noise, w.xcur, nel, c.sigma_max, s);
     const float smin = c.sigma_min, sd2 = c.sigma_data * c.sigma_data;
     for (int i = 0; i < n_steps; ++i) {
@@ -2090,8 +2138,8 @@
         const float t_resc = 250.0f * logf(sg + 1e-44f);
         const bool new_sigma = i == 0 || sigmas[i] != sigmas[i - 1];
         const bool embed_side = i == 0 && ss != nullptr;
-        if (new_sigma) k_fill_float(w.tbuf, t_resc, B, embed_side ? ss->side : s);
-        if (embed_side) CHK(step_embedding(m, w, w.tbuf, speaker_emb, B, ss->side, t_resc));
+        if (new_sigma && !(i == 0 && entry_done)) k_fill_float(w.tbuf, t_resc, B, embed_side ? ss->side : s);
+        if (embed_side) CHK(step_embedding(m, w, w.tbuf, speaker_emb, B, ss->side, t_resc, row_done));
         const bool last = i + 1 == n_steps;
         const bool renoise = renoise_std[i] >= 0.0f;
         const MelPost post = {w.xcur, renoise ? renoise0 + (long)i * noise_stride : nullptr, c_out, c_skip,
@@ -3080,6 +3128,10 @@
         {"pred_wino", &g_pred_wino, 0, 1},
         {"energy_head", &g_energy_head, 0, 1},
         {"stats_mlp", &g_stats_mlp, 0, 1},
+        {"entry_merged", &g_entry_merged, 0, 1},
+        {"masks_merged", &g_masks_merged, 0, 1},
+        {"cwt_pos_staged", &g_cwt_pos_staged, 0, 1},
+        {"cond_p1t_gemm", &g_cond_p1t_gemm, 0, 1},
         {"text_xt16", &g_conv_xt16, 0, 1},
     };
     if (!strcmp(name, "voc_xl_split")) return cmtts_xl_set_split(value);
@@ -3089,6 +3141,18 @@
     const int prev = knob_set(tab, sizeof(tab) / sizeof(tab[0]), name, value, &found);
     if (found) return prev;
     return fail(CMTTS_E_INVALID, "cmtts_internal_set: unknown switch");
+}
+
+int cmtts_internal_length_masks(const int64_t* lens_a, uint8_t* mask_a, int Ba, int Wa, const int64_t* lens_b, uint8_t* mask_b, int Bb, int Wb, void* stream) {
+    if (!lens_a || !mask_a || !lens_b || !mask_b || Ba <= 0 || Bb <= 0 || Wa < 0 || Wb < 0) return fail(CMTTS_E_INVALID, "cmtts_internal_length_masks: bad argument");
+    if (g_masks_merged) {
+        if ((long)Ba * Wa + (long)Bb * Wb > 0) k_length_mask2(lens_a, mask_a, Ba, Wa, lens_b, mask_b, Bb, Wb, (hipStream_t)stream);
+    } else {
+        if (Wa > 0) k_length_mask(lens_a, mask_a, Ba, Wa, (hipStream_t)stream);
+        if (Wb > 0) k_length_mask(lens_b, mask_b, Bb, Wb, (hipStream_t)stream);
+    }
+    HIPCHK(hipGetLastError());
+    return 0;
 }
 
 int cmtts_internal_cond_projections(cmtts_model* m, const float* cond_ct, int B, int T, float* cp, void* stream) {
diff --git a/cm-tts_amd/csrc/cond_gemm.h b/cm-tts_amd/csrc/cond_gemm.h
--- a/cm-tts_amd/csrc/cond_gemm.h
+++ b/cm-tts_amd/csrc/cond_gemm.h
@@ -9,12 +9,15 @@
     int force;
     int flat;
     int row_split;
+    float* Yt;
+    int C;
 };
 
 #ifdef __cplusplus
 extern "C" {
 #endif
 int cmtts_launch_cond_gemm(const CondGemmArgs* a, void* stream);
+int cmtts_cond_gemm_takes_yt(const CondGemmArgs* a);
 int cmtts_launch_cond_expand(const float* p1, int ldp, int L, const float* p2, int ld2, const int64_t* mel2ph, const int64_t* pidx,
                              float* cp, int B, int M, int T, void* stream);
 int cmtts_launch_cond_gemm16(const CondGemmArgs* a, const void* wf16, int mode, void* stream);
diff --git a/cm-tts_amd/csrc/cond_gemm.hip b/cm-tts_amd/csrc/cond_gemm.hip
--- a/cm-tts_amd/csrc/cond_gemm.hip
+++ b/cm-tts_amd/csrc/cond_gemm.hip
@@ -20,6 +20,7 @@
 }
 __device__ __forceinline__ int acc_row(int r, int lane) { return (r & 3) + 8 * (r >> 2) + 4 * (lane >> 5); }
 
+template <bool TR>
 __global__ __launch_bounds__(64 * NW, 2) void cond_gemm_kernel(const CondGemmArgs a) {
     extern __shared__ __attribute__((aligned(16))) float xs[];
     const int tid = threadIdx.x, lane = tid & 63, w = tid >> 6;
@@ -111,29 +112,49 @@
 #pragma unroll
                 for (int r = 0; r < 16; ++r)
                     if (t < ncol) yb[yo + (long)(m0 + acc_row(r, lane)) * T] = acc[i][j][r] + bi[r];
-            }
-        }
-    }
-}
-
+                if (TR && t < ncol) {
+                    const long b = a.flat ? t / T : (long)blockIdx.y, ph = a.flat ? t % T : t;
+                    float* yt = a.Yt + ((b * (a.M / a.C) + m0 / a.C) * T + ph) * a.C + m0 % a.C + 4 * khalf;
+#pragma unroll
+                    for (int q = 0; q < 4; ++q) {
+                        f32x4 v;
+#pragma unroll
+                        for (int e = 0; e < 4; ++e) v[e] = acc[i][j][4 * q + e] + bi[4 * q + e];
+                        *reinterpret_cast<f32x4*>(yt + 8 * q) = v;
+                    }
+                }
+            }
+        }
+    }
+}
+
+}
+
+extern "C" int cmtts_cond_gemm_takes_yt(const CondGemmArgs* ap) {
+    const CondGemmArgs& a = *ap;
+    return a.Yt && a.C >= 32 && a.C % 32 == 0 && a.M % a.C == 0 && ((uintptr_t)a.Yt & 15) == 0;
 }
 
 extern "C" int cmtts_launch_cond_gemm(const CondGemmArgs* ap, void* stream_) {
     const CondGemmArgs& a = *ap;
+    if (a.Yt && !cmtts_cond_gemm_takes_yt(ap)) return -2;
     if (a.K != K || a.M % (32 * MT * NW) != 0 || (long)a.M * a.T >= (1L << 30) || a.B <= 0 || a.T <= 0) return -2;
     if (a.flat && (long)a.B * a.T >= (1L << 30)) return -2;
     if (!a.force && (long)((a.T + FN - 1) / FN) * a.B < 128) return -2;
     static bool attr_set = false;
     const size_t lds = (size_t)K * X_LD * sizeof(float);
     if (!attr_set) {
-        if (hipFuncSetAttribute(reinterpret_cast<const void*>(cond_gemm_kernel), hipFuncAttributeMaxDynamicSharedMemorySize,
+        if (hipFuncSetAttribute(reinterpret_cast<const void*>(cond_gemm_kernel<false>), hipFuncAttributeMaxDynamicSharedMemorySize,
+                                (int)lds) != hipSuccess ||
+            hipFuncSetAttribute(reinterpret_cast<const void*>(cond_gemm_kernel<true>), hipFuncAttributeMaxDynamicSharedMemorySize,
                                 (int)lds) != hipSuccess)
             return -3;
         attr_set = true;
     }
     const int zsplit = a.row_split > 1 ? a.row_split : 1;
     const dim3 grid = a.flat ? dim3((unsigned)(((long)a.B * a.T + FN - 1) / FN), 1, zsplit) : dim3((a.T + FN - 1) / FN, a.B, zsplit);
-    hipLaunchKernelGGL(cond_gemm_kernel, grid, dim3(64 * NW), lds, (hipStream_t)stream_, a);
+    if (a.Yt) hipLaunchKernelGGL(cond_gemm_kernel<true>, grid, dim3(64 * NW), lds, (hipStream_t)stream_, a);
+    else hipLaunchKernelGGL(cond_gemm_kernel<false>, grid, dim3(64 * NW), lds, (hipStream_t)stream_, a);
     return hipGetLastError() == hipSuccess ? 0 : -3;
 }
 
diff --git a/cm-tts_amd/csrc/conv_k5q.hip b/cm-tts_amd/csrc/conv_k5q.hip
--- a/cm-tts_amd/csrc/conv_k5q.hip
+++ b/cm-tts_amd/csrc/conv_k5q.hip
@@ -21,10 +21,11 @@
 constexpr int R = 4;
 constexpr int U = 2;
 
-template <int CIN, bool LN>
-__global__ __launch_bounds__(256, 2) void conv_k5q_kernel(const ConvXlArgs a) {
+template <int CIN, bool LN, bool PH>
+__global__ __launch_bounds__(256, 2) void conv_k5q_kernel(const ConvXlArgs a, const ConvK5qPh ph) {
     constexpr int NKS = CIN / 4;
     static_assert(NKS % U == 0, "k-steps per round");
+    static_assert(!(PH && LN), "the phoneme-level staging is the first block's");
     extern __shared__ __attribute__((aligned(16))) float Xs[];
     const int tid = threadIdx.x, lane = tid & 63, nthr = blockDim.x;
     const int wl = __builtin_amdgcn_readfirstlane(tid >> 6), nwv = nthr >> 6;
@@ -39,7 +40,41 @@
     if (LN) {
         for (int i = tid; i < 256; i += nthr) { gs[i] = a.ln_g[i]; gs[256 + i] = a.ln_b[i]; }
     }
-    {
+    if constexpr (PH) {
+        int* phs = reinterpret_cast<int*>(Xs + CIN * XW);
+        int* pss = phs + XW;
+        for (int c = tid; c < XW; c += nthr) {
+            const int t = t0 - PAD + c;
+            int pv = -1, p = 0;
+            if (c < XIN && t >= 0 && t < T) {
+                const long long v = ph.mel2ph[(long)b * T + t];
+                pv = (int)(v < 0 ? 0 : (v > ph.ld ? ph.ld : v));
+                p = ph.pos[(long)b * T + t];
+                p = p < 0 ? 0 : (p < ph.pe_rows ? p : ph.pe_rows - 1);
+            }
+            phs[c] = pv; pss[c] = p;
+        }
+        __syncthreads();
+        const float al = ph.alpha[0];
+        const float* sb = ph.src + (long)b * CIN * ph.ld;
+        constexpr int total = CIN * NV;
+#pragma unroll 2
+        for (int idx = tid; idx < total; idx += nthr) {
+            const int r = idx / NV, q = idx - r * NV;
+            const float* sc = sb + (long)r * ph.ld;
+            const float pc = ph.pad[r];
+            f32x4 o;
+#pragma unroll
+            for (int c = 0; c < 4; ++c) {
+                const int pv = phs[4 * q + c], p = pss[4 * q + c];
+                const float xv = pv > 0 ? sc[pv - 1] : pc;
+                const float pe = p == 0 ? 0.f : ph.pe_tab[(long)p * CIN + r];
+                const float v = xv + al * pe;
+                o[c] = pv >= 0 ? v : 0.f;
+            }
+            *reinterpret_cast<f32x4*>(Xs + r * XW + 4 * q) = o;
+        }
+    } else {
         const int tbase = t0 - PAD;
         constexpr int total = CIN * NV;
 #pragma unroll 1
@@ -225,18 +260,18 @@
     }
 }
 
-template <int CIN, bool LN>
-int launch_k5q(const ConvXlArgs& a, hipStream_t stream) {
-    const size_t lds = ((size_t)CIN * XW + (LN ? 512 : 0)) * sizeof(float);
+template <int CIN, bool LN, bool PH = false>
+int launch_k5q(const ConvXlArgs& a, hipStream_t stream, const ConvK5qPh& ph = ConvK5qPh()) {
+    const size_t lds = ((size_t)CIN * XW + (LN ? 512 : 0) + (PH ? 2 * XW : 0)) * sizeof(float);
     static bool attr_set = false;
     if (!attr_set) {
-        if (hipFuncSetAttribute(reinterpret_cast<const void*>(conv_k5q_kernel<CIN, LN>), hipFuncAttributeMaxDynamicSharedMemorySize, (int)lds) != hipSuccess) return -3;
+        if (hipFuncSetAttribute(reinterpret_cast<const void*>(conv_k5q_kernel<CIN, LN, PH>), hipFuncAttributeMaxDynamicSharedMemorySize, (int)lds) != hipSuccess) return -3;
         attr_set = true;
     }
     const long tiles = (long)((a.T + BN - 1) / BN) * a.B;
     const int split = a.row_split == 1 || a.row_split == 2 || a.row_split == 4 ? a.row_split : (tiles >= 128 ? 1 : tiles >= 64 ? 2 : 4);
     dim3 grid((a.T + BN - 1) / BN, a.B, split);
-    hipLaunchKernelGGL((conv_k5q_kernel<CIN, LN>), grid, dim3(256 / split), lds, stream, a);
+    hipLaunchKernelGGL((conv_k5q_kernel<CIN, LN, PH>), grid, dim3(256 / split), lds, stream, a, ph);
     return hipGetLastError() == hipSuccess ? 0 : -3;
 }
 
@@ -251,3 +286,10 @@
     if (cin == 128 && !a->ln_g) return launch_k5q<128, false>(*a, s);
     return -2;
 }
+
+extern "C" int cmtts_launch_conv_k5q_ph(const ConvXlArgs* a, const ConvK5qPh* ph, void* stream_) {
+    if (a->C != CO || a->k != KT || a->dil != 1 || a->T < 1 || a->B < 1 || a->res || a->accum || a->slope != 1.0f || !a->wf || !a->bias) return -2;
+    if (a->cin != 128 || a->ln_g) return -2;
+    if (!ph || !ph->src || !ph->pad || !ph->mel2ph || !ph->pos || !ph->alpha || !ph->pe_tab || ph->ld < 1 || a->T >= ph->pe_rows) return -2;
+    return launch_k5q<128, false, true>(*a, (hipStream_t)stream_, *ph);
+}
diff --git a/cm-tts_amd/csrc/internal_hooks.h b/cm-tts_amd/csrc/internal_hooks.h
--- a/cm-tts_amd/csrc/internal_hooks.h
+++ b/cm-tts_amd/csrc/internal_hooks.h
@@ -3,6 +3,7 @@
 extern "C" {
 #endif
 int cmtts_internal_set(const char* name, int value);
+int cmtts_internal_length_masks(const int64_t* lens_a, uint8_t* mask_a, int Ba, int Wa, const int64_t* lens_b, uint8_t* mask_b, int Bb, int Wb, void* stream);
 struct cmtts_model;
 int cmtts_internal_cond_projections(struct cmtts_model* m, const float* cond_ct, int B, int T, float* cp, void* stream);
 int cmtts_internal_cond_factored(struct cmtts_model* m, const float* p1, int p1_ld, int L, const int64_t* mel2ph, const int64_t* p_idx, int B, int T,
diff --git a/cm-tts_amd/csrc/kernels.h b/cm-tts_amd/csrc/kernels.h
--- a/cm-tts_amd/csrc/kernels.h
+++ b/cm-tts_amd/csrc/kernels.h
@@ -46,6 +46,7 @@
                  const int64_t* ln_lens, const int64_t* out_lens, int B, int T, int ld, int O, hipStream_t s);
 void k_cumsum_durations(const float* dur, int* cum, int64_t* mel_len, int B, int L, hipStream_t s);
 void k_mel2ph(const int* cum, int64_t* mel2ph, int B, int L, int T, hipStream_t s);
+void k_mel2ph_pos(const int* cum, int64_t* mel2ph, const float* src, long sbs, const float* padv, int* pos, int B, int L, int T, hipStream_t s);
 void k_length_regulate(const float* out1, const int64_t* mel2ph, float* xlr, int B, int C, int ldl,
                        int T, hipStream_t s, const float* padv = nullptr);
 void k_pitch_index(const float* cwt, int O, const float* mean_p, const float* std_p, int stat_ld, float std_scale,
@@ -64,6 +65,8 @@
                  int C, int T, int ld, int KW, hipStream_t s);
 void k_wav_to_int16(const float* wav, int16_t* pcm, long n, float max_wav, hipStream_t s);
 void k_length_mask(const int64_t* lens, uint8_t* mask, int B, int W, hipStream_t s);
+void k_length_mask2(const int64_t* lens_a, uint8_t* mask_a, int Ba, int Wa, const int64_t* lens_b, uint8_t* mask_b, int Bb, int Wb, hipStream_t s);
+void k_sampler_entry(const float* in, float* out, long n, float sc, float* tb, float tv, int B, const float* row, float* dproj, int nrow, hipStream_t s);
 void k_transpose(const float* in, float* out, int B, int R, int Cn, hipStream_t s);
 void k_fill_lens(int64_t* lens, int64_t v, int B, hipStream_t s);
 void k_gather_rows(const float* table, const int64_t* idx, float* out, int B, int C, int n_rows, hipStream_t s);
diff --git a/cm-tts_amd/csrc/kernels.hip b/cm-tts_amd/csrc/kernels.hip
--- a/cm-tts_amd/csrc/kernels.hip
+++ b/cm-tts_amd/csrc/kernels.hip
@@ -798,6 +798,30 @@
     if (i < n) out[i] = in[i] * sc;
 }
 
+__global__ __launch_bounds__(256) void mel2ph_pos_kernel(const int* cum, int64_t* mel2ph, const float* src, long sbs, const float* padv, int* posg, int L, int T) {
+    extern __shared__ int sh[];
+    int* counts = sh;
+    int* pos = sh + 256;
+    const int b = blockIdx.x;
+    const int* c = cum + (long)b * L;
+    const int total = c[L - 1];
+    for (int t = threadIdx.x; t < T; t += 256) {
+        int r = 0;
+        if (t < total) {
+            int lo = 0, hi = L;
+            while (lo < hi) { const int mid = (lo + hi) >> 1; if (c[mid] > t) hi = mid; else lo = mid + 1; }
+            r = lo + 1;
+        }
+        mel2ph[(long)b * T + t] = r;
+        pos[t] = r;
+    }
+    __syncthreads();
+    const float* s0 = src + (long)b * sbs;
+    const float pad0 = padv[0];
+    block_positions([&](int t) { const int ph = pos[t]; return (ph > 0 ? s0[ph - 1] : pad0) != 0.f; }, T, pos, counts);
+    for (int t = threadIdx.x; t < T; t += 256) posg[(long)b * T + t] = pos[t];
+}
+
 __global__ void pitch_table_scale_kernel(float* cwt, const int64_t* mel2ph, const int* cum, const float* ptab, int O, int L, int T) {
     const int i = blockIdx.x * blockDim.x + threadIdx.x;
     const int b = blockIdx.y;
@@ -815,6 +839,39 @@
 __global__ void fill_float_kernel(float* p, float v, int n) {
     const int i = blockIdx.x * blockDim.x + threadIdx.x;
     if (i < n) p[i] = v;
+}
+
+__global__ void sampler_entry_kernel(const float* in, float* out, long n, float sc, float* tb, float tv, int B, const float* __restrict__ row,
+                                     float* __restrict__ dproj, int nrow, long nbs, int nbr) {
+    long blk = blockIdx.x;
+    if (blk < nbs) {
+        const long i = blk * 256 + threadIdx.x;
+        if (i < n) out[i] = in[i] * sc;
+        return;
+    }
+    blk -= nbs;
+    if (row) {
+        if (blk < (long)nbr * B) {
+            const int b = (int)(blk / nbr), i = (int)(blk - (long)b * nbr) * 256 + threadIdx.x;
+            if (i < nrow) dproj[(long)b * nrow + i] = row[i];
+            return;
+        }
+        blk -= (long)nbr * B;
+    }
+    const long i = blk * 256 + threadIdx.x;
+    if (i < B) tb[i] = tv;
+}
+
+__global__ void length_mask2_kernel(const int64_t* __restrict__ lens_a, uint8_t* __restrict__ mask_a, long na, int Wa,
+                                    const int64_t* __restrict__ lens_b, uint8_t* __restrict__ mask_b, long nb, int Wb, long nba) {
+    const bool first = (long)blockIdx.x < nba;
+    const long i = ((long)blockIdx.x - (first ? 0 : nba)) * 256 + threadIdx.x;
+    const int64_t* lens = first ? lens_a : lens_b;
+    uint8_t* mask = first ? mask_a : mask_b;
+    const int W = first ? Wa : Wb;
+    if (i >= (first ? na : nb)) return;
+    const int b = (int)(i / W), t = (int)(i - (long)b * W);
+    mask[i] = t >= lens[b] ? 1 : 0;
 }
 
 __global__ void fill_lens_kernel(int64_t* lens, int64_t v, int B) {
@@ -982,6 +1039,16 @@
 void k_length_mask(const int64_t* lens, uint8_t* mask, int B, int W, hipStream_t s) {
     hipLaunchKernelGGL(length_mask_kernel, dim3(cdiv((long)B * W, 256)), dim3(256), 0, s, lens, mask, B, W);
 }
+void k_length_mask2(const int64_t* lens_a, uint8_t* mask_a, int Ba, int Wa, const int64_t* lens_b, uint8_t* mask_b, int Bb, int Wb, hipStream_t s) {
+    const long na = (long)Ba * Wa, nb = (long)Bb * Wb, nba = cdiv(na, 256);
+    hipLaunchKernelGGL(length_mask2_kernel, dim3(nba + cdiv(nb, 256)), dim3(256), 0, s, lens_a, mask_a, na, Wa, lens_b, mask_b, nb, Wb, nba);
+}
+void k_sampler_entry(const float* in, float* out, long n, float sc, float* tb, float tv, int B, const float* row, float* dproj, int nrow, hipStream_t s) {
+    const long nbs = cdiv(n, 256);
+    const int nbr = cdiv(nrow, 256);
+    hipLaunchKernelGGL(sampler_entry_kernel, dim3(nbs + (row ? (long)nbr * B : 0) + cdiv(B, 256)), dim3(256), 0, s, in, out, n, sc, tb, tv, B, row, dproj, nrow,
+                       nbs, nbr);
+}
 void k_transpose(const float* in, float* out, int B, int R, int Cn, hipStream_t s) {
     hipLaunchKernelGGL(transpose_kernel, dim3(cdiv(Cn, 32), cdiv(R, 32), B), dim3(256), 0, s, in, out, R, Cn);
 }
@@ -1002,6 +1069,9 @@
 void k_copy_rows(float* dst, int dst_ld, const float* src, int src_ld, int width, long rows, hipStream_t s) {
     hipLaunchKernelGGL(copy_rows_kernel, dim3(cdiv(rows, 4), cdiv(width, 64)), dim3(64, 4), 0, s, dst, dst_ld, src, src_ld, width, rows);
 }
+void k_mel2ph_pos(const int* cum, int64_t* mel2ph, const float* src, long sbs, const float* padv, int* pos, int B, int L, int T, hipStream_t s) {
+    hipLaunchKernelGGL(mel2ph_pos_kernel, dim3(B), dim3(256), (256 + T) * sizeof(int), s, cum, mel2ph, src, sbs, padv, pos, L, T);
+}
 void k_scale(const float* in, float* out, long n, float sc, hipStream_t s) {
     hipLaunchKernelGGL(scale_kernel, dim3(cdiv(n, 256)), dim3(256), 0, s, in, out, n, sc);
 }
diff --git a/cm-tts_amd/csrc/resblock_pair.h b/cm-tts_amd/csrc/resblock_pair.h
--- a/cm-tts_amd/csrc/resblock_pair.h
+++ b/cm-tts_amd/csrc/resblock_pair.h
@@ -36,6 +36,16 @@
     int row_split;
 };
 
+struct ConvK5qPh {
+    const float* src;
+    const float* pad;
+    const long long* mel2ph;
+    const int* pos;
+    const float* alpha;
+    const float* pe_tab;
+    int ld, pe_rows;
+};
+
 struct WinoEntry { signed char acc, a, b, sgn, wkind, tau; };
 #define WINO_F23(t) {0, t, (t) + 2, -1, 0, t}, {1, (t) + 1, (t) + 2, 1, 1, t}, {2, (t) + 2, (t) + 1, -1, 2, t}, {3, (t) + 1, (t) + 3, -1, 3, t}
 #define WINO_F22(t) {0, t, (t) + 1, -1, 0, t}, {1, (t) + 1, 0, 0, 5, t}, {3, (t) + 1, (t) + 2, -1, 6, t}
@@ -53,6 +63,7 @@
 int cmtts_launch_conv_xlq(const ConvXlArgs* a, void* stream);
 int cmtts_launch_conv_xlq_pair(const PairArgs* a, void* stream);
 int cmtts_launch_conv_k5q(const ConvXlArgs* a, void* stream);
+int cmtts_launch_conv_k5q_ph(const ConvXlArgs* a, const ConvK5qPh* ph, void* stream);
 int cmtts_launch_convT(const float* x, float* y, const float* wf, const float* bias, long xbstride, long ybstride, int B, int cin,
                        int co, int Ti, int To, int ldx, int ldy, int s, float pre_div, float slope, void* stream);
 int cmtts_launch_conv_xl16(const ConvXlArgs* a, int mode, int io, void* stream);
diff --git a/cm-tts_amd/host.py b/cm-tts_amd/host.py
--- a/cm-tts_amd/host.py
+++ b/cm-tts_amd/host.py
@@ -136,6 +136,19 @@
         return mask
     ids = torch.arange(0, max_len, device=lengths.device).unsqueeze(0)
     return ids >= lengths.unsqueeze(1)
+
+
+def get_masks_from_lengths(lengths_a, max_len_a, lengths_b, max_len_b):
+    if not (lengths_a.is_cuda and lengths_b.is_cuda and lengths_a.device == lengths_b.device and
+            lengths_a.dtype == torch.int64 and lengths_b.dtype == torch.int64 and lengths_a.shape[0] > 0 and lengths_b.shape[0] > 0):
+        return get_mask_from_lengths(lengths_a, max_len_a), get_mask_from_lengths(lengths_b, max_len_b)
+    lengths_a, lengths_b = lengths_a.contiguous(), lengths_b.contiguous()
+    mask_a = torch.empty(lengths_a.shape[0], int(max_len_a), dtype=torch.bool, device=lengths_a.device)
+    mask_b = torch.empty(lengths_b.shape[0], int(max_len_b), dtype=torch.bool, device=lengths_b.device)
+    with torch.cuda.device(lengths_a.device):
+        _lib.check(_lib.internal_length_masks(_ptr(lengths_a), _ptr(mask_a), lengths_a.shape[0], int(max_len_a),
+                                              _ptr(lengths_b), _ptr(mask_b), lengths_b.shape[0], int(max_len_b), _stream()))
+    return mask_a, mask_b
 
 
 class CondFactors:
@@ -325,7 +338,7 @@
                 if vc is not None:
                     lib.cmtts_set_variance_controls(o._h, None)
                     torch.cuda.current_stream(dev).synchronize()
-        mel_masks = get_mask_from_lengths(mel_len, T)
+        mel_masks, src_masks = get_masks_from_lengths(mel_len, T, src_lens, L)
         factors = None if p1 is None else CondFactors(p1, p1_ld, L, mel2ph, p_idx, cond_ct, p1t)
         cond_ct._cmtts_factors = factors
         return {
@@ -342,7 +355,7 @@
             "mel_lens": mel_len,
             "mel_masks": mel_masks,
             "mel2ph": mel2ph,
-            "src_masks": get_mask_from_lengths(src_lens, L),
+            "src_masks": src_masks,
             "speaker_emb": spk,
             "src_lens": src_lens,
             "enc_out": enc_ct.transpose(1, 2),
```
